# JuanJoZP/cfd-hemodynamic

Hardware: AMD Instinct MI355X
Metric: time-steps/sec, dfg_1 ~1M DOF (stabilized_schur) (higher is better)
Workload: dtype f64 (fp32 only in the AMG matrix values of the flexible preconditioner and in a read-only copy of the Krylov basis that Gram-Schmidt reads in solves of >= 20 iterations)

## Files before the change

### cfd_hemodynamic_amd/_lib.py

```python
from __future__ import annotations

import ctypes as C
import os
import subprocess

import numpy as np

_HERE = os.path.dirname(os.path.abspath(__file__))
_SO = os.path.join(_HERE, "libcfdh.so")
_LIB = None

dp = C.POINTER(C.c_double)
ip = C.POINTER(C.c_int32)
lp = C.POINTER(C.c_int64)


class Options(C.Structure):
    _fields_ = [
        ("snes_rtol", C.c_double), ("snes_atol", C.c_double), ("snes_stol", C.c_double), ("snes_max_it", C.c_int32),
        ("ksp_rtol", C.c_double), ("ksp_atol", C.c_double), ("ksp_max_it", C.c_int32), ("ksp_restart", C.c_int32),
        ("cheb_degree", C.c_int32), ("cheb_ratio", C.c_double), ("schur_full", C.c_int32),
        ("amg_smooth_degree", C.c_int32), ("amg_smooth_ratio", C.c_double), ("amg_theta", C.c_double),
        ("amg_max_coarse", C.c_int32), ("pc_refresh", C.c_int32), ("remove_p_mean", C.c_int32), ("verbose", C.c_int32),
        ("pc_type", C.c_int32), ("cc_smooth_degree", C.c_int32), ("ksp_guess", C.c_int32),
    ]


class Stats(C.Structure):
    _fields_ = [
        ("newton_its", C.c_int32), ("krylov_its", C.c_int32), ("reason", C.c_int32), ("pc_refreshes", C.c_int32),
        ("fnorm0", C.c_double), ("fnorm", C.c_double), ("ms_assemble", C.c_double), ("ms_solve", C.c_double),
        ("ms_pc_setup", C.c_double), ("ms_total", C.c_double),
    ]


class IpcsStats(C.Structure):
    _fields_ = [
        ("its", C.c_int32 * 3), ("reason", C.c_int32 * 3), ("rel_res", C.c_double * 3), ("ms_assemble", C.c_double),
        ("ms_solve", C.c_double * 3), ("ms_total", C.c_double), ("launches", C.c_int32), ("host_syncs", C.c_int32),
    ]


ALLREDUCE_FN = C.CFUNCTYPE(C.c_int, C.c_void_p, dp, C.c_int, C.c_int)
EXCHANGE_FN = C.CFUNCTYPE(C.c_int, C.c_void_p, dp, dp)

SYMBOLS = [
    "cfdh_create", "cfdh_create_elem", "cfdh_create_elem_part", "cfdh_set_facet_markers", "cfdh_destroy", "cfdh_last_error", "cfdh_abi_version", "cfdh_set_params", "cfdh_default_options",
    "cfdh_set_options", "cfdh_clear_dirichlet", "cfdh_add_dirichlet", "cfdh_update_dirichlet", "cfdh_set_state", "cfdh_get_solution",
    "cfdh_get_previous", "cfdh_get_residual", "cfdh_advance", "cfdh_advance_field", "cfdh_set_time_scheme", "cfdh_set_previous2", "cfdh_get_previous2",
    "cfdh_shift_history", "cfdh_set_boundary_terms", "cfdh_set_formulation", "cfdh_set_pressure_boundaries", "cfdh_assemble", "cfdh_get_csr", "cfdh_spmv", "cfdh_solve_step",
    "cfdh_functional", "cfdh_wall_shear_stress", "cfdh_set_global_pressure_space", "cfdh_set_halo", "cfdh_comm_unique_id", "cfdh_comm_init", "cfdh_comm_set_callbacks",
    "cfdh_profile_enable", "cfdh_profile_get", "cfdh_profile_reset", "cfdh_info",
    "cfdh_set_schur_pcd", "cfdh_set_ksp_forcing", "cfdh_get_newton_history", "cfdh_get_pcd_operator", "cfdh_apply_preconditioner", "cfdh_apply_operator",
    "cfdh_get_amg_operator", "cfdh_get_amg_vectors",
    "cfdh_create_ipcs", "cfdh_ipcs_set_form", "cfdh_ipcs_set_tolerances", "cfdh_ipcs_step", "cfdh_ipcs_get_operator", "cfdh_ipcs_get_intermediate",
    "cfdh_ipcs_apply_pressure_pc",
]


def build(force=False):
    src = os.path.join(_HERE, "csrc")
    newest = max(os.path.getmtime(os.path.join(src, f)) for f in os.listdir(src)
                 if f.endswith((".hip", ".cpp", ".hpp", ".h")))
    hdr = os.path.join(os.path.dirname(_HERE), "include", "cfdh.h")
    if os.path.exists(hdr):
        newest = max(newest, os.path.getmtime(hdr))
    if force or not os.path.exists(_SO) or os.path.getmtime(_SO) < newest:
        if not os.path.exists("/opt/rocm/bin/hipcc") and os.path.exists(_SO):
            return _SO
        subprocess.check_call(["make", "-C", src, "-s", "-j4"])
    return _SO


def lib():
    global _LIB
    if _LIB is not None:
        return _LIB
    if not os.path.exists(_SO):
        raise RuntimeError(
            "libcfdh.so is missing (%s): build it with `python -c 'import __graft_entry__ as g; g.build()'`; "
            "this package has no CPU fallback" % _SO)
    L = C.CDLL(_SO)
    vp = C.c_void_p
    L.cfdh_create.argtypes = [C.POINTER(vp), C.c_int, C.c_int, C.c_int64, C.c_int64, C.c_int64, ip, dp, C.c_int64, ip, ip, ip]
    L.cfdh_create_elem.argtypes = [C.POINTER(vp), C.c_int, C.c_int, C.c_int, C.c_int64, C.c_int64, ip, dp, C.c_int64, ip, ip, ip]
    L.cfdh_create_elem_part.argtypes = [C.POINTER(vp), C.c_int, C.c_int, C.c_int, C.c_int64, C.c_int64, C.c_int64, ip, dp, C.c_int64, ip, ip, ip]
    L.cfdh_set_facet_markers.argtypes = [vp, C.c_int64, ip]
    L.cfdh_destroy.argtypes = [vp]
    L.cfdh_destroy.restype = None
    L.cfdh_last_error.argtypes = [vp]
    L.cfdh_last_error.restype = C.c_char_p
    L.cfdh_set_params.argtypes = [vp, C.c_double, C.c_double, C.c_double, C.c_double, dp]
    L.cfdh_default_options.argtypes = [C.POINTER(Options)]
    L.cfdh_set_options.argtypes = [vp, C.POINTER(Options)]
    L.cfdh_clear_dirichlet.argtypes = [vp]
    L.cfdh_add_dirichlet.argtypes = [vp, C.c_int, C.c_int64, ip, dp]
    L.cfdh_update_dirichlet.argtypes = [vp, C.c_int, C.c_int64, ip, dp]
    L.cfdh_set_state.argtypes = [vp, dp, dp, dp, dp]
    L.cfdh_get_solution.argtypes = [vp, dp, dp]
    L.cfdh_set_time_scheme.argtypes = [vp, C.c_double, C.c_double, C.c_double, C.c_double]
    L.cfdh_set_previous2.argtypes = [vp, dp]
    L.cfdh_get_previous2.argtypes = [vp, dp]
    L.cfdh_shift_history.argtypes = [vp]
    L.cfdh_wall_shear_stress.argtypes = [vp, dp]
    L.cfdh_set_boundary_terms.argtypes = [vp, C.c_int, C.c_int, C.c_double]
    L.cfdh_set_formulation.argtypes = [vp, C.c_int]
    L.cfdh_set_pressure_boundaries.argtypes = [vp, C.c_int, ip, dp, C.c_double]
    L.cfdh_get_residual.argtypes = [vp, dp, dp]
    L.cfdh_get_previous.argtypes = [vp, dp, dp]
    L.cfdh_advance.argtypes = [vp]
    L.cfdh_advance_field.argtypes = [vp, C.c_int]
    L.cfdh_assemble.argtypes = [vp, C.c_int]
    L.cfdh_get_csr.argtypes = [vp, lp, ip, ip, dp]
    L.cfdh_spmv.argtypes = [vp, dp, dp]
    L.cfdh_solve_step.argtypes = [vp, C.POINTER(Stats)]
    L.cfdh_functional.argtypes = [vp, C.c_int, C.c_int, dp]
    L.cfdh_set_halo.argtypes = [vp, C.c_int, ip, lp, ip, lp, ip]
    L.cfdh_set_global_pressure_space.argtypes = [vp, C.c_int64, C.c_int64, ip, dp, ip, C.c_int64, ip]
    L.cfdh_comm_unique_id.argtypes = [C.c_void_p]
    L.cfdh_comm_init.argtypes = [vp, C.c_void_p, C.c_int, C.c_int]
    L.cfdh_comm_set_callbacks.argtypes = [vp, ALLREDUCE_FN, EXCHANGE_FN, C.c_void_p, C.c_int, C.c_int]
    L.cfdh_profile_enable.argtypes = [vp, C.c_int]
    L.cfdh_profile_get.argtypes = [vp, C.c_int, dp, lp]
    L.cfdh_profile_reset.argtypes = [vp]
    L.cfdh_info.argtypes = [vp, C.c_int]
    L.cfdh_info.restype = C.c_int64
    L.cfdh_set_schur_pcd.argtypes = [vp, C.c_int, C.c_int, C.c_int]
    L.cfdh_set_ksp_forcing.argtypes = [vp, C.c_int, C.c_double, C.c_double, C.c_double, C.c_double, C.c_double]
    L.cfdh_get_newton_history.argtypes = [vp, ip, dp, dp, ip, dp]
    L.cfdh_get_pcd_operator.argtypes = [vp, lp, ip, ip, dp, dp]
    L.cfdh_apply_preconditioner.argtypes = [vp, dp, dp]
    L.cfdh_apply_operator.argtypes = [vp, dp, dp, dp]
    L.cfdh_get_amg_operator.argtypes = [vp, C.c_int, C.c_int, C.c_int, lp, lp, lp, ip, ip, dp]
    L.cfdh_get_amg_vectors.argtypes = [vp, C.c_int, C.c_int, C.c_int, lp, dp]
    L.cfdh_create_ipcs.argtypes = [C.POINTER(vp), C.c_int, C.c_int, C.c_int64, C.c_int64, C.c_int64, ip, dp, C.c_int64, ip, ip, ip]
    L.cfdh_ipcs_set_form.argtypes = [vp, C.c_double, C.c_double]
    L.cfdh_ipcs_set_tolerances.argtypes = [vp, dp, C.c_double, ip]
    L.cfdh_ipcs_step.argtypes = [vp, C.POINTER(IpcsStats)]
    L.cfdh_ipcs_get_operator.argtypes = [vp, C.c_int, lp, ip, ip, dp]
    L.cfdh_ipcs_get_intermediate.argtypes = [vp, C.c_int, dp]
    L.cfdh_ipcs_apply_pressure_pc.argtypes = [vp, dp, dp]
    _LIB = L
    return L


def _dp(a):
    return None if a is None else a.ctypes.data_as(dp)


def _ip(a):
    return None if a is None else a.ctypes.data_as(ip)


def _lp(a):
    return None if a is None else a.ctypes.data_as(lp)


class CfdhError(RuntimeError):
    pass


def _raise(code, msg):
    if code == -1:
        raise ValueError(msg)
    raise CfdhError(msg)


FORM_CONVECTIVE, FORM_ROTATIONAL = 0, 1
PC_SELFP, PC_CAHOUET_CHABARD, PC_PCD = 0, 1, 2
AMG_HIER_A, AMG_HIER_P, AMG_HIER_H = 0, 1, 2
AMG_OP_A, AMG_OP_P, AMG_OP_G, AMG_OP_SB, AMG_OP_SC = 0, 1, 2, 3, 4
(AMG_VEC_DINV, AMG_VEC_WDINV, AMG_VEC_AGG, AMG_VEC_COARSE_INV, AMG_VEC_D, AMG_VEC_LAMBDA, AMG_VEC_CC_SCALARS, AMG_VEC_CC_ML,
 AMG_VEC_CC_PBC, AMG_VEC_SPGEMM_ROWS, AMG_VEC_SHAPE, AMG_VEC_ORDER, AMG_VEC_A00_LMAX, AMG_VEC_A00_DINV) = range(14)
EW_DEFAULTS = (0.3, 0.9, 1.0, (1.0 + 5.0 ** 0.5) / 2.0, 0.1)


class Context:

    def __init__(self, x, cells, facet_cells, facet_local, facet_marker, nv_owned=None, device=0, etype=0):
        L = lib()
        self.L = L
        x = np.asarray(x, dtype=np.float64)
        cells = np.asarray(cells)
        self.etype = int(etype)
        self.dim = (3 if x.shape[1] >= 3 and cells.shape[1] in (8, 10) or (self.etype == 3 and cells.shape[1] == 4) else 2) if self.etype \
            else cells.shape[1] - 1
        if self.dim not in (2, 3) or x.shape[1] < self.dim:
            raise ValueError("cells must be triangles [nc,3] or tetrahedra [nc,4] with matching coordinates")
        nodes = {(1, 2): 6, (2, 2): 4, (3, 2): 3, (1, 3): 10, (2, 3): 8, (3, 3): 4}
        if self.etype and cells.shape[1] != nodes[(self.etype, self.dim)]:
            raise ValueError("element type %d needs %d nodes per cell for gdim %d" % (self.etype, nodes[(self.etype, self.dim)], self.dim))
        self.x = np.ascontiguousarray(x[:, : self.dim]).copy()
        self.cells = np.ascontiguousarray(cells, dtype=np.int32)
        self.nv = len(self.x)
        self.nvo = self.nv if nv_owned is None else int(nv_owned)
        fc = np.ascontiguousarray(facet_cells, dtype=np.int32)
        fl = np.ascontiguousarray(facet_local, dtype=np.int32)
        fm = np.ascontiguousarray(facet_marker, dtype=np.int32)
        h = C.c_void_p()
        if self.etype:
            if self.nvo != self.nv:
                rc = L.cfdh_create_elem_part(C.byref(h), int(device), self.dim, self.etype, self.nv, self.nvo, len(self.cells), _ip(self.cells),
                                             _dp(self.x), len(fc), _ip(fc), _ip(fl), _ip(fm))
            else:
                rc = L.cfdh_create_elem(C.byref(h), int(device), self.dim, self.etype, self.nv, len(self.cells), _ip(self.cells), _dp(self.x),
                                        len(fc), _ip(fc), _ip(fl), _ip(fm))
        else:
            rc = L.cfdh_create(C.byref(h), int(device), self.dim, self.nv, self.nvo, len(self.cells), _ip(self.cells), _dp(self.x),
                               len(fc), _ip(fc), _ip(fl), _ip(fm))
        if rc != 0:
            _raise(rc, "cfdh_create failed: " + L.cfdh_last_error(None).decode())
        self.h = h
        self._cb = None

    def close(self):
# ... 144 lines not shown
        self._chk(self.L.cfdh_functional(self.h, int(kind), int(marker), C.byref(out)))
        return out.value

    def set_halo(self, nbr_rank, send_ptr, send_idx, recv_ptr, recv_idx):
        a = np.ascontiguousarray(nbr_rank, dtype=np.int32)
        sp_ = np.ascontiguousarray(send_ptr, dtype=np.int64)
        si = np.ascontiguousarray(send_idx, dtype=np.int32)
        rp = np.ascontiguousarray(recv_ptr, dtype=np.int64)
        ri = np.ascontiguousarray(recv_idx, dtype=np.int32)
        self._chk(self.L.cfdh_set_halo(self.h, len(a), _ip(a), _lp(sp_), _ip(si), _lp(rp), _ip(ri)))

    def set_global_pressure_space(self, x_global, cells_global, owned_global, pbc_nodes_global):
        xg = np.ascontiguousarray(x_global, dtype=np.float64)[:, : self.dim].copy()
        cg = np.ascontiguousarray(cells_global, dtype=np.int32)
        og = np.ascontiguousarray(owned_global, dtype=np.int32)
        pb = np.ascontiguousarray(pbc_nodes_global, dtype=np.int32)
        self._chk(self.L.cfdh_set_global_pressure_space(self.h, len(xg), len(cg), _ip(cg), _dp(xg), _ip(og), len(pb), _ip(pb)))

    def comm_init_rccl(self, uid_bytes, rank, nranks):
        buf = C.create_string_buffer(bytes(uid_bytes), 128)
        self._chk(self.L.cfdh_comm_init(self.h, buf, int(rank), int(nranks)))

    def comm_set_callbacks(self, allreduce, exchange, rank, nranks):
        self._cb = (ALLREDUCE_FN(allreduce), EXCHANGE_FN(exchange))
        self._chk(self.L.cfdh_comm_set_callbacks(self.h, self._cb[0], self._cb[1], None, int(rank), int(nranks)))

    def profile_enable(self, on=True):
        self._chk(self.L.cfdh_profile_enable(self.h, int(on)))

    def profile_reset(self):
        self._chk(self.L.cfdh_profile_reset(self.h))

    def profile_get(self, kind):
        ms, n = C.c_double(), C.c_int64()
        self._chk(self.L.cfdh_profile_get(self.h, int(kind), C.byref(ms), C.byref(n)))
        return ms.value, n.value

    def info(self, what):
        return int(self.L.cfdh_info(self.h, int(what)))

    def set_schur_pcd(self, inlet_marker, outlet_marker, time_term=1):
        self._chk(self.L.cfdh_set_schur_pcd(self.h, int(inlet_marker), int(outlet_marker), int(time_term)))

    def set_ksp_forcing(self, version=2, rtol_0=None, rtol_max=None, gamma=None, alpha=None, threshold=None):
        a = [d if v is None else float(v) for v, d in zip((rtol_0, rtol_max, gamma, alpha, threshold), EW_DEFAULTS)]
        self._chk(self.L.cfdh_set_ksp_forcing(self.h, int(version), *a))

    def newton_history(self):
        n = C.c_int32()
        self._chk(self.L.cfdh_get_newton_history(self.h, C.byref(n), None, None, None, None))
        fn, rt, rr = np.zeros(n.value), np.zeros(n.value), np.zeros(n.value)
        its = np.zeros(n.value, dtype=np.int32)
        self._chk(self.L.cfdh_get_newton_history(self.h, C.byref(n), _dp(fn), _dp(rt), _ip(its), _dp(rr)))
        return {"fnorm": fn, "ksp_rtol": rt, "ksp_its": its, "ksp_rel_res": rr}

    def get_pcd_operator(self):
        import scipy.sparse as sp
        nnz = C.c_int64()
        self._chk(self.L.cfdh_get_pcd_operator(self.h, C.byref(nnz), None, None, None, None))
        rowptr = np.empty(self.nvo + 1, dtype=np.int32)
        col = np.empty(nnz.value, dtype=np.int32)
        val = np.empty(nnz.value)
        md = np.empty(self.nvo)
        self._chk(self.L.cfdh_get_pcd_operator(self.h, C.byref(nnz), _ip(rowptr), _ip(col), _dp(val), _dp(md)))
        return sp.csr_matrix((val, col, rowptr), shape=(self.nvo, self.nv)), md

    def apply_preconditioner(self, r):
        r = np.ascontiguousarray(r, dtype=np.float64)
        if r.size != (self.dim + 1) * self.nv:
            raise ValueError("monolithic vector of (gdim + 1) nv entries expected")
        z = np.zeros_like(r)
        self._chk(self.L.cfdh_apply_preconditioner(self.h, _dp(r), _dp(z)))
        return z

    def apply_operator(self, r):
        r = np.ascontiguousarray(r, dtype=np.float64)
        if r.size != (self.dim + 1) * self.nv:
            raise ValueError("monolithic vector of (gdim + 1) nv entries expected")
        z = np.zeros_like(r)
        w = np.zeros((self.dim + 1) * self.nvo)
        self._chk(self.L.cfdh_apply_operator(self.h, _dp(r), _dp(z), _dp(w)))
        return z, w

    def get_amg_operator(self, hier, level, which, raw=False):
        import scipy.sparse as sp
        nr, nc, nnz = C.c_int64(), C.c_int64(), C.c_int64()
        self._chk(self.L.cfdh_get_amg_operator(self.h, int(hier), int(level), int(which), C.byref(nr), C.byref(nc), C.byref(nnz), None, None, None))
        rowptr = np.empty(nr.value + 1, dtype=np.int32)
        col = np.empty(nnz.value, dtype=np.int32)
        val = np.empty(nnz.value)
        self._chk(self.L.cfdh_get_amg_operator(self.h, int(hier), int(level), int(which), C.byref(nr), C.byref(nc), C.byref(nnz), _ip(rowptr),
                                               _ip(col), _dp(val)))
        if raw:
            return rowptr, col, val, (nr.value, nc.value), nnz.value
        return sp.csr_matrix((val, col, rowptr), shape=(nr.value, nc.value))

    def get_amg_vectors(self, hier, level, which):
        n = C.c_int64()
        self._chk(self.L.cfdh_get_amg_vectors(self.h, int(hier), int(level), int(which), C.byref(n), None))
        out = np.empty(n.value)
        self._chk(self.L.cfdh_get_amg_vectors(self.h, int(hier), int(level), int(which), C.byref(n), _dp(out)))
        return out


class IpcsContext(Context):

    def __init__(self, x, cells, nvert, facet_cells, facet_local, facet_marker, device=0):
        L = lib()
        self.L = L
        cells = np.ascontiguousarray(cells, dtype=np.int32)
        if cells.ndim != 2 or cells.shape[1] not in (6, 10):
            raise ValueError("cells must list the 6 nodes of P2 triangles or the 10 nodes of P2 tetrahedra")
        self.dim = 2 if cells.shape[1] == 6 else 3
        self.etype = 1
        self.x = np.ascontiguousarray(np.asarray(x, dtype=np.float64)[:, : self.dim]).copy()
        self.cells = cells
        self.nv = self.nvo = len(self.x)
        self.nvert = int(nvert)
        fc = np.ascontiguousarray(facet_cells, dtype=np.int32)
        fl = np.ascontiguousarray(facet_local, dtype=np.int32)
        fm = np.ascontiguousarray(facet_marker, dtype=np.int32)
        h = C.c_void_p()
        rc = L.cfdh_create_ipcs(C.byref(h), int(device), self.dim, self.nv, self.nvert, len(cells), _ip(cells), _dp(self.x), len(fc), _ip(fc), _ip(fl),
                                _ip(fm))
        if rc != 0:
            _raise(rc, "cfdh_create_ipcs failed: " + L.cfdh_last_error(None).decode())
        self.h = h
        self._cb = None

    def set_state(self, u_prev=None, p_prev=None, u=None, p=None):
        a = [None if v is None else np.ascontiguousarray(v, dtype=np.float64).reshape(-1) for v in (u_prev, p_prev, u, p)]
        for v, n in zip(a, (self.dim * self.nv, self.nvert, self.dim * self.nv, self.nvert)):
            if v is not None and v.size != n:
                raise ValueError("state array has wrong size")
        self._chk(self.L.cfdh_set_state(self.h, _dp(a[0]), _dp(a[1]), _dp(a[2]), _dp(a[3])))

    def get_solution(self, u=None, p=None):
        u = np.empty(self.dim * self.nv) if u is None else u
        p = np.empty(self.nvert) if p is None else p
        self._chk(self.L.cfdh_get_solution(self.h, _dp(u), _dp(p)))
        return u, p

    def get_previous(self, u=None, p=None):
        u = np.empty(self.dim * self.nv) if u is None else u
        p = np.empty(self.nvert) if p is None else p
        self._chk(self.L.cfdh_get_previous(self.h, _dp(u), _dp(p)))
        return u, p

    def set_form(self, conv_coeff, force_coeff):
        self._chk(self.L.cfdh_ipcs_set_form(self.h, float(conv_coeff), float(force_coeff)))

    def set_tolerances(self, rtol=(1e-5, 1e-5, 1e-5), atol=1e-50, max_it=(10000, 10000, 10000)):
        r = np.ascontiguousarray(np.broadcast_to(np.asarray(rtol, dtype=np.float64), (3,)))
        m = np.ascontiguousarray(np.broadcast_to(np.asarray(max_it, dtype=np.int32), (3,)))
        self._chk(self.L.cfdh_ipcs_set_tolerances(self.h, _dp(r), float(atol), _ip(m)))

    def step(self):
        st = IpcsStats()
        rc = self.L.cfdh_ipcs_step(self.h, C.byref(st))
        if rc != 0:
            msg = self.L.cfdh_last_error(self.h).decode()
            if rc == -4:
                bad = [r for r in st.reason if r <= 0]
                raise RuntimeError("Did not converge, reason: %d. (%s)" % (bad[0] if bad else 0, msg))
            _raise(rc, msg)
        return st
# ... 35 lines not shown
```

### cfd_hemodynamic_amd/csrc/cfdh_amg_dev.hip

```cpp
#include <hip/hip_runtime.h>

#include <algorithm>
#include <chrono>
#include <cmath>

#include "cfdh_internal.hpp"

#define TPB 256

namespace {

double now_ms() {
  using namespace std::chrono;
  return duration<double, std::milli>(steady_clock::now().time_since_epoch()).count();
}

__device__ __forceinline__ int wave_incl_scan(int v, int lane) {
#pragma unroll
  for (int d = 1; d < 64; d <<= 1) {
    const int t = __shfl_up(v, d);
    if (lane >= d) v += t;
  }
  return v;
}
__global__ __launch_bounds__(TPB) void scan_block_kernel(int n, int *__restrict__ a, int *__restrict__ sums) {
  __shared__ int wsum[4];
  const int t = threadIdx.x, lane = t & 63, wv = t >> 6;
  const int base = blockIdx.x * 1024 + t * 4;
  int v[4], s = 0;
#pragma unroll
  for (int q = 0; q < 4; q++) { v[q] = base + q < n ? a[base + q] : 0; s += v[q]; v[q] = s; }
  int inc = wave_incl_scan(s, lane);
  if (lane == 63) wsum[wv] = inc;
  __syncthreads();
  int off = inc - s;
  for (int w = 0; w < wv; w++) off += wsum[w];
#pragma unroll
  for (int q = 0; q < 4; q++) if (base + q < n) a[base + q] = v[q] + off;
  if (t == TPB - 1) sums[blockIdx.x] = off + s;
}
__global__ __launch_bounds__(TPB) void scan_sums_kernel(int nb, int *__restrict__ sums) {
  __shared__ int wsum[4];
  __shared__ int carry_s;
  const int t = threadIdx.x, lane = t & 63, wv = t >> 6;
  if (t == 0) carry_s = 0;
  __syncthreads();
  for (int b0 = 0; b0 < nb; b0 += TPB) {
    const int v = b0 + t < nb ? sums[b0 + t] : 0;
    int inc = wave_incl_scan(v, lane);
    if (lane == 63) wsum[wv] = inc;
    __syncthreads();
    int off = carry_s;
    for (int w = 0; w < wv; w++) off += wsum[w];
    if (b0 + t < nb) sums[b0 + t] = inc + off;
    __syncthreads();
    if (t == TPB - 1) carry_s = inc + off;
    __syncthreads();
  }
}
__global__ __launch_bounds__(TPB) void scan_add_kernel(int n, int *__restrict__ a, const int *__restrict__ sums) {
  const int b = blockIdx.x + 1;
  const int off = sums[b - 1];
  const int base = b * 1024 + threadIdx.x * 4;
#pragma unroll
  for (int q = 0; q < 4; q++) if (base + q < n) a[base + q] += off;
}

struct Dev {
  cfdh_ctx *c;
  hipStream_t s;
  dbuf<int> scan_sums;
  int rc = 0;
  long long *path_rows = nullptr;
  explicit Dev(cfdh_ctx *c_) : c(c_), s(c_->stream) {}
  int scan(int *a, int n) {
    if (n <= 0) return 0;
    const int nb = (n + 1023) / 1024;
    if ((size_t)nb > scan_sums.n) HIPCHK(c, scan_sums.alloc((size_t)nb + 1024));
    hipLaunchKernelGGL(scan_block_kernel, dim3(nb), dim3(TPB), 0, s, n, a, scan_sums.p);
    if (nb > 1) {
      hipLaunchKernelGGL(scan_sums_kernel, dim3(1), dim3(TPB), 0, s, nb, scan_sums.p);
      hipLaunchKernelGGL(scan_add_kernel, dim3(nb - 1), dim3(TPB), 0, s, n, a, scan_sums.p);
    }
    HIPCHK(c, hipGetLastError());
    return 0;
  }
  int read_int(const int *p, int *out) {
    HIPCHK(c, hipMemcpyAsync(out, p, sizeof(int), hipMemcpyDeviceToHost, s));
    HIPCHK(c, hipStreamSynchronize(s));
// ... 806 lines not shown
    *na_out = na;
    return 0;
  }
};

struct ProxyF {
  const double *A00;
  int dim, nvo;
  __device__ double value(int i, int k, int w) const {
    double v = 0.0;
    for (int q = 0; q < dim; q++) v += A00[(size_t)dim * dim * k + (size_t)q * (dim + 1)];
    return v / dim;
  }
  __device__ bool whole_row_identity(int) const { return false; }
  __device__ bool keep(int i, int k, int w) const { return w < nvo && (w == i || value(i, k, w) != 0.0); }
};
struct HF {
  const double *A11, *Lval, *Ml;
  const unsigned char *pbc;
  const int *vdiag;
  double alpha, beta;
  int nvo;
  __device__ bool whole_row_identity(int i) const { return (pbc[i] & 1) != 0; }
  __device__ bool keep(int, int, int w) const { return w < nvo && !(pbc[w] & 1); }
  __device__ double value(int i, int k, int w) const {
    double v = beta * A11[k];
    if (w == i) {
      const int kd = vdiag[i];
      const double T = Lval[kd] > 0 ? A11[kd] / Lval[kd] : 0.0;
      v += (1.0 + alpha * T) * Ml[i];
    }
    return v;
  }
};
template <class F>
__global__ __launch_bounds__(TPB) void vg_count_kernel(int n, const int *__restrict__ vptr, const int *__restrict__ vcol, F f, int *__restrict__ rp1) {
  const int i = blockIdx.x * TPB + threadIdx.x;
  if (i >= n) return;
  int cnt = 0;
  if (f.whole_row_identity(i)) cnt = 1;
  else for (int k = vptr[i], e = vptr[i + 1]; k < e; k++) cnt += f.keep(i, k, vcol[k]) ? 1 : 0;
  rp1[i + 1] = cnt;
}
template <class F>
__global__ __launch_bounds__(TPB) void vg_fill_kernel(int n, const int *__restrict__ vptr, const int *__restrict__ vcol, F f, const int *__restrict__ rp,
                                                      int *__restrict__ col, double *__restrict__ val) {
  const int i = blockIdx.x * TPB + threadIdx.x;
  if (i >= n) return;
  int p = rp[i];
  if (f.whole_row_identity(i)) { col[p] = i; val[p] = 1.0; return; }
  for (int k = vptr[i], e = vptr[i + 1]; k < e; k++) {
    const int w = vcol[k];
    if (f.keep(i, k, w)) { col[p] = w; val[p] = f.value(i, k, w); p++; }
  }
}
template <class F>
int vg_build(cfdh_ctx *c, F f, CsrDev &out) {
  Dev dv(c);
  hipStream_t s = c->stream;
  const int n = c->nvo;
  out.n = out.m = n;
  HIPCHK(c, out.rowptr.alloc((size_t)n + 1));
  HIPCHK(c, hipMemsetAsync(out.rowptr.p, 0, sizeof(int), s));
  hipLaunchKernelGGL((vg_count_kernel<F>), dim3((n + TPB - 1) / TPB), dim3(TPB), 0, s, n, c->vptr.p, c->vcol.p, f, out.rowptr.p);
  CHK(dv.scan(out.rowptr.p + 1, n));
  int nnz = 0;
  CHK(dv.read_int(out.rowptr.p + n, &nnz));
  out.nnz = nnz;
  HIPCHK(c, out.col.alloc((size_t)std::max(nnz, 1)));
  HIPCHK(c, out.val.alloc((size_t)std::max(nnz, 1)));
  hipLaunchKernelGGL((vg_fill_kernel<F>), dim3((n + TPB - 1) / TPB), dim3(TPB), 0, s, n, c->vptr.p, c->vcol.p, f, out.rowptr.p, out.col.p, out.val.p);
  HIPCHK(c, hipGetLastError());
  return 0;
}

static void move_csr(CsrDev &dst, CsrDev &src) {
  dst.n = src.n; dst.m = src.m; dst.nnz = src.nnz;
  dst.rowptr.adopt(src.rowptr); dst.col.adopt(src.col); dst.val.adopt(src.val);
}

}

int cfdh_aggregate_host_csr(const CsrHost &A, double theta, std::vector<int> &agg);

int cfdh_amg_setup_dev(cfdh_ctx *c, AmgHier &H, CsrDev &A0, bool singular, int ncol) {
  const double t_begin = now_ms();
  Builder B(c);
  hipStream_t s = c->stream;
  const cfdh_options &o = c->opt;
  H.clear();
  H.ncol = ncol;
  H.fused = false; H.nnz_G0 = H.nnz_S0 = 0;
  H.fine_nnz = A0.nnz;
  const char *ml_env = getenv(&H == &c->hA ? "CFDH_A_MAXLEV" : "CFDH_L_MAXLEV");
  const int maxlev = ml_env && atoi(ml_env) >= 1 ? std::min(atoi(ml_env), 16) : 16;
  static const double theta_env = getenv("CFDH_AMG_THETA") ? atof(getenv("CFDH_AMG_THETA")) : -1.0;
  const double theta = o.amg_theta >= 0 ? o.amg_theta : (theta_env >= 0 ? theta_env : (c->dim == 3 ? 0.02 : 0.07));
  const bool host_agg = getenv("CFDH_AMG_AGG") && !strcmp(getenv("CFDH_AMG_AGG"), "host");
  const bool keep = getenv("CFDH_AMG_KEEP") && getenv("CFDH_AMG_KEEP")[0] == '1';
  for (long long &q : H.spgemm_rows) q = 0;
  B.dv.path_rows = H.spgemm_rows;
  const bool velocity = &H == &c->hA;
  const char *gap_env = getenv(velocity ? "CFDH_AGG_GAP_A" : "CFDH_AGG_GAP_L");
  if (!gap_env) gap_env = getenv("CFDH_AGG_GAP");
  const int gap = gap_env ? atoi(gap_env) : (velocity ? 4 : 0);
  CsrDev A;
  move_csr(A, A0);
  AmgLevel *lastL = nullptr;
  double tm[10] = {0, 0, 0, 0, 0, 0, 0, 0, 0, 0}, tq = now_ms();
  const bool timing = c->opt.verbose > 0;
#define TICK(i) do { if (timing) { (void)hipStreamSynchronize(s); const double n_ = now_ms(); tm[i] += n_ - tq; tq = n_; } } while (0)
  for (;;) {
    AmgLevel *L = new AmgLevel();
    H.lev.push_back(L);
    double lm = 1.0;
    TICK(9);
    CHK(B.level_quantities(*L, A, o.amg_smooth_ratio, &lm));
    CHK(B.work_vectors(*L, ncol));
    TICK(0);
    L->fine = A.nnz <= (c->dim == 3 ? 20ll : 12ll) * A.n && A.n >= 16384;
    L->sell = L->fine && (A.nnz <= 12ll * A.n || ncol == 1);
    const bool last = A.n <= o.amg_max_coarse || (int)H.lev.size() >= maxlev;
    int na = 0;
    dbuf<int> agg;
    static const bool no_pmg = getenv("CFDH_NO_PMG") && getenv("CFDH_NO_PMG")[0] == '1';
    const bool pmg = !last && !no_pmg && H.lev.size() == 1 && c->etype == 1 && c->gen_P1.n == A.n && c->gen_P1.m > 0;
    if (!last && !pmg) {
      if (host_agg) {
        CsrHost Ah;
        Ah.n = Ah.m = A.n;
        Ah.rowptr.resize((size_t)A.n + 1); Ah.col.resize(A.nnz); Ah.val.resize(A.nnz);
        HIPCHK(c, hipMemcpyAsync(Ah.rowptr.data(), A.rowptr.p, sizeof(int) * ((size_t)A.n + 1), hipMemcpyDeviceToHost, s));
        HIPCHK(c, hipMemcpyAsync(Ah.col.data(), A.col.p, sizeof(int) * (size_t)A.nnz, hipMemcpyDeviceToHost, s));
        HIPCHK(c, hipMemcpyAsync(Ah.val.data(), A.val.p, sizeof(double) * (size_t)A.nnz, hipMemcpyDeviceToHost, s));
        HIPCHK(c, hipStreamSynchronize(s));
        std::vector<int> ha;
        na = cfdh_aggregate_host_csr(Ah, theta, ha);
        HIPCHK(c, agg.upload(ha, s));
        HIPCHK(c, hipStreamSynchronize(s));
      } else {
        CHK(B.aggregate(A, theta, gap, agg, &na));
      }
    }
    TICK(1);
    if (pmg) na = c->gen_P1.m;
    if (last || na >= A.n || na < 1) {
      move_csr(L->A, A);
      break;
    }
    const MatV Am{A.rowptr.p, A.col.p, A.val.p};
    CsrDev P, R, AP, Ac;
    if (pmg) {
      P.n = c->gen_P1.n; P.m = c->gen_P1.m; P.nnz = c->gen_P1.nnz();
      HIPCHK(c, P.rowptr.upload(c->gen_P1.rowptr, s)); HIPCHK(c, P.col.upload(c->gen_P1.col, s)); HIPCHK(c, P.val.upload(c->gen_P1.val, s));
      HIPCHK(c, hipStreamSynchronize(s));
    } else
    CHK((Spgemm<AOpImwDA, BOpAgg>::run(B.dv, A.n, na, AOpImwDA{Am, L->dinv.p, 4.0 / 3.0 / lm, agg.p}, BOpAgg{agg.p}, P, B.lists, B.tmp, B.cnts)));
    TICK(2);
    if (H.keep_host0 && H.lev.size() == 1) {
      auto down = [&](const CsrDev &D, CsrHost &Hc) -> int {
        Hc.n = D.n; Hc.m = D.m;
        Hc.rowptr.resize((size_t)D.n + 1); Hc.col.resize((size_t)D.nnz); Hc.val.resize((size_t)D.nnz);
        HIPCHK(c, hipMemcpyAsync(Hc.rowptr.data(), D.rowptr.p, sizeof(int) * ((size_t)D.n + 1), hipMemcpyDeviceToHost, s));
        HIPCHK(c, hipMemcpyAsync(Hc.col.data(), D.col.p, sizeof(int) * (size_t)D.nnz, hipMemcpyDeviceToHost, s));
        HIPCHK(c, hipMemcpyAsync(Hc.val.data(), D.val.p, sizeof(double) * (size_t)D.nnz, hipMemcpyDeviceToHost, s));
        return 0;
// ... 1 lines not shown
      CHK(down(A, H.h_A0)); CHK(down(P, H.h_P0));
      H.h_wdinv0.resize((size_t)A.n);
      HIPCHK(c, hipMemcpyAsync(H.h_wdinv0.data(), L->wdinv.p, sizeof(double) * (size_t)A.n, hipMemcpyDeviceToHost, s));
      HIPCHK(c, hipStreamSynchronize(s));
    }
    CHK(B.transpose(P, R));
    TICK(3);
    const MatV Pm{P.rowptr.p, P.col.p, P.val.p}, Rm{R.rowptr.p, R.col.p, R.val.p};
    CHK((Spgemm<AOpPlain, BOpPlain>::run(B.dv, A.n, na, AOpPlain{Am}, BOpPlain{Pm}, AP, B.lists, B.tmp, B.cnts)));
    TICK(4);
    CHK((Spgemm<AOpPlain, BOpImAW>::run(B.dv, na, A.n, AOpPlain{Rm}, BOpImAW{Am, L->wdinv.p}, L->G, B.lists, B.tmp, B.cnts)));
    TICK(5);
    L->Sb.n = A.n; L->Sb.m = A.n; L->Sb.nnz = A.nnz;
    HIPCHK(c, L->Sb.rowptr.alloc((size_t)A.n + 1)); HIPCHK(c, L->Sb.col.alloc(A.nnz)); HIPCHK(c, L->Sb.val.alloc(A.nnz));
    HIPCHK(c, hipMemcpyAsync(L->Sb.rowptr.p, A.rowptr.p, sizeof(int) * ((size_t)A.n + 1), hipMemcpyDeviceToDevice, s));
    HIPCHK(c, hipMemcpyAsync(L->Sb.col.p, A.col.p, sizeof(int) * (size_t)A.nnz, hipMemcpyDeviceToDevice, s));
    hipLaunchKernelGGL(sb_kernel, dim3((unsigned)((8ll * A.n + TPB - 1) / TPB)), dim3(TPB), 0, s, A.n, A.rowptr.p, A.col.p, A.val.p, L->wdinv.p, L->Sb.val.p);
    L->Sc.n = A.n; L->Sc.m = na; L->Sc.nnz = AP.nnz;
    HIPCHK(c, L->Sc.rowptr.alloc((size_t)A.n + 1)); HIPCHK(c, L->Sc.col.alloc(std::max(AP.nnz, 1))); HIPCHK(c, L->Sc.val.alloc(std::max(AP.nnz, 1)));
    HIPCHK(c, hipMemcpyAsync(L->Sc.rowptr.p, AP.rowptr.p, sizeof(int) * ((size_t)A.n + 1), hipMemcpyDeviceToDevice, s));
    HIPCHK(c, hipMemcpyAsync(L->Sc.col.p, AP.col.p, sizeof(int) * (size_t)AP.nnz, hipMemcpyDeviceToDevice, s));
    hipLaunchKernelGGL(sc_kernel, dim3((A.n + TPB - 1) / TPB), dim3(TPB), 0, s, A.n, AP.rowptr.p, AP.col.p, AP.val.p, P.rowptr.p, P.col.p, P.val.p,
                       L->wdinv.p, L->Sc.val.p);
    HIPCHK(c, hipGetLastError());
    TICK(6);
    const MatV APm{AP.rowptr.p, AP.col.p, AP.val.p};
    CHK((Spgemm<AOpPlain, BOpPlain>::run(B.dv, na, na, AOpPlain{Rm}, BOpPlain{APm}, Ac, B.lists, B.tmp, B.cnts)));
    TICK(7);
    if (L->fine) CHK(B.formats(L->G, CFDH_UP_CSRF));
    if (L->sell) { CHK(B.formats(L->Sb, CFDH_UP_SELL)); CHK(B.formats(L->Sc, CFDH_UP_SELL)); }
    if (H.lev.size() == 1) { H.nnz_G0 = L->G.nnz; H.nnz_S0 = (long long)L->Sb.nnz + L->Sc.nnz; }
    if (c->nranks > 1) { move_csr(L->P, P); move_csr(L->R, R); }
    else if (keep) { move_csr(L->P, P); L->agg.adopt(agg); }
    move_csr(L->A, A);
    lastL = L;
    move_csr(A, Ac);
    HIPCHK(c, hipStreamSynchronize(s));
    TICK(8);
  }
  tq = now_ms();
  AmgLevel *Lc = H.lev.back();
  const int n = Lc->n;
  H.coarse_n = 0;
  if (n > 2500) {
    CsrDev &A = Lc->A;
    Lc->Sb.n = n; Lc->Sb.m = n; Lc->Sb.nnz = A.nnz;
    HIPCHK(c, Lc->Sb.rowptr.alloc((size_t)n + 1)); HIPCHK(c, Lc->Sb.col.alloc(A.nnz)); HIPCHK(c, Lc->Sb.val.alloc(A.nnz));
    HIPCHK(c, hipMemcpyAsync(Lc->Sb.rowptr.p, A.rowptr.p, sizeof(int) * ((size_t)n + 1), hipMemcpyDeviceToDevice, s));
    HIPCHK(c, hipMemcpyAsync(Lc->Sb.col.p, A.col.p, sizeof(int) * (size_t)A.nnz, hipMemcpyDeviceToDevice, s));
    hipLaunchKernelGGL(sb_kernel, dim3((unsigned)((8ll * n + TPB - 1) / TPB)), dim3(TPB), 0, s, n, A.rowptr.p, A.col.p, A.val.p, Lc->wdinv.p, Lc->Sb.val.p);
    if (Lc->sell) CHK(B.formats(Lc->Sb, CFDH_UP_SELL));
    H.fused = true;
  } else {
    dbuf<double> D0, D1, ad;
    dbuf<int> failf;
    HIPCHK(c, D0.alloc((size_t)n * n)); HIPCHK(c, D1.alloc((size_t)n * n)); HIPCHK(c, ad.alloc(n)); HIPCHK(c, failf.alloc(4));
    HIPCHK(c, D0.zero(s)); HIPCHK(c, failf.zero(s));
    hipLaunchKernelGGL(densify_kernel, dim3((n + TPB - 1) / TPB), dim3(TPB), 0, s, n, Lc->A.rowptr.p, Lc->A.col.p, Lc->A.val.p, D0.p, ad.p);
    if (singular) hipLaunchKernelGGL(trace_shift_kernel, dim3(64), dim3(TPB), 0, s, n, ad.p, D0.p);
    const unsigned gb = (unsigned)(((size_t)n * n + TPB - 1) / TPB);
    double *in = D0.p, *out = D1.p;
    for (int p = 0; p < n; p++) { hipLaunchKernelGGL(gj_step_kernel, dim3(gb), dim3(TPB), 0, s, n, p, in, out, failf.p); std::swap(in, out); }
    HIPCHK(c, hipGetLastError());
    int hf = 0;
    CHK(B.dv.read_int(failf.p, &hf));
    if (hf) return cfdh_fail(c, CFDH_E_STATE, "singular coarsest AMG operator (n=%d, device Gauss-Jordan)", n);
    HIPCHK(c, H.coarse_inv.alloc((size_t)n * n));
    HIPCHK(c, hipMemcpyAsync(H.coarse_inv.p, in, sizeof(double) * (size_t)n * n, hipMemcpyDeviceToDevice, s));
    H.coarse_n = n;
    if (lastL) {
      H.fused = true;
      lastL->Dn = 0;
      const long long ent = (long long)lastL->n * n;
      if (lastL->Sc.m == n && ent <= 8000000ll && !lastL->sell) {
        HIPCHK(c, lastL->D.alloc((size_t)ent));
        hipLaunchKernelGGL(fold_dense_kernel, dim3(lastL->n), dim3(TPB), 0, s, lastL->n, n, lastL->Sc.rowptr.p, lastL->Sc.col.p, lastL->Sc.val.p,
                           H.coarse_inv.p, lastL->D.p);
        HIPCHK(c, hipGetLastError());
        lastL->Dn = n;
      }
    }
    HIPCHK(c, hipStreamSynchronize(s));
  }
  H.valid = true;
  HIPCHK(c, hipStreamSynchronize(s));
  if (c->opt.verbose) {
    fprintf(stderr, "[cfdh] AMG hierarchy built on the device in %.1f ms (ncol %d%s):", now_ms() - t_begin, ncol, H.fused ? ", fused" : "");
    for (AmgLevel *l : H.lev) fprintf(stderr, " (%d, nnz %d; G %d Sb %d Sc %d D %d)", l->n, l->A.nnz, l->G.nnz, l->Sb.nnz, l->Sc.nnz, l->Dn);
    fprintf(stderr, "\n[cfdh]   ms: level quantities %.1f, aggregation %.1f, P %.1f, R = P^T %.1f, A P %.1f, G %.1f, Sb + Sc %.1f, A_c %.1f, formats %.1f, releases %.1f, "
            "coarsest level %.1f\n", tm[0], tm[1], tm[2], tm[3], tm[4], tm[5], tm[6], tm[7], tm[8], tm[9], now_ms() - tq);
  }
#undef TICK
  return 0;
}

int cfdh_level_setup_dev(cfdh_ctx *c, AmgLevel &L, CsrDev &A, double ratio, int ncol) {
  Builder B(c);
  double lm;
  CHK(B.level_quantities(L, A, ratio, &lm));
  CHK(B.work_vectors(L, ncol));
  move_csr(L.A, A);
  CHK(B.formats(L.A, CFDH_UP_SELL, L.wdinv.p));
  HIPCHK(c, hipStreamSynchronize(c->stream));
  return 0;
}

bool cfdh_amg_dev_enabled(const cfdh_ctx *c) {
  const bool host_only = getenv("CFDH_AMG_HOST") && getenv("CFDH_AMG_HOST")[0] == '1';
  const char *nf = getenv("CFDH_NO_FUSED_AMG");
  return !host_only && c->opt.amg_smooth_degree == 1 && !(nf && nf[0] == '1');
}

int cfdh_proxy_dev(cfdh_ctx *c, CsrDev &out) { return vg_build(c, ProxyF{c->A00.p, c->dim, c->nvo}, out); }

namespace {
__global__ __launch_bounds__(TPB) void ras_pack_kernel(int nvo, int dim, int k0, const int *__restrict__ vptr, const int *__restrict__ vcol,
                                                       const double *__restrict__ A00, const int *__restrict__ gid, double *__restrict__ rec) {
  const int i = blockIdx.x * TPB + threadIdx.x;
  if (i >= nvo) return;
  for (int t = 0; t <= dim; t++) {
    const int k = vptr[i] + k0 + t;
    double v = gid ? -1.0 : 0.0;
    if (k < vptr[i + 1]) {
      if (gid) v = (double)gid[vcol[k]];
      else {
        v = 0.0;
        for (int q = 0; q < dim; q++) v += A00[(size_t)dim * dim * k + (size_t)q * (dim + 1)];
        v /= dim;
      }
    }
    rec[t < dim ? (size_t)dim * i + t : (size_t)dim * nvo + i] = v;
  }
}
__global__ __launch_bounds__(TPB) void ras_unpack_kernel(int ng, int nvo, int dim, int k0, int maxlen, const double *__restrict__ rec,
                                                         double *__restrict__ gval) {
  const int g = blockIdx.x * TPB + threadIdx.x;
  if (g >= ng) return;
  const size_t W = (size_t)dim + 1;
  for (int t = 0; t <= dim; t++)
    if (k0 + t < maxlen) gval[(size_t)g * maxlen + k0 + t] = rec[W * (size_t)nvo + W * (size_t)g + t];
}
__device__ __forceinline__ double ras_proxy_value(const double *A00, int dim, int k) {
  double v = 0.0;
  for (int q = 0; q < dim; q++) v += A00[(size_t)dim * dim * k + (size_t)q * (dim + 1)];
  return v / dim;
}
template <bool FILL>
__global__ __launch_bounds__(TPB) void ras_rows_kernel(int nv, int nvo, int dim, int maxlen, const int *__restrict__ vptr, const int *__restrict__ vcol,
                                                       const double *__restrict__ A00, const int *__restrict__ gptr, const int *__restrict__ gcol,
                                                       const int *__restrict__ gsrc, const double *__restrict__ gval, int *__restrict__ rp,
                                                       int *__restrict__ col, double *__restrict__ val) {
  const int i = blockIdx.x * TPB + threadIdx.x;
  if (i >= nv) return;
  int p = FILL ? rp[i] : 0;
  if (i < nvo) {
    for (int k = vptr[i], e = vptr[i + 1]; k < e; k++) {
      const int w = vcol[k];
      if (w >= nv) continue;
      const double v = ras_proxy_value(A00, dim, k);
      if (v == 0.0 && w != i) continue;
      if (FILL) { col[p] = w; val[p] = v; }
      p++;
    }
  } else {
    const int g = i - nvo;
    for (int j = gptr[g], e = gptr[g + 1]; j < e; j++) {
// ... 97 lines not shown
```

### cfd_hemodynamic_amd/csrc/cfdh_api.cpp

```cpp
#include <algorithm>
#include <cmath>
#include <numeric>

#include <dlfcn.h>

#include "cfdh_internal.hpp"
#include "cfdh_ipcs.hpp"

std::string g_cfdh_last_error;

int cfdh_prepare_assembly(cfdh_ctx *c);

#define ENTER(c)                         \
  do {                                   \
    if (!(c)) return CFDH_E_ARG;         \
    (void)hipSetDevice((c)->device);     \
  } while (0)

#define NOT_IPCS(c, name)                                                                                                    \
  do {                                                                                                                       \
    if ((c) && (c)->ipcs) return cfdh_fail((c), CFDH_E_STATE, name ": not available on an incremental pressure-correction context (cfdh_create_ipcs)"); \
  } while (0)
#define NEED_IPCS(c, name)                                                                                         \
  do {                                                                                                             \
    if (!(c)) return CFDH_E_ARG;                                                                                   \
    if (!(c)->ipcs) return cfdh_fail((c), CFDH_E_STATE, name ": the context was not created by cfdh_create_ipcs"); \
    (void)hipSetDevice((c)->device);                                                                               \
  } while (0)

static int ipcs_put(cfdh_ctx *c, dbuf<double> &dst, const double *src) {
  if (!src) return 0;
  c->ipcs->n_field_copies++;
  HIPCHK(c, hipMemcpyAsync(dst.p, src, sizeof(double) * dst.n, hipMemcpyHostToDevice, c->stream));
  HIPCHK(c, hipStreamSynchronize(c->stream));
  return 0;
}
static int ipcs_get(cfdh_ctx *c, const dbuf<double> &src, double *dst) {
  if (!dst) return 0;
  c->ipcs->n_field_copies++;
  HIPCHK(c, hipMemcpyAsync(dst, src.p, sizeof(double) * src.n, hipMemcpyDeviceToHost, c->stream));
  HIPCHK(c, hipStreamSynchronize(c->stream));
  return 0;
}
static int ipcs_copy(cfdh_ctx *c, const dbuf<double> &src, dbuf<double> &dst) {
  HIPCHK(c, hipMemcpyAsync(dst.p, src.p, sizeof(double) * src.n, hipMemcpyDeviceToDevice, c->stream));
  return 0;
}

extern "C" {

int cfdh_abi_version(void) { return CFDH_ABI_VERSION; }

const char *cfdh_last_error(const cfdh_ctx *c) { return c ? c->err.c_str() : g_cfdh_last_error.c_str(); }

int cfdh_default_options(cfdh_options *o) {
  if (!o) return CFDH_E_ARG;
  o->snes_rtol = 1e-8; o->snes_atol = 1e-50; o->snes_stol = 1e-8; o->snes_max_it = 100;
  o->ksp_rtol = 1e-5; o->ksp_atol = 1e-50; o->ksp_max_it = 1000; o->ksp_restart = 200;
  o->cheb_degree = 3; o->cheb_ratio = 10.0; o->schur_full = 2;
  o->amg_smooth_degree = 1; o->amg_smooth_ratio = 8.0; o->amg_theta = -1.0; o->amg_max_coarse = 1000;
  o->pc_refresh = 0; o->remove_p_mean = 1; o->verbose = 0; o->pc_type = 1; o->cc_smooth_degree = 2;
  o->ksp_guess = getenv("CFDH_KSP_GUESS") ? atoi(getenv("CFDH_KSP_GUESS")) : 4;
  return 0;
}

static int create_ctx(cfdh_ctx **out, int device, int gdim, int etype, int64_t nv, int64_t nv_owned, int64_t nc, const int32_t *cells,
                      const double *coords, int64_t nfacets, const int32_t *facet_cells, const int32_t *facet_local,
                      const int32_t *facet_marker) {
  if (!out) return cfdh_fail(nullptr, CFDH_E_ARG, "null output pointer");
  *out = nullptr;
  if (gdim != 2 && gdim != 3) return cfdh_fail(nullptr, CFDH_E_ARG, "gdim must be 2 (P1 triangles) or 3 (P1 tetrahedra)");
  if (etype < 0 || etype > 3) return cfdh_fail(nullptr, CFDH_E_ARG, "unknown element type %d", etype);
  if (!cells || !coords || (nfacets > 0 && (!facet_cells || !facet_local)))
    return cfdh_fail(nullptr, CFDH_E_ARG, "null mesh array");
  int ndev = 0;
  if (hipGetDeviceCount(&ndev) != hipSuccess || ndev <= 0)
    return cfdh_fail(nullptr, CFDH_E_HIP, "no HIP device available: libcfdh has no CPU fallback");
  if (device < 0 || device >= ndev) return cfdh_fail(nullptr, CFDH_E_ARG, "device %d out of range (%d devices)", device, ndev);
  cfdh_ctx *c = new (std::nothrow) cfdh_ctx();
  if (!c) return cfdh_fail(nullptr, CFDH_E_NOMEM, "out of host memory");
  c->device = device;
  cfdh_default_options(&c->opt);
  { const char *e = getenv("CFDH_NO_GRAPH"); c->use_graph = !(e && e[0] == '1'); }
  { const char *e = getenv("CFDH_SOLVE_LEAN"); c->lean = !(e && e[0] == '0'); }
  {
    cfdh_ctx::SolveEnv &v = c->env;
    const char *e;
    if ((e = getenv("CFDH_KRYLOV_FP32"))) v.krylov_fp32 = atoi(e);
    v.guess_check = getenv("CFDH_GUESS_CHECK") != nullptr;
    e = getenv("CFDH_NO_ATTAINABLE_STOP"); v.no_attainable_stop = e && e[0] == '1';
    if ((e = getenv("CFDH_GS_REFINE_FROM"))) v.gs_refine_from = atoi(e);
    if ((e = getenv("CFDH_KSP_LAG"))) v.ksp_lag = atoi(e);
    if ((e = getenv("CFDH_GS_ETA2"))) v.gs_eta2 = atof(e);
    if ((e = getenv("CFDH_L_CYCLES"))) v.l_cycles = atoi(e);
    if ((e = getenv("CFDH_A_CYCLES"))) v.a_cycles = atoi(e);
  }
  if (c->use_graph && (getenv("ROCP_TOOL_LIBRARIES") || dlsym(RTLD_DEFAULT, "rocprofiler_configure"))) {
    int rt = 0;
    const char *ov = getenv("CFDH_GRAPH_UNDER_PROFILER");
    if (!(ov && ov[0] == '1') && hipRuntimeGetVersion(&rt) == hipSuccess && rt >= 70200000) c->use_graph = false;
  }
  memset(&c->last_stats, 0, sizeof c->last_stats);
  int rc = 0;
  do {
    if (hipSetDevice(device) != hipSuccess) { rc = cfdh_fail(nullptr, CFDH_E_HIP, "hipSetDevice(%d) failed", device); break; }
    if (hipStreamCreateWithFlags(&c->stream, hipStreamNonBlocking) != hipSuccess) { rc = cfdh_fail(nullptr, CFDH_E_HIP, "hipStreamCreate failed"); break; }
    rc = gdim == 3 ? k3_upload_quadrature(c) : k_upload_quadrature(c);
    if (rc) break;
    if (etype != 0) {
      rc = gdim == 3 ? kg3_upload_tables(c) : kg_upload_tables(c);
      if (rc) break;
      rc = gdim == 3 ? cfdh_build_mesh_gen3(c, etype, nv, nv_owned, nc, cells, coords, nfacets, facet_cells, facet_local, facet_marker)
                     : cfdh_build_mesh_gen(c, etype, nv, nv_owned, nc, cells, coords, nfacets, facet_cells, facet_local, facet_marker);
      break;
    }
    rc = gdim == 3 ? cfdh_build_mesh3(c, nv, nv_owned, nc, cells, coords, nfacets, facet_cells, facet_local, facet_marker)
                   : cfdh_build_mesh(c, nv, nv_owned, nc, cells, coords, nfacets, facet_cells, facet_local, facet_marker);
  } while (0);
  if (rc) {
    g_cfdh_last_error = c->err.empty() ? g_cfdh_last_error : c->err;
    cfdh_destroy(c);
    return rc;
  }
  *out = c;
  return 0;
}

int cfdh_create(cfdh_ctx **out, int device, int gdim, int64_t nv, int64_t nv_owned, int64_t nc, const int32_t *cells,
                const double *coords, int64_t nfacets, const int32_t *facet_cells, const int32_t *facet_local,
                const int32_t *facet_marker) {
  return create_ctx(out, device, gdim, CFDH_ELEM_P1, nv, nv_owned, nc, cells, coords, nfacets, facet_cells, facet_local, facet_marker);
}

int cfdh_create_elem(cfdh_ctx **out, int device, int gdim, int elem, int64_t nn, int64_t nc, const int32_t *cells, const double *node_coords,
                     int64_t nfacets, const int32_t *facet_cells, const int32_t *facet_local, const int32_t *facet_marker) {
  return create_ctx(out, device, gdim, elem, nn, nn, nc, cells, node_coords, nfacets, facet_cells, facet_local, facet_marker);
}

int cfdh_create_elem_part(cfdh_ctx **out, int device, int gdim, int elem, int64_t nn, int64_t nn_owned, int64_t nc, const int32_t *cells,
                          const double *node_coords, int64_t nfacets, const int32_t *facet_cells, const int32_t *facet_local, const int32_t *facet_marker) {
  return create_ctx(out, device, gdim, elem, nn, nn_owned, nc, cells, node_coords, nfacets, facet_cells, facet_local, facet_marker);
}

void cfdh_destroy(cfdh_ctx *c) {
  if (!c) return;
  (void)hipSetDevice(c->device);
  if (c->stream) (void)hipStreamSynchronize(c->stream);
  cfdh_ipcs_free(c);
  comm_finalize(c);
  c->hS.clear(); c->hL.clear(); c->hA.clear(); c->hLg.clear();
  for (hipEvent_t e : c->ev_pool) (void)hipEventDestroy(e);
  for (auto &e : c->pc_graphs) for (auto &x : e.exec) if (x) (void)hipGraphExecDestroy(x);
  if (c->h_pinned) (void)hipHostFree(c->h_pinned);
  if (c->h_stage) (void)hipHostFree(c->h_stage);
  if (c->ev_h) (void)hipEventDestroy(c->ev_h);
  if (c->h_big) (void)hipHostFree(c->h_big);
  if (c->h_ring) (void)hipHostFree(c->h_ring);
  for (hipEvent_t e : c->ev_ring) if (e) (void)hipEventDestroy(e);
  hipStream_t s = c->stream;
  delete c;
  if (s) (void)hipStreamDestroy(s);
}

int cfdh_set_params(cfdh_ctx *c, double dt, double rho, double mu, double mu_facet, const double f[3]) {
  ENTER(c);
  if (!(dt > 0) || !(rho > 0) || !(mu > 0)) return cfdh_fail(c, CFDH_E_ARG, "dt, rho, mu must be positive");
  const bool changed = !c->params_set || dt != c->dt || rho != c->rho || mu != c->mu;
// ... 372 lines not shown
  const bool markers_changed = !c->pcd_set || inlet_marker != c->pcd_in || outlet_marker != c->pcd_out;
  c->pcd_in = inlet_marker; c->pcd_out = outlet_marker; c->pcd_time = time_term;
  c->pcd_set = true;
  if (markers_changed) { c->pcd_ready = false; c->pc_valid = false; }
  return 0;
}

int cfdh_set_ksp_forcing(cfdh_ctx *c, int version, double rtol_0, double rtol_max, double gamma, double alpha, double threshold) {
  NOT_IPCS(c, "cfdh_set_ksp_forcing");
  ENTER(c);
  if (version != 0 && version != 2) return cfdh_fail(c, CFDH_E_ARG, "cfdh_set_ksp_forcing: version 0 (off) or 2");
  if (version == 2 && !(rtol_0 > 0 && rtol_0 < 1 && rtol_max > 0 && rtol_max < 1 && gamma > 0 && gamma <= 1 && alpha > 1 && alpha <= 2 &&
                        threshold > 0 && threshold < 1))
    return cfdh_fail(c, CFDH_E_ARG, "cfdh_set_ksp_forcing: need 0 < rtol_0, rtol_max, threshold < 1, 0 < gamma <= 1, 1 < alpha <= 2");
  c->ew_version = version;
  if (version == 2) { c->ew_rtol0 = rtol_0; c->ew_rtol_max = rtol_max; c->ew_gamma = gamma; c->ew_alpha = alpha; c->ew_threshold = threshold; }
  return 0;
}

int cfdh_get_newton_history(cfdh_ctx *c, int32_t *n, double *fnorm, double *ksp_rtol, int32_t *ksp_its, double *ksp_rel_res) {
  NOT_IPCS(c, "cfdh_get_newton_history");
  if (!c || !n) return CFDH_E_ARG;
  const size_t m = c->hist_fnorm.size();
  *n = (int32_t)m;
  for (size_t k = 0; k < m; k++) {
    if (fnorm) fnorm[k] = c->hist_fnorm[k];
    if (ksp_rtol) ksp_rtol[k] = c->hist_rtol[k];
    if (ksp_its) ksp_its[k] = c->hist_its[k];
    if (ksp_rel_res) ksp_rel_res[k] = c->hist_relres[k];
  }
  return 0;
}

int cfdh_get_pcd_operator(cfdh_ctx *c, int64_t *nnz, int32_t *rowptr, int32_t *col, double *vals, double *mass_diag) {
  NOT_IPCS(c, "cfdh_get_pcd_operator");
  if (!c || !nnz) return CFDH_E_ARG;
  ENTER(c);
  *nnz = c->nnzv;
  if (!rowptr && !col && !vals && !mass_diag) return 0;
  if (!rowptr || !col || !vals) return cfdh_fail(c, CFDH_E_ARG, "pass all of rowptr/col/vals or none");
  CHK(cfdh_pcd_supported(c, "cfdh_get_pcd_operator"));
  if (!c->pcd_set) return cfdh_fail(c, CFDH_E_STATE, "cfdh_get_pcd_operator: cfdh_set_schur_pcd was not called");
  if (!c->params_set || !c->state_set) return cfdh_fail(c, CFDH_E_STATE, "cfdh_get_pcd_operator: parameters and state are needed");
  CHK(k_pcd_assemble(c, c->x.p));
  std::vector<double> K(c->pcd_K.n);
  std::vector<int> sptr(c->pcd_sptr.n);
  HIPCHK(c, hipMemcpyAsync(K.data(), c->pcd_K.p, sizeof(double) * K.size(), hipMemcpyDeviceToHost, c->stream));
  HIPCHK(c, hipMemcpyAsync(sptr.data(), c->pcd_sptr.p, sizeof(int) * sptr.size(), hipMemcpyDeviceToHost, c->stream));
  HIPCHK(c, hipStreamSynchronize(c->stream));
  const int nvo = c->nvo;
  int64_t pos = 0;
  std::vector<std::pair<int, int>> ord;
  for (int vu = 0; vu < nvo; vu++) {
    const int r = c->perm[vu];
    ord.clear();
    for (int k = c->h_vptr[r]; k < c->h_vptr[r + 1]; k++) ord.push_back({c->iperm[c->h_vcol[k]], k - c->h_vptr[r]});
    std::sort(ord.begin(), ord.end());
    rowptr[vu] = (int32_t)pos;
    const size_t base = (size_t)sptr[r >> 6] + (r & 63);
    for (auto &e : ord) { col[pos] = e.first; vals[pos] = K[base + 64 * (size_t)e.second]; pos++; }
  }
  rowptr[nvo] = (int32_t)pos;
  if (mass_diag) for (int vu = 0; vu < nvo; vu++) mass_diag[vu] = c->h_pcd_md[c->perm[vu]];
  return 0;
}

int cfdh_apply_preconditioner(cfdh_ctx *c, const double *r, double *z) {
  NOT_IPCS(c, "cfdh_apply_preconditioner");
  if (!c || !r || !z) return CFDH_E_ARG;
  ENTER(c);
  if (!c->jac_valid) return cfdh_fail(c, CFDH_E_STATE, "no Jacobian assembled yet");
  CHK(cfdh_pc_update(c, false));
  std::vector<double> h;
  pack_vec(c, r, r + (size_t)c->dim * c->nv, h, nullptr);
  CHK(upload_vec(c, h, c->xt.p));
  CHK(cfdh_pc_apply(c, c->xt.p, c->dvec.p));
  std::vector<double> o;
  CHK(download_vec(c, c->dvec.p, o));
  for (int k = 0; k < c->nvo; k++) {
    const int v = c->iperm[k], d = c->dim;
    for (int i = 0; i < d; i++) z[(size_t)d * v + i] = o[(size_t)d * k + i];
    z[(size_t)d * c->nv + v] = o[(size_t)d * c->nvo + k];
  }
  return 0;
}

int cfdh_apply_operator(cfdh_ctx *c, const double *r, double *z, double *w) {
  NOT_IPCS(c, "cfdh_apply_operator");
  if (!c || !r || !z || !w) return CFDH_E_ARG;
  ENTER(c);
  if (c->nranks > 1 || c->nvo != c->nv) return cfdh_fail(c, CFDH_E_STATE, "cfdh_apply_operator: one GPU only");
  if (!c->jac_valid) return cfdh_fail(c, CFDH_E_STATE, "no Jacobian assembled yet");
  CHK(cfdh_pc_update(c, false));
  std::vector<double> h;
  pack_vec(c, r, r + (size_t)c->dim * c->nv, h, nullptr);
  CHK(upload_vec(c, h, c->xt.p));
  CHK(cfdh_apply_operator_dev(c, c->xt.p, c->dvec.p));
  std::vector<double> oz, ow;
  CHK(download_vec(c, c->dvec.p, oz));
  CHK(download_vec(c, c->kw.p, ow));
  for (int k = 0; k < c->nvo; k++) {
    const int v = c->iperm[k], d = c->dim;
    for (int i = 0; i < d; i++) { z[(size_t)d * v + i] = oz[(size_t)d * k + i]; w[(size_t)d * v + i] = ow[(size_t)d * k + i]; }
    z[(size_t)d * c->nv + v] = oz[(size_t)d * c->nvo + k];
    w[(size_t)d * c->nvo + v] = ow[(size_t)d * c->nvo + k];
  }
  return 0;
}

static int amg_pick(cfdh_ctx *c, const char *name, int hier, int level, AmgHier **H, AmgLevel **L) {
  if (c->nranks > 1 || c->nvo != c->nv) return cfdh_fail(c, CFDH_E_STATE, "%s: one GPU only", name);
  if (!c->pc_valid) return cfdh_fail(c, CFDH_E_STATE, "%s: no preconditioner built yet (cfdh_apply_preconditioner or cfdh_solve_step first)", name);
  *H = nullptr;
  if (hier == CFDH_AMG_HIER_H) {
    if (c->opt.pc_type != 1 || c->Hlev.n <= 0) return cfdh_fail(c, CFDH_E_STATE, "%s: H exists for pc_type 1 only", name);
    *L = &c->Hlev;
    return 0;
  }
  if (hier != CFDH_AMG_HIER_A && hier != CFDH_AMG_HIER_P) return cfdh_fail(c, CFDH_E_ARG, "%s: unknown hierarchy %d", name, hier);
  if (hier == CFDH_AMG_HIER_A && c->opt.pc_type == 0) return cfdh_fail(c, CFDH_E_STATE, "%s: pc_type 0 has no velocity hierarchy", name);
  AmgHier *h = hier == CFDH_AMG_HIER_A ? &c->hA : (c->opt.pc_type == 0 ? &c->hS : &c->hL);
  if (!h->valid) return cfdh_fail(c, CFDH_E_STATE, "%s: hierarchy %d is not built", name, hier);
  if (level < 0 || level >= (int)h->lev.size()) return cfdh_fail(c, CFDH_E_ARG, "%s: level %d of %d", name, level, (int)h->lev.size());
  *H = h;
  *L = h->lev[level];
  return 0;
}

int cfdh_get_amg_operator(cfdh_ctx *c, int hier, int level, int which, int64_t *nrow, int64_t *ncol, int64_t *nnz, int32_t *rowptr,
                          int32_t *col, double *vals) {
  NOT_IPCS(c, "cfdh_get_amg_operator");
  if (!c || !nrow || !ncol || !nnz) return CFDH_E_ARG;
  ENTER(c);
  AmgHier *H = nullptr;
  AmgLevel *L = nullptr;
  CHK(amg_pick(c, "cfdh_get_amg_operator", hier, level, &H, &L));
  if (which < CFDH_AMG_OP_A || which > CFDH_AMG_OP_SC) return cfdh_fail(c, CFDH_E_ARG, "cfdh_get_amg_operator: unknown operator %d", which);
  if (!H) level = 0;
  const CsrDev &M = which == CFDH_AMG_OP_A ? L->A : which == CFDH_AMG_OP_P ? L->P : which == CFDH_AMG_OP_G ? L->G : which == CFDH_AMG_OP_SB ? L->Sb : L->Sc;
  if (M.n <= 0 || !M.rowptr.p || !M.col.p || !M.val.p)
    return cfdh_fail(c, CFDH_E_STATE, "cfdh_get_amg_operator: operator %d of level %d is not kept in fp64 CSR (P: CFDH_AMG_KEEP=1 before the build)", which, level);
  *nrow = M.n; *ncol = M.m; *nnz = M.nnz;
  if (!rowptr && !col && !vals) return 0;
  if (!rowptr || !col || !vals) return cfdh_fail(c, CFDH_E_ARG, "pass all of rowptr/col/vals or none");
  std::vector<int> rp((size_t)M.n + 1), cl((size_t)M.nnz);
  std::vector<double> vl((size_t)M.nnz);
  HIPCHK(c, hipMemcpyAsync(rp.data(), M.rowptr.p, sizeof(int) * rp.size(), hipMemcpyDeviceToHost, c->stream));
  if (M.nnz > 0) {
    HIPCHK(c, hipMemcpyAsync(cl.data(), M.col.p, sizeof(int) * cl.size(), hipMemcpyDeviceToHost, c->stream));
    HIPCHK(c, hipMemcpyAsync(vl.data(), M.val.p, sizeof(double) * vl.size(), hipMemcpyDeviceToHost, c->stream));
  }
  HIPCHK(c, hipStreamSynchronize(c->stream));
  if (rp[M.n] != M.nnz) return cfdh_fail(c, CFDH_E_STATE, "cfdh_get_amg_operator: rowptr ends at %d, the operator holds %d entries", rp[M.n], M.nnz);
  const bool rows0 = level == 0 && which != CFDH_AMG_OP_G && (int)c->perm.size() == M.n;
  const bool cols0 = level == 0 && (which == CFDH_AMG_OP_A || which == CFDH_AMG_OP_SB || which == CFDH_AMG_OP_G) && (int)c->iperm.size() == M.m;
  int64_t pos = 0;
  std::vector<std::pair<int, double>> row;
  for (int ru = 0; ru < M.n; ru++) {
    const int r = rows0 ? c->perm[ru] : ru;
    rowptr[ru] = (int32_t)pos;
    row.clear();
    for (int k = rp[r]; k < rp[r + 1]; k++) row.push_back({cols0 ? c->iperm[cl[k]] : cl[k], vl[k]});
    if (cols0) std::stable_sort(row.begin(), row.end(), [](const std::pair<int, double> &a, const std::pair<int, double> &b) { return a.first < b.first; });
    for (auto &e : row) { col[pos] = e.first; vals[pos] = e.second; pos++; }
  }
  rowptr[M.n] = (int32_t)pos;
// ... 435 lines not shown
  return 0;
}
int cfdh_profile_get(cfdh_ctx *c, int kind, double *total_ms, int64_t *launches) {
  NOT_IPCS(c, "cfdh_profile_get");
  if (!c || kind < 0 || kind >= 12) return CFDH_E_ARG;
  prof_flush(c);
  if (total_ms) *total_ms = c->prof[kind].total_ms;
  if (launches) *launches = c->prof[kind].launches;
  return 0;
}
int cfdh_profile_reset(cfdh_ctx *c) {
  NOT_IPCS(c, "cfdh_profile_reset");
  ENTER(c);
  prof_flush(c);
  for (auto &p : c->prof) { p.total_ms = 0; p.launches = 0; }
  c->n_allreduce = c->n_halo = c->n_host_sync = c->n_krylov = c->n_allgather = 0;
  c->n_cycles = c->n_guess_projections = c->n_iter_sync = 0;
  c->n_krylov_discarded = 0;
  return 0;
}

int64_t cfdh_info(const cfdh_ctx *c, int what) {
  if (!c) return -1;
  if (c->ipcs) {
    const IpcsData *I = c->ipcs;
    switch (what) {
      case 0: case 1: return I->nn;
      case 2: return I->nc;
      case 3: return (int64_t)I->hM.col.size();
      case 6: return (int64_t)I->hLam.lev.size();
      case 15: return I->last.host_syncs;
      case 18: return 1;
      case 26: return I->D;
      case 29: return I->NL;
      case 80: return I->last.launches;
      case 81: return I->nvert;
      case 82: return I->n_field_copies;
      case 83: return 1;
      default: return -1;
    }
  }
  switch (what) {
    case 0: return c->nvo;
    case 1: return c->nv;
    case 2: return c->nc;
    case 3: return c->nnzv;
    case 4: return c->opt.pc_type >= 1 ? c->hL.fine_nnz : c->hS.fine_nnz;
    case 5: return c->ninc;
    case 6: return (int64_t)(c->opt.pc_type >= 1 ? c->hL.lev.size() : c->hS.lev.size());
    case 7: return c->nblk;
    case 8: return c->hA.fine_nnz;
    case 9: return c->gp_allgather ? c->gp_maxcnt : 0;
    case 10: return c->nccl_comm ? 1 : 0;
    case 11: return c->dl0.on ? c->dl0.n1 : 0;
    case 12: return c->ras ? 1 : 0;
    case 13: return c->n_allreduce;
    case 14: return c->n_halo;
    case 15: return c->n_host_sync;
    case 16: return c->n_krylov;
    case 17: return c->n_allgather;
    case 18: return c->nranks;
    case 26: return c->dim;
    case 30: case 31: case 32: case 33: case 34: case 35: case 36: case 37: case 38: case 39:
    case 40: case 41: case 42: case 43: case 44: case 45: case 46: case 47: case 48: case 49:
    case 50: case 51: case 52: case 53: case 54: case 55: case 56: case 57: case 58: case 59:
    case 60: case 61: case 62: case 63: case 64: case 65: case 66: case 67: case 68: case 69: {
      const AmgHier &h = what < 50 ? c->hA : (c->opt.pc_type >= 1 ? c->hL : c->hS);
      const size_t l = (size_t)(what % 10);
      if (l >= h.lev.size()) return 0;
      return ((what / 10) & 1) ? (int64_t)h.lev[l]->n : (int64_t)h.lev[l]->A.nnz;
    }
    case 28: return c->etype;
    case 70: return c->n_guess_solves;
    case 71: return c->n_guess_solves ? (int64_t)(1e6 * c->guess_reduction_sum / (double)c->n_guess_solves) : 0;
    case 29: return c->nloc;
    case 73: return c->n_krylov_discarded;
    case 74: return c->n_pc_builds;
    case 84: return c->n_cycles;
    case 86: return c->n_guess_projections;
    case 87: return c->n_iter_sync;
    case 88: return c->guess_last_rank;
    case 89: return c->guess_last_k;
    case 85: return c->lean ? 1 : 0;
    case 75: return c->pc_valid ? 1 : 0;
    case 76: return c->singular;
    case 77: return c->form;
    case 78: return c->opt.pc_type;
    case 79: return c->ew_version;
    case 72: return c->n_attainable_stops;
    case 27: return (int64_t)(1000.0 * c->ms_pc_build_dev);
    case 19: return c->opt.pc_type >= 1 ? c->hL.nnz_S0 : c->hS.nnz_S0;
    case 20: return c->hA.nnz_S0;
    case 21: return c->opt.pc_type >= 1 ? c->hL.nnz_G0 : c->hS.nnz_G0;
    case 22: return c->hA.nnz_G0;
    case 23: { const AmgHier &h = c->opt.pc_type >= 1 ? c->hL : c->hS; return h.lev.size() > 1 ? h.lev[1]->n : 0; }
    case 24: return c->hA.lev.size() > 1 ? c->hA.lev[1]->n : 0;
    case 25: { const AmgHier &h = c->opt.pc_type >= 1 ? c->hL : c->hS; return h.fused ? 1 : 0; }
    default: return -1;
  }
}


int cfdh_create_ipcs(cfdh_ctx **out, int device, int gdim, int64_t nn, int64_t nvert, int64_t nc, const int32_t *cells, const double *node_coords,
                     int64_t nfacets, const int32_t *facet_cells, const int32_t *facet_local, const int32_t *facet_marker) {
  if (!out) return cfdh_fail(nullptr, CFDH_E_ARG, "null output pointer");
  *out = nullptr;
  if (gdim != 2 && gdim != 3) return cfdh_fail(nullptr, CFDH_E_ARG, "gdim must be 2 (P2/P1 triangles) or 3 (P2/P1 tetrahedra)");
  if (!cells || !node_coords || nfacets < 0 || (nfacets > 0 && (!facet_cells || !facet_local))) return cfdh_fail(nullptr, CFDH_E_ARG, "null mesh array");
  int ndev = 0;
  if (hipGetDeviceCount(&ndev) != hipSuccess || ndev <= 0)
    return cfdh_fail(nullptr, CFDH_E_HIP, "no HIP device available: libcfdh has no CPU fallback");
  if (device < 0 || device >= ndev) return cfdh_fail(nullptr, CFDH_E_ARG, "device %d out of range (%d devices)", device, ndev);
  cfdh_ctx *c = new (std::nothrow) cfdh_ctx();
  if (!c) return cfdh_fail(nullptr, CFDH_E_NOMEM, "out of host memory");
  c->device = device;
  cfdh_default_options(&c->opt);
  c->use_graph = false;
  memset(&c->last_stats, 0, sizeof c->last_stats);
  int rc = 0;
  if (hipSetDevice(device) != hipSuccess) rc = cfdh_fail(nullptr, CFDH_E_HIP, "hipSetDevice(%d) failed", device);
  else if (hipStreamCreateWithFlags(&c->stream, hipStreamNonBlocking) != hipSuccess) rc = cfdh_fail(nullptr, CFDH_E_HIP, "hipStreamCreate failed");
  else rc = cfdh_ipcs_create(c, gdim, nn, nvert, nc, cells, node_coords, nfacets, facet_cells, facet_local, facet_marker);
  if (rc) {
    g_cfdh_last_error = c->err.empty() ? g_cfdh_last_error : c->err;
    cfdh_destroy(c);
    return rc;
  }
  *out = c;
  return 0;
}

int cfdh_ipcs_set_form(cfdh_ctx *c, double conv_coeff, double force_coeff) {
  NEED_IPCS(c, "cfdh_ipcs_set_form");
  if (!(conv_coeff >= 0) || !std::isfinite(conv_coeff) || !std::isfinite(force_coeff)) return cfdh_fail(c, CFDH_E_ARG, "cfdh_ipcs_set_form: conv_coeff >= 0 and finite coefficients");
  c->ipcs->conv_coeff = conv_coeff; c->ipcs->force_coeff = force_coeff; c->ipcs->force_default = false;
  c->ipcs->assembled = false;
  return 0;
}

int cfdh_ipcs_set_tolerances(cfdh_ctx *c, const double rtol[3], double atol, const int32_t max_it[3]) {
  NEED_IPCS(c, "cfdh_ipcs_set_tolerances");
  if (!rtol || !max_it || !(atol >= 0)) return cfdh_fail(c, CFDH_E_ARG, "cfdh_ipcs_set_tolerances: bad arguments");
  for (int k = 0; k < 3; k++)
    if (!(rtol[k] >= 0) || !(rtol[k] < 1) || max_it[k] < 1) return cfdh_fail(c, CFDH_E_ARG, "cfdh_ipcs_set_tolerances: 0 <= rtol < 1, max_it >= 1");
  for (int k = 0; k < 3; k++) { c->ipcs->rtol[k] = rtol[k]; c->ipcs->max_it[k] = max_it[k]; }
  c->ipcs->atol = atol;
  return 0;
}

int cfdh_ipcs_step(cfdh_ctx *c, cfdh_ipcs_stats *stats) {
  NEED_IPCS(c, "cfdh_ipcs_step");
  c->err.clear();
  cfdh_ipcs_stats st;
  const int rc = cfdh_ipcs_step_impl(c, &st);
  if (stats) *stats = st;
  return rc;
}

int cfdh_ipcs_get_operator(cfdh_ctx *c, int which, int64_t *nnz, int32_t *rowptr, int32_t *col, double *vals) {
  NEED_IPCS(c, "cfdh_ipcs_get_operator");
  IpcsData *I = c->ipcs;
  const int D = I->D;
  if (!nnz || which < 0 || which >= 3 + 2 * D) return cfdh_fail(c, CFDH_E_ARG, "cfdh_ipcs_get_operator: which in [0, %d)", 3 + 2 * D);
  const std::vector<int> &ptr = which == 1 ? I->hL.rowptr : which < 3 ? I->hM.rowptr : which < 3 + D ? I->bptr : I->gptr;
  const std::vector<int> &cl = which == 1 ? I->hL.col : which < 3 ? I->hM.col : which < 3 + D ? I->bcol : I->gcol;
  *nnz = (int64_t)cl.size();
// ... 42 lines not shown
```

### cfd_hemodynamic_amd/csrc/cfdh_internal.hpp

```cpp
#pragma once
#include <hip/hip_runtime.h>

#include <cstdint>
#include <cstdio>
#include <cstring>
#include <string>
#include <vector>

#include "cfdh.h"

#ifndef CFDH_MAX_INC
#define CFDH_MAX_INC 256
#endif
#ifndef CFDH_MAX_BV
#define CFDH_MAX_BV 192
#endif
#ifndef CFDH_MAX_BC
#define CFDH_MAX_BC 192
#endif
#ifndef CFDH_MAX_ROWS
#define CFDH_MAX_ROWS 128
#endif

#if defined(__HIPCC__)
__device__ __forceinline__ double cfdh_rsqrt(double x) {
  double y = __builtin_amdgcn_rsq(x);
  const double h = 0.5 * x;
  y = __builtin_fma(y, __builtin_fma(-h * y, y, 0.5), y);
  y = __builtin_fma(y, __builtin_fma(-h * y, y, 0.5), y);
  return y;
}
#endif

template <class T>
struct dbuf {
  T *p = nullptr;
  size_t n = 0;
  dbuf() = default;
  dbuf(const dbuf &) = delete;
  dbuf &operator=(const dbuf &) = delete;
  ~dbuf() { release(); }
  void release() {
    if (p) (void)hipFree(p);
    p = nullptr;
    n = 0;
  }
  hipError_t alloc(size_t count) {
    if (count == n && p) return hipSuccess;
    release();
    if (count == 0) return hipSuccess;
    hipError_t e = hipMalloc((void **)&p, count * sizeof(T));
    if (e == hipSuccess) n = count;
    return e;
  }
  hipError_t upload(const std::vector<T> &h, hipStream_t s) {
    hipError_t e = alloc(h.size());
    if (e != hipSuccess || h.empty()) return e;
    return hipMemcpyAsync(p, h.data(), h.size() * sizeof(T), hipMemcpyHostToDevice, s);
  }
  hipError_t zero(hipStream_t s) { return n ? hipMemsetAsync(p, 0, n * sizeof(T), s) : hipSuccess; }
  void adopt(dbuf &o) {
    if (&o == this) return;
    release();
    p = o.p; n = o.n;
    o.p = nullptr; o.n = 0;
  }
};

struct CsrHost {
  int n = 0, m = 0;
  std::vector<int> rowptr, col;
  std::vector<double> val;
  int nnz() const { return (int)col.size(); }
};

struct CsrDev {
  int n = 0, m = 0, nnz = 0;
  dbuf<int> rowptr, col;
  dbuf<double> val;
  int nslice = 0, sell_maxw = 0;
  dbuf<int> sptr, scol;
  dbuf<float> sval, svalw;
  dbuf<float> valf;
};
enum { CFDH_UP_CSR = 1, CFDH_UP_SELL = 2, CFDH_UP_CSRF = 4};

struct AmgLevel {
  int n = 0;
  CsrDev A, P, R;
  dbuf<double> dinv, wdinv, x, b, r, d0, d1;
  double lmax = 0, lmin = 0;
  CsrDev G, Sb, Sc;
  dbuf<float> D;
  int Dn = 0;
  bool fine = false;
  bool sell = false;
  dbuf<int> agg;
};

struct AmgHier {
  std::vector<AmgLevel *> lev;
  dbuf<double> coarse_inv;
  int coarse_n = 0, ncol = 1;
  long long fine_nnz = 0;
  bool valid = false;
  bool fused = false;
  long long nnz_G0 = 0, nnz_S0 = 0;
  long long spgemm_rows[3] = {0, 0, 0};
  bool keep_host0 = false;
  CsrHost h_A0, h_P0;
  std::vector<double> h_wdinv0;
  void clear() {
    for (AmgLevel *l : lev) delete l;
    lev.clear();
    valid = false;
  }
  ~AmgHier() { clear(); }
};

struct ProfSlot {
  double total_ms = 0;
  long long launches = 0;
};

struct IpcsData;

struct cfdh_ctx {
  int device = 0;
  IpcsData *ipcs = nullptr;
  hipStream_t stream = nullptr;
  std::string err;

  int dim = 2;
  int etype = 0, nloc = 3;
  bool gen = false;
  dbuf<int> gslot;
  dbuf<int> g_eptr, g_fptr, g_fdst;
  dbuf<double> gE, gEF;
  dbuf<unsigned short> gflag;
  dbuf<unsigned char> gpbidx;
  dbuf<int> g3_fcells;
  int g3_nfcells = 0;
  dbuf<unsigned char> g3_pbslot;
  dbuf<int> g3_pcells;
  int g3_npcells = 0;
  CsrHost gen_P1;
  int nv = 0, nvo = 0, ng = 0, nc = 0, nfac = 0;
  int NL = 0;
  int NO = 0;

  std::vector<int> perm;
  std::vector<int> iperm;
  std::vector<int> h_cells;
  std::vector<int> cell_user;
  std::vector<double> h_coords;
  std::vector<int> fac_cell, fac_local, fac_marker;
  std::vector<int> fac_user;
  int nfac_user = 0;

  bool params_set = false;
  double dt = 0, rho = 0, mu = 0, muf = 0, f[3] = {0, 0, 0};
  cfdh_options opt;

  dbuf<double> coords;
  dbuf<int> cells;
  dbuf<unsigned char> cflag;
// ... 105 lines not shown
  long long bc_version = 0;
  int gp_n = 0;
  CsrHost gp_L;
  bool gp_singular = false, gp_dirty = false;
  AmgHier hLg;
  dbuf<int> gp_l2g;
  dbuf<double> gp_rhs, gp_sol;
  bool ras = false;
  std::vector<int> h_gid;
  std::vector<int> h_g2l;
  dbuf<double> ras_b, ras_x;
  struct RasPlan {
    bool ready = false;
    int maxlen = 0;
    int nent = 0;
    dbuf<int> gptr, gcol, gsrc;
    dbuf<double> gval;
  } rasp;
  struct DistL0 {
    bool on = false;
    bool ghost_rhs = true;
    int n1 = 0;
    CsrDev A;
    CsrDev P;
    CsrDev PT;
    dbuf<double> wdinv, b, xa, r, x1;
  } dl0;
  bool gp_allgather = false;
  int gp_maxcnt = 0;
  dbuf<int> gp_send_idx;
  dbuf<int> gp_src_idx;
  dbuf<double> gp_sendbuf, gp_recvbuf;
  dbuf<double> pcw;
  double *h_big = nullptr;
  size_t h_big_n = 0;
  std::vector<unsigned char> hL_pbc;
  int hL_singular = -1;
  bool pc_valid = false;
  int pc_its_ref = 0;
  int steps_since_refresh = 0;
  int singular = 0;

  int nnbr = 0;
  std::vector<int> nbr_rank;
  std::vector<long long> send_ptr, recv_ptr;
  dbuf<int> send_idx;
  dbuf<double> send_buf;
  std::vector<double> h_send, h_recv;
  int rank = 0, nranks = 1;
  double nvo_global = 0;
  void *nccl_comm = nullptr;
  cfdh_allreduce_fn cb_ar = nullptr;
  cfdh_exchange_fn cb_ex = nullptr;
  void *cb_user = nullptr;

  bool prof_on = false;
  ProfSlot prof[12];
  std::vector<hipEvent_t> ev_pool;
  struct EvRec { int kind; hipEvent_t a, b; };
  std::vector<EvRec> ev_pending;
  size_t ev_next = 0;

  cfdh_stats last_stats;
  long long n_allreduce = 0, n_halo = 0, n_host_sync = 0, n_krylov = 0, n_allgather = 0;
  long long n_attainable_stops = 0;
  long long n_pc_builds = 0;

  bool pcd_set = false, pcd_ready = false;
  int pcd_in = -1, pcd_out = -1, pcd_time = 0;
  double pcd_ct = 0;
  dbuf<int> pcd_iptr, pcd_inc, pcd_fptr, pcd_fac;
  dbuf<unsigned> pcd_islot, pcd_fslot;
  dbuf<int> pcd_sptr, pcd_scol, pcd_rlen;
  dbuf<double> pcd_K, pcd_mdinv, pcd_t, pcd_q;
  dbuf<float> pcd_Kf;
  dbuf<unsigned char> pcd_flag;
  std::vector<double> h_pcd_md;
  int ew_version = 0;
  double ew_rtol0 = 0.3, ew_rtol_max = 0.9, ew_gamma = 1.0, ew_alpha = 1.6180339887498949, ew_threshold = 0.1;
  std::vector<double> hist_fnorm, hist_rtol, hist_relres;
  std::vector<int> hist_its;
  double ksp_last_relres = 0;
  bool lean = true;
  struct SolveEnv {
    int krylov_fp32 = 1;
    bool guess_check = false;
    bool no_attainable_stop = false;
    int gs_refine_from = -1;
    int ksp_lag = KRING - 3;
    double gs_eta2 = 1e-6;
    int l_cycles = 1, a_cycles = 1;
  } env;
  dbuf<double> qu;
  long long n_guess_projections = 0;
  int guess_last_rank = -1, guess_last_k = 0;
  long long n_iter_sync = 0;
  long long n_cycles = 0;
};

#define CFDH_MAX_PBND 8

int cfdh_fail(cfdh_ctx *c, int code, const char *fmt, ...);
#define HIPCHK(c, call)                                                                           \
  do {                                                                                            \
    hipError_t e_ = (call);                                                                       \
    if (e_ != hipSuccess) return cfdh_fail((c), CFDH_E_HIP, "%s: %s (%s:%d)", #call, hipGetErrorString(e_), \
                                           __FILE__, __LINE__);                                   \
  } while (0)
#define CHK(call)            \
  do {                       \
    int r_ = (call);         \
    if (r_ != 0) return r_;  \
  } while (0)

int cfdh_build_mesh(cfdh_ctx *c, int64_t nv, int64_t nvo, int64_t nc, const int32_t *cells, const double *coords,
                    int64_t nfac, const int32_t *fcell, const int32_t *flocal, const int32_t *fmarker);
int cfdh_amg_setup(cfdh_ctx *c, AmgHier &H, const CsrHost &A, bool singular, int ncol);
int cfdh_level_setup(cfdh_ctx *c, AmgLevel &L, const CsrHost &A, double ratio, int ncol, std::vector<double> *w_out = nullptr);
int cfdh_upload_csr(cfdh_ctx *c, const CsrHost &H, CsrDev &D, const std::vector<double> *colw = nullptr, int parts = CFDH_UP_CSR | CFDH_UP_SELL);
int cfdh_aggregate_host_csr(const CsrHost &A, double theta, std::vector<int> &agg);

bool cfdh_amg_dev_enabled(const cfdh_ctx *c);
int cfdh_amg_setup_dev(cfdh_ctx *c, AmgHier &H, CsrDev &A0, bool singular, int ncol);
int cfdh_level_setup_dev(cfdh_ctx *c, AmgLevel &L, CsrDev &A, double ratio, int ncol);
int cfdh_proxy_dev(cfdh_ctx *c, CsrDev &out);
int cfdh_proxy_ras_dev(cfdh_ctx *c, CsrDev &out);
int cfdh_cc_h_dev(cfdh_ctx *c, double alpha, double beta, CsrDev &out);

#define CFDH3_MAX_SLOTS 320
int cfdh_build_mesh3(cfdh_ctx *c, int64_t nv, int64_t nvo, int64_t nc, const int32_t *cells, const double *coords,
                     int64_t nfac, const int32_t *fcell, const int32_t *flocal, const int32_t *fmarker);
int k3_upload_quadrature(cfdh_ctx *c);
int k3_moments(cfdh_ctx *c);
int k3_assemble(cfdh_ctx *c, const double *xstate, int mode);
int k3_spmv_full(cfdh_ctx *c, const double *x, double *y);
int k3_spmv_full_multi(cfdh_ctx *c, const double *X, double *Y, int ld, int nvec);
int k3_spmv_block(cfdh_ctx *c, int blk, const double *x, double *y, const double *b);
int k3_spmv_block_ghost(cfdh_ctx *c, int blk, const double *xv, double *y, const double *b);
int k3_nullspace_test(cfdh_ctx *c, double *nrm, double *absnrm);
int k3_functional(cfdh_ctx *c, int kind, int marker, double *out);
int k3_wss(cfdh_ctx *c, double *out);

int kg_upload_tables(cfdh_ctx *c);
int cfdh_build_mesh_gen(cfdh_ctx *c, int etype, int64_t nv, int64_t nv_owned, int64_t nc, const int32_t *cells, const double *coords, int64_t nfac,
                        const int32_t *fcell, const int32_t *flocal, const int32_t *fmarker);
int cfdh_gen_element_stiffness(const cfdh_ctx *c, const int32_t *v, const double *X, double *K);
int cfdh_facet_nodes(const cfdh_ctx *c, int f, int out[3]);
int kg_assemble(cfdh_ctx *c, const double *xstate, int mode);
int kg_functional_partials(cfdh_ctx *c, int kind, int marker, int nb);
int kg_wss(cfdh_ctx *c, double *out);

int kg3_upload_tables(cfdh_ctx *c);
int cfdh_build_mesh_gen3(cfdh_ctx *c, int etype, int64_t nv, int64_t nv_owned, int64_t nc, const int32_t *cells, const double *coords, int64_t nfac,
                         const int32_t *fcell, const int32_t *flocal, const int32_t *fmarker);
int cfdh_gen3_element_stiffness(const cfdh_ctx *c, const int32_t *v, const double *X, double *K);
int cfdh_facet_nodes3(const cfdh_ctx *c, int f, int out[8]);
int kg3_assemble(cfdh_ctx *c, const double *xstate, int mode);
int kg3_functional_partials(cfdh_ctx *c, int kind, int marker, int nb);
int kg3_wss(cfdh_ctx *c, double *out);

int cfdh_pcd_supported(cfdh_ctx *c, const char *who);
int cfdh_pcd_setup(cfdh_ctx *c);
int k_pcd_assemble(cfdh_ctx *c, const double *xstate);
int k_pcd_apply(cfdh_ctx *c, const double *r, double *s);

void prof_begin(cfdh_ctx *c, int kind);
void prof_end(cfdh_ctx *c, int kind);
void prof_flush(cfdh_ctx *c);

int k_upload_quadrature(cfdh_ctx *c);
int k_halo_pack(cfdh_ctx *c, const double *vec);
int v_pointwise_mult(cfdh_ctx *c, int n, const double *a, const double *b, double *out);
int k_moments(cfdh_ctx *c);
int k_assemble(cfdh_ctx *c, const double *xstate, int mode);
int k_spmv_full(cfdh_ctx *c, const double *x, double *y);
int k_spmv_full_multi(cfdh_ctx *c, const double *X, double *Y, int ld, int nvec);
int k_spmv_block(cfdh_ctx *c, int blk, const double *x, double *y, const double *b, double alpha);
int k_spmv_block_ghost(cfdh_ctx *c, int blk, const double *xv, double *y, const double *b);
int k_extract_diag(cfdh_ctx *c);
int k_cheb_a00(cfdh_ctx *c, const double *b, double *x);
int k_cheb_a00_coeffs(cfdh_ctx *c);
int k_csr_spmv(cfdh_ctx *c, const CsrDev &A, const double *x, double *y, int mode, const double *b);
int k_csr_spmv_ncol(cfdh_ctx *c, const CsrDev &A, const double *x, double *y, int mode, const double *b, int ncol);
int k_amg_vcycle(cfdh_ctx *c, AmgHier &H, const double *b, double *x);
int k_level_smooth(cfdh_ctx *c, AmgLevel *L, const double *b, double *x, int degree);
bool k_cc_cheb2_scale(cfdh_ctx *c, AmgLevel *L, const double *b, double *x, const double *ml, double *y);
int k_cc_scale(cfdh_ctx *c, int n, const double *ml, const double *z, double *y);
int k_dl0_down(cfdh_ctx *c, const double *halo_vec);
int k_dl0_up(cfdh_ctx *c, double *out);
int k_ext_pack(cfdh_ctx *c, const double *vec, double *out);
int k_scatter_global(cfdh_ctx *c, int n, const int *l2g, const double *loc, double *glob);
int k_gather_global(cfdh_ctx *c, int n, const int *l2g, const double *glob, double *loc);
int k_cc_combine(cfdh_ctx *c, int n, double alpha, double beta, const double *t, const double *z, const double *r, const unsigned char *pbc, double *out, double *out2 = nullptr);
int k_nullspace_test(cfdh_ctx *c, double *nrm, double *absnrm);
int k_spmv_a01_keep(cfdh_ctx *c, const double *x, double *y, const double *b, double *q);
int k_spmv_full_kept(cfdh_ctx *c, const double *x, double *y, const double *q);
int k_resid_norm(cfdh_ctx *c, const double *x, const double *b, double *r, double *nrm, bool *done);
int k_fnorm_nulltest(cfdh_ctx *c, int n, const double *F, double *fn, double *nrm, double *absnrm);
int v_guess_combine(cfdh_ctx *c, int n, const double *U, const double *W, int ld, int k, const double *hd, const double *b, double *x, double *r);
int v_guess_read(cfdh_ctx *c, int k, double *beta, bool *used, int *rank, double *y);
int v_scale_inv_lean(cfdh_ctx *c, int n, double *x);
int v_lincomb_keep(cfdh_ctx *c, int n, const double *Z, int ld, int nvec, const double *y_dev, double *x, double *x2);
int v_norm2_triple(cfdh_ctx *c, int n, const double *a, const double *b, const double *cc, double *out);
int k_bc_scatter(cfdh_ctx *c, int n, int ncomp, const int *idx, const unsigned char *flag, const double *val, const double *mult);

int v_copy(cfdh_ctx *c, int n, const double *x, double *y);
int v_zero(cfdh_ctx *c, int n, double *y);
int v_axpy(cfdh_ctx *c, int n, double a, const double *x, double *y);
int v_waxpy(cfdh_ctx *c, int n, double a, const double *x, const double *y, double *w);
int v_scale(cfdh_ctx *c, int n, double a, double *x);
int v_dot(cfdh_ctx *c, int n, const double *x, const double *y, double *out_host);
int v_norm2(cfdh_ctx *c, int n, const double *x, double *out_host);
int v_norminf_diff(cfdh_ctx *c, int n, const double *x, const double *y, double *out_host);
int v_sub_mean(cfdh_ctx *c, int n, double *p);
int v_multidot(cfdh_ctx *c, int n, const double *V, int ld, int nvec, const double *w, double *h_dev, bool with_ww, double *mirror = nullptr,
               bool reduce_ranks = true);
int v_scale_to(cfdh_ctx *c, int n, double a, const double *x, double *y);
int v_multidot32(cfdh_ctx *c, int n, const float *V, int ld, int nvec, const double *w, double *h_dev, double *mirror);
int v_gs_update32(cfdh_ctx *c, int n, const float *V, int ld, int nvec, const double *h_dev, const double *w, double *vn, float *v32n,
                  double *s_dev, double *mirror);
int v_store32(cfdh_ctx *c, int n, const double *v, float *v32);
int v_gram(cfdh_ctx *c, int n, const double *W, int ld, int k, const double *b, double *out_dev);
int v_multiaxpy(cfdh_ctx *c, int n, const double *V, int ld, int nvec, const double *h_dev, double *w);
int v_gs_update_normalize(cfdh_ctx *c, int n, const double *V, int ld, int nvec, const double *h_dev, const double *w, double *vn, double *s_dev);
int v_norm_to_dev(cfdh_ctx *c, int n, const double *w, double *out_dev);
int v_norm_to_dev_local(cfdh_ctx *c, int n, const double *w, double *out_dev);
int v_scale_inv_dev(cfdh_ctx *c, int n, const double *w, const double *nrm_dev, double *v);
int v_lincomb(cfdh_ctx *c, int n, const double *Z, int ld, int nvec, const double *y_dev, double *x);
int v_pack_state(cfdh_ctx *c, const double *u_user, const double *p_user, double *dst);
int k_functional(cfdh_ctx *c, int kind, int marker, double *out);
int k_wss(cfdh_ctx *c, double *out);

int comm_allreduce_dev(cfdh_ctx *c, double *dev, int n, int op);
int comm_allgather_dev(cfdh_ctx *c, const double *send, double *recv, int count);
int comm_halo(cfdh_ctx *c, double *vec);
int comm_finalize(cfdh_ctx *c);

int cfdh_pc_update(cfdh_ctx *c, bool force_refresh);
int cfdh_pc_apply(cfdh_ctx *c, const double *r, double *z);
int cfdh_apply_operator_dev(cfdh_ctx *c, const double *r, double *z);
int cfdh_host_threads();
int cfdh_fgmres(cfdh_ctx *c, const double *b, double *x, int *its, int *reason, double bnorm = -1.0);
int v_norm2_pair(cfdh_ctx *c, int n, const double *x, const double *y, double *nx, double *ny);
int cfdh_newton_step(cfdh_ctx *c, cfdh_stats *st);
int cfdh_download_blocks(cfdh_ctx *c, std::vector<double> &a00, std::vector<double> &a01, std::vector<double> &a10,
                         std::vector<double> &a11);
```

### cfd_hemodynamic_amd/csrc/cfdh_kernels.hip

```cpp
#include <hip/hip_runtime.h>

#include <cmath>

#include "cfdh_internal.hpp"
#include "cfdh_krylov_host.hpp"
#include "cfdh_quad_tri.h"

#define TPB 256
#define NTLOAD(p) __builtin_nontemporal_load(p)

__constant__ double d_qw[CFDH_NQ];
__constant__ double d_ql[CFDH_NQ][3];

int k_upload_quadrature(cfdh_ctx *c) {
  HIPCHK(c, hipMemcpyToSymbol(HIP_SYMBOL(d_qw), CFDH_QW, sizeof(CFDH_QW)));
  HIPCHK(c, hipMemcpyToSymbol(HIP_SYMBOL(d_ql), CFDH_QL, sizeof(CFDH_QL)));
  return 0;
}

void prof_begin(cfdh_ctx *c, int kind) {
  if (!c->prof_on || c->capturing) return;
  if (c->ev_next + 2 > c->ev_pool.size()) {
    for (int i = 0; i < 64; i++) { hipEvent_t e; if (hipEventCreate(&e) != hipSuccess) return; c->ev_pool.push_back(e); }
  }
  cfdh_ctx::EvRec r;
  r.kind = kind; r.a = c->ev_pool[c->ev_next++]; r.b = c->ev_pool[c->ev_next++];
  (void)hipEventRecord(r.a, c->stream);
  c->ev_pending.push_back(r);
}
void prof_end(cfdh_ctx *c, int kind) {
  if (!c->prof_on || c->capturing || c->ev_pending.empty()) return;
  (void)kind;
  (void)hipEventRecord(c->ev_pending.back().b, c->stream);
  if (c->ev_pending.size() >= 4096) prof_flush(c);
}
void prof_flush(cfdh_ctx *c) {
  if (c->ev_pending.empty()) return;
  (void)hipStreamSynchronize(c->stream);
  for (auto &r : c->ev_pending) {
    float ms = 0;
    if (hipEventElapsedTime(&ms, r.a, r.b) == hipSuccess) { c->prof[r.kind].total_ms += ms; c->prof[r.kind].launches++; }
  }
  c->ev_pending.clear();
  c->ev_next = 0;
}

#include "cfdh_wave.hpp"

__device__ __forceinline__ int uoff(int w, int nvo) { return w < nvo ? 2 * w : 3 * w; }
__device__ __forceinline__ int poff(int w, int nvo) { return w < nvo ? 2 * nvo + w : 3 * w + 2; }

__global__ __launch_bounds__(TPB) void moments_kernel(int nc, int nvo, const int *__restrict__ cells,
                                                      const double *__restrict__ coords,
                                                      const double *__restrict__ un, double *__restrict__ mom,
                                                      double dt, double nu) {
  int e = blockIdx.x * TPB + threadIdx.x;
  if (e >= nc) return;
  int v0 = cells[3 * e], v1 = cells[3 * e + 1], v2 = cells[3 * e + 2];
  double2 X0 = *(const double2 *)(coords + 2 * v0), X1 = *(const double2 *)(coords + 2 * v1), X2 = *(const double2 *)(coords + 2 * v2);
  double u0x = un[uoff(v0, nvo)], u0y = un[uoff(v0, nvo) + 1];
  double u1x = un[uoff(v1, nvo)], u1y = un[uoff(v1, nvo) + 1];
  double u2x = un[uoff(v2, nvo)], u2y = un[uoff(v2, nvo) + 1];
  double det = (X1.x - X0.x) * (X2.y - X0.y) - (X1.y - X0.y) * (X2.x - X0.x);
  double area = 0.5 * fabs(det);
  double d01 = hypot(X0.x - X1.x, X0.y - X1.y), d12 = hypot(X1.x - X2.x, X1.y - X2.y), d20 = hypot(X2.x - X0.x, X2.y - X0.y);
  double h = fmax(d01, fmax(d12, d20));
  double ih2 = 1.0 / (h * h);
  double t2 = 4.0 / (dt * dt), t3 = 16.0 * nu * nu * ih2 * ih2;
  double hr = h / (2.0 * nu);
  double m00 = 0, m01 = 0, m02 = 0, m11 = 0, m12 = 0, m22 = 0, L = 0;
#pragma unroll 7
  for (int q = 0; q < CFDH_NQ; q++) {
    double l0 = d_ql[q][0], l1 = d_ql[q][1], l2 = d_ql[q][2], wq = d_qw[q];
    double ux = l0 * u0x + l1 * u1x + l2 * u2x;
    double uy = l0 * u0y + l1 * u1y + l2 * u2y;
    double s = ux * ux + uy * uy;
    double t1 = fmax(4.0 * s, 1e-30) * ih2;
    double tau = cfdh_rsqrt(t1 + t2 + t3);
    double vn = s > 1e-280 ? s * cfdh_rsqrt(s) : 0.0;
    double Re = vn * hr;
    double z = (Re <= 3.0) ? Re * (1.0 / 3.0) : 1.0;
    double tl = vn * h * z * 0.5;
    double w = wq * tau;
    m00 += w * l0 * l0; m01 += w * l0 * l1; m02 += w * l0 * l2;
    m11 += w * l1 * l1; m12 += w * l1 * l2; m22 += w * l2 * l2;
    L += wq * tl;
  }
  double4 *o = (double4 *)(mom + 8 * (size_t)e);
// ... 1190 lines not shown
  const int p0 = sptr[sl], w = (sptr[sl + 1] - p0) >> 6;
  T a = vzero((const T *)nullptr);
#pragma unroll 4
  for (int k = 0; k < w; k++) {
    const int p = p0 + k * 64 + lane;
    a = vfma((double)sval[p], xin[scol[p]], a);
  }
  xout[row] = vadd(xin[row], vscale(wdinv[row], vsub(b[row], a)));
}

template <typename T>
static int amg_cycle_jacobi(cfdh_ctx *c, AmgHier &H, size_t lev, const T *b, T *x, int prof) {
  AmgLevel *L = H.lev[lev];
  if (lev + 1 == H.lev.size()) {
    if (H.coarse_n > 0) {
      hipLaunchKernelGGL((dense_mv_kernel<T>), dim3(H.coarse_n), dim3(64), 0, c->stream, H.coarse_n, H.coarse_inv.p, b, x);
    } else {
      const int n = L->n;
      dim3 block(TPB), gridC((unsigned)((8ll * n + TPB - 1) / TPB));
      T *xa = (T *)L->d0.p, *r = (T *)L->r.p;
      hipLaunchKernelGGL((jacobi_pre_kernel<T>), gridC, block, 0, c->stream, n, L->A.rowptr.p, L->A.col.p, L->A.val.p,
                         L->wdinv.p, b, xa, r);
      hipLaunchKernelGGL((jacobi_post_kernel<T>), gridC, block, 0, c->stream, n, L->A.rowptr.p, L->A.col.p, L->A.val.p,
                         L->wdinv.p, b, (const T *)xa, x);
    }
    HIPCHK(c, hipGetLastError());
    return 0;
  }
  AmgLevel *N = H.lev[lev + 1];
  const int n = L->n;
  const bool sell = L->A.nnz <= 12ll * n && n >= 16384;
  dim3 block(TPB), gridS((unsigned)((n + TPB - 1) / TPB)), gridC((unsigned)((8ll * n + TPB - 1) / TPB));
  T *xa = (T *)L->d0.p, *x1 = (T *)L->d1.p, *r = (T *)L->r.p;
  if (prof && lev == 0) prof_begin(c, prof);
  if (sell)
    hipLaunchKernelGGL((sell_jacobi_pre_kernel<T>), gridS, block, 0, c->stream, n, L->A.sptr.p, L->A.scol.p, L->A.svalw.p,
                       L->wdinv.p, b, xa, r);
  else
    hipLaunchKernelGGL((jacobi_pre_kernel<T>), gridC, block, 0, c->stream, n, L->A.rowptr.p, L->A.col.p, L->A.val.p,
                       L->wdinv.p, b, xa, r);
  if (prof && lev == 0) prof_end(c, prof);
  CHK(csr_spmv_t<T>(c, L->R, r, (T *)N->b.p, 0, (const T *)nullptr));
  CHK(amg_cycle_jacobi<T>(c, H, lev + 1, (const T *)N->b.p, (T *)N->x.p, prof));
  if (sell)
    hipLaunchKernelGGL((sell_spmv_kernel<3, T>), gridS, block, 0, c->stream, n, L->P.sptr.p, L->P.scol.p, L->P.sval.p,
                       (const T *)N->x.p, x1, (const T *)xa);
  else
    CHK(csr_spmv_t<T>(c, L->P, (const T *)N->x.p, x1, 3, xa));
  if (prof && lev == 0) prof_begin(c, prof);
  if (sell)
    hipLaunchKernelGGL((sell_jacobi_post_kernel<T>), gridS, block, 0, c->stream, n, L->A.sptr.p, L->A.scol.p, L->A.sval.p,
                       L->wdinv.p, b, x1, x);
  else
    hipLaunchKernelGGL((jacobi_post_kernel<T>), gridC, block, 0, c->stream, n, L->A.rowptr.p, L->A.col.p, L->A.val.p,
                       L->wdinv.p, b, x1, x);
  if (prof && lev == 0) prof_end(c, prof);
  HIPCHK(c, hipGetLastError());
  return 0;
}

template <int LPR>
__device__ __forceinline__ double lpr_sum(double v) {
  v = group8_sum(v);
  if (LPR >= 16) v += dpp_shuffle<0x140>(v);
  if (LPR >= 32) v += __shfl_xor(v, 16);
  if (LPR >= 64) v += __shfl_xor(v, 32);
  return v;
}
template <int LPR> __device__ __forceinline__ double lsum(double v) { return lpr_sum<LPR>(v); }
template <int LPR> __device__ __forceinline__ double2 lsum(double2 v) { return make_double2(lpr_sum<LPR>(v.x), lpr_sum<LPR>(v.y)); }
template <int LPR> __device__ __forceinline__ d3 lsum(d3 v) { return d3{lpr_sum<LPR>(v.x), lpr_sum<LPR>(v.y), lpr_sum<LPR>(v.z)}; }

__device__ __forceinline__ double epi_apply(double acc, int row, double alpha, double beta, const double *zH, const double *r, const unsigned char *pbc) {
  return (pbc[row] & 1) ? r[row] : alpha * acc + beta * zH[row];
}
__device__ __forceinline__ double2 epi_apply(double2 acc, int, double, double, const double *, const double *, const unsigned char *) { return acc; }
__device__ __forceinline__ double epi_value(double acc, unsigned flag, double alpha, double beta, double zh, double r) { return (flag & 1u) ? r : alpha * acc + beta * zh; }
__device__ __forceinline__ double2 epi_value(double2 acc, unsigned, double, double, double, double) { return acc; }
__device__ __forceinline__ d3 epi_apply(d3 acc, int, double, double, const double *, const double *, const unsigned char *) { return acc; }
__device__ __forceinline__ d3 epi_value(d3 acc, unsigned, double, double, double, double) { return acc; }

template <int LPR, typename VT, typename T>
__global__ __launch_bounds__(TPB) void fused_down_kernel(int n, const int *__restrict__ rowptr, const int *__restrict__ col,
                                                         const VT *__restrict__ val, const T *__restrict__ x, T *__restrict__ y) {
  const int gid = blockIdx.x * TPB + threadIdx.x;
  const int row = gid / LPR, l = gid % LPR;
  T a = vzero((const T *)nullptr);
  if (row < n) {
    const int ks = rowptr[row], ke = rowptr[row + 1];
    int cidx[4];
    VT cval[4];
#pragma unroll
    for (int q = 0; q < 4; q++) { const int k = ks + l + q * LPR; if (k < ke) { cidx[q] = col[k]; cval[q] = val[k]; } }
    T g[4];
#pragma unroll
    for (int q = 0; q < 4; q++) { const int k = ks + l + q * LPR; if (k < ke) g[q] = x[cidx[q]]; }
#pragma unroll
    for (int q = 0; q < 4; q++) { const int k = ks + l + q * LPR; if (k < ke) a = vfma((double)cval[q], g[q], a); }
    for (int k = ks + l + 4 * LPR; k < ke; k += LPR) a = vfma((double)val[k], x[col[k]], a);
  }
  a = lsum<LPR>(a);
  if (row < n && l == 0) y[row] = a;
}
template <typename T>
__global__ __launch_bounds__(TPB) void fused_up_csr_kernel(int n, const int *__restrict__ rpB, const int *__restrict__ clB,
                                                           const double *__restrict__ vlB, const T *__restrict__ b,
                                                           const int *__restrict__ rpC, const int *__restrict__ clC,
                                                           const double *__restrict__ vlC, const T *__restrict__ xc,
                                                           T *__restrict__ x, double ea, double eb, const double *__restrict__ ezH,
                                                           const double *__restrict__ er, const unsigned char *__restrict__ epbc) {
  const int gid = blockIdx.x * TPB + threadIdx.x;
  const int row = gid >> 3, l = gid & 7;
  T a = vzero((const T *)nullptr);
  if (row < n) {
    const int kb = rpB[row] + l, keB = rpB[row + 1];
    int kc = 0, keC = 0;
    if (rpC) { kc = rpC[row] + l; keC = rpC[row + 1]; }
    int cb[2], cc[2];
    double vb[2], vc[2];
#pragma unroll
    for (int q = 0; q < 2; q++) {
      if (kb + 8 * q < keB) { cb[q] = clB[kb + 8 * q]; vb[q] = vlB[kb + 8 * q]; }
      if (kc + 8 * q < keC) { cc[q] = clC[kc + 8 * q]; vc[q] = vlC[kc + 8 * q]; }
    }
    T gb[2], gc[2];
#pragma unroll
    for (int q = 0; q < 2; q++) {
      if (kb + 8 * q < keB) gb[q] = b[cb[q]];
      if (kc + 8 * q < keC) gc[q] = xc[cc[q]];
    }
#pragma unroll
    for (int q = 0; q < 2; q++) {
      if (kb + 8 * q < keB) a = vfma(vb[q], gb[q], a);
      if (kc + 8 * q < keC) a = vfma(vc[q], gc[q], a);
    }
    for (int k = kb + 16; k < keB; k += 8) a = vfma(vlB[k], b[clB[k]], a);
    for (int k = kc + 16; k < keC; k += 8) a = vfma(vlC[k], xc[clC[k]], a);
  }
  a = g8(a);
  if (row < n && l == 0) x[row] = epbc ? epi_apply(a, row, ea, eb, ezH, er, epbc) : a;
}
template <typename T, bool WIDE>
__global__ __launch_bounds__(TPB) void fused_up_sell_kernel(int n, const int *__restrict__ spB, const int *__restrict__ scB,
                                                            const float *__restrict__ svB, const T *__restrict__ b,
                                                            const int *__restrict__ spC, const int *__restrict__ scC,
                                                            const float *__restrict__ svC, const T *__restrict__ xc,
                                                            T *__restrict__ x, double ea, double eb, const double *__restrict__ ezH,
                                                            const double *__restrict__ er, const unsigned char *__restrict__ epbc) {
  const int row = blockIdx.x * TPB + threadIdx.x;
  if (row >= n) return;
  const int sl = __builtin_amdgcn_readfirstlane(row >> 6), lane = row & 63;
  T a = vzero((const T *)nullptr);
  double e_zh = 0.0, e_r = 0.0;
  unsigned e_f = 0;
  if (epbc) { e_f = epbc[row]; e_zh = ezH[row]; e_r = er[row]; }
  constexpr int MW = sizeof(T) > 8 ? 8 : 10;
  const int pB = spB[sl], wB = (spB[sl + 1] - pB) >> 6;
  int pC = 0, wC = 0;
  if (spC) { pC = spC[sl]; wC = (spC[sl + 1] - pC) >> 6; }
  const int wmax = wB > wC ? wB : wC;
  for (int k0 = 0; k0 < (WIDE ? wmax : 1); k0 += MW) {
    int cB[MW], cC[MW];
    float vB[MW], vC[MW];
#pragma unroll
    for (int k = 0; k < MW; k++) if (k0 + k < wB) { const int p = pB + (k0 + k) * 64 + lane; cB[k] = NTLOAD(scB + p); vB[k] = NTLOAD(svB + p); }
#pragma unroll
    for (int k = 0; k < MW; k++) if (k0 + k < wC) { const int p = pC + (k0 + k) * 64 + lane; cC[k] = NTLOAD(scC + p); vC[k] = NTLOAD(svC + p); }
    T gB[MW], gC[MW];
#pragma unroll
    for (int k = 0; k < MW; k++) if (k0 + k < wB) gB[k] = b[cB[k]];
#pragma unroll
    for (int k = 0; k < MW; k++) if (k0 + k < wC) gC[k] = xc[cC[k]];
#pragma unroll
    for (int k = 0; k < MW; k++) if (k0 + k < wB) a = vfma((double)vB[k], gB[k], a);
#pragma unroll
    for (int k = 0; k < MW; k++) if (k0 + k < wC) a = vfma((double)vC[k], gC[k], a);
  }
  if (!WIDE) {
    for (int k = MW; k < wB; k++) { const int p = pB + k * 64 + lane; a = vfma((double)svB[p], b[scB[p]], a); }
    for (int k = MW; k < wC; k++) { const int p = pC + k * 64 + lane; a = vfma((double)svC[p], xc[scC[p]], a); }
  }
  x[row] = epbc ? epi_value(a, e_f, ea, eb, e_zh, e_r) : a;
}
template <typename T>
__global__ __launch_bounds__(TPB) void fused_up_dense_kernel(int n, const int *__restrict__ rpB, const int *__restrict__ clB,
                                                             const double *__restrict__ vlB, const T *__restrict__ b,
                                                             const float *__restrict__ D, int nc, const T *__restrict__ bc,
                                                             T *__restrict__ x) {
  const int gid = blockIdx.x * TPB + threadIdx.x;
  const int row = gid >> 6, l = gid & 63;
  T a = vzero((const T *)nullptr);
  if (row < n) {
    for (int k = rpB[row] + l, ke = rpB[row + 1]; k < ke; k += 64) a = vfma(vlB[k], b[clB[k]], a);
    const float *Dr = D + (size_t)row * nc;
    float dv[12];
    T bv[12];
#pragma unroll
    for (int q = 0; q < 12; q++) { const int j = l + 64 * q; if (j < nc) { dv[q] = Dr[j]; bv[q] = bc[j]; } }
#pragma unroll
    for (int q = 0; q < 12; q++) { const int j = l + 64 * q; if (j < nc) a = vfma((double)dv[q], bv[q], a); }
    for (int j = l + 768; j < nc; j += 64) a = vfma((double)Dr[j], bc[j], a);
  }
  a = wsum(a);
  if (row < n && l == 0) x[row] = a;
}

template <typename VT, typename T>
static void launch_down(cfdh_ctx *c, const CsrDev &G, const VT *val, const T *x, T *y) {
  const long long avg = G.n > 0 ? (G.nnz + G.n - 1) / G.n : 1;
  const int lpr = avg > 96 ? 64 : (avg > 48 ? 32 : (avg > 20 ? 16 : 8));
  dim3 block(TPB), grid((unsigned)(((long long)G.n * lpr + TPB - 1) / TPB));
  if (lpr == 64) hipLaunchKernelGGL((fused_down_kernel<64, VT, T>), grid, block, 0, c->stream, G.n, G.rowptr.p, G.col.p, val, x, y);
  else if (lpr == 32) hipLaunchKernelGGL((fused_down_kernel<32, VT, T>), grid, block, 0, c->stream, G.n, G.rowptr.p, G.col.p, val, x, y);
  else if (lpr == 16) hipLaunchKernelGGL((fused_down_kernel<16, VT, T>), grid, block, 0, c->stream, G.n, G.rowptr.p, G.col.p, val, x, y);
  else hipLaunchKernelGGL((fused_down_kernel<8, VT, T>), grid, block, 0, c->stream, G.n, G.rowptr.p, G.col.p, val, x, y);
}

template <typename T>
static int amg_cycle_fused(cfdh_ctx *c, AmgHier &H, const T *b, T *x, int prof, int l0 = 0) {
  const int nl = (int)H.lev.size();
  for (int l = l0; l + 1 < nl; l++) {
    AmgLevel *L = H.lev[l], *N = H.lev[l + 1];
    const T *src = l == l0 ? b : (const T *)L->b.p;
    if (prof && l == 0) prof_begin(c, prof + 4);
    if (L->fine) launch_down<float, T>(c, L->G, L->G.valf.p, src, (T *)N->b.p);
    else launch_down<double, T>(c, L->G, L->G.val.p, src, (T *)N->b.p);
    if (prof && l == 0) prof_end(c, prof + 4);
  }
  int l = nl - 1;
  {
    AmgLevel *L = H.lev[l];
    const T *bl = l == l0 ? b : (const T *)L->b.p;
    T *xl = l == l0 ? x : (T *)L->x.p;
    if (nl - 2 >= l0 && H.lev[nl - 2]->Dn > 0) {
      AmgLevel *U = H.lev[nl - 2];
      const T *bu = nl - 2 == l0 ? b : (const T *)U->b.p;
      T *xu = nl - 2 == l0 ? x : (T *)U->x.p;
      const int un = (nl - 2 == 0 && c->up0_rows > 0 && c->up0_rows < U->n) ? c->up0_rows : U->n;
      hipLaunchKernelGGL((fused_up_dense_kernel<T>), dim3((unsigned)((64ll * un + TPB - 1) / TPB)), dim3(TPB), 0, c->stream, un,
                         U->Sb.rowptr.p, U->Sb.col.p, U->Sb.val.p, bu, U->D.p, U->Dn, bl, xu);
      l = nl - 3;
    } else {
      if (H.coarse_n > 0)
        hipLaunchKernelGGL((dense_mv_kernel<T>), dim3(H.coarse_n), dim3(64), 0, c->stream, H.coarse_n, H.coarse_inv.p, bl, xl);
      else if (L->sell)
        hipLaunchKernelGGL((fused_up_sell_kernel<T, true>), dim3((unsigned)((L->n + TPB - 1) / TPB)), dim3(TPB), 0, c->stream, L->n,
                           L->Sb.sptr.p, L->Sb.scol.p, L->Sb.sval.p, bl, (const int *)nullptr, (const int *)nullptr,
                           (const float *)nullptr, (const T *)nullptr, xl, 0.0, 0.0, (const double *)nullptr, (const double *)nullptr,
                           (const unsigned char *)nullptr);
      else
        hipLaunchKernelGGL((fused_up_csr_kernel<T>), dim3((unsigned)((8ll * L->n + TPB - 1) / TPB)), dim3(TPB), 0, c->stream, L->n,
                           L->Sb.rowptr.p, L->Sb.col.p, L->Sb.val.p, bl, (const int *)nullptr, (const int *)nullptr,
                           (const double *)nullptr, (const T *)nullptr, xl, 0.0, 0.0, (const double *)nullptr, (const double *)nullptr,
                           (const unsigned char *)nullptr);
      l = nl - 2;
    }
  }
  for (; l >= l0; l--) {
    AmgLevel *L = H.lev[l], *N = H.lev[l + 1];
    const T *bl = l == l0 ? b : (const T *)L->b.p;
    T *xl = l == l0 ? x : (T *)L->x.p;
    const bool epi = l == 0 && c->epi.on && sizeof(T) == sizeof(double);
    const double ea = epi ? c->epi.alpha : 0.0, eb = epi ? c->epi.beta : 0.0;
    const double *ezH = epi ? c->epi.zH : nullptr, *er = epi ? c->epi.r : nullptr;
    const unsigned char *epbc = epi ? c->epi.pbc : nullptr;
    if (epi) { xl = (T *)c->epi.out; c->epi.done = true; }
    const int nrow = (l == 0 && c->up0_rows > 0 && c->up0_rows < L->n) ? c->up0_rows : L->n;
    if (prof && l == 0) prof_begin(c, prof);
    if (L->sell && L->Sb.sell_maxw <= 14 && L->Sc.sell_maxw <= 14)
      hipLaunchKernelGGL((fused_up_sell_kernel<T, false>), dim3((unsigned)((nrow + TPB - 1) / TPB)), dim3(TPB), 0, c->stream, nrow,
                         L->Sb.sptr.p, L->Sb.scol.p, L->Sb.sval.p, bl, L->Sc.sptr.p, L->Sc.scol.p, L->Sc.sval.p, (const T *)N->x.p, xl,
                         ea, eb, ezH, er, epbc);
    else if (L->sell)
      hipLaunchKernelGGL((fused_up_sell_kernel<T, true>), dim3((unsigned)((nrow + TPB - 1) / TPB)), dim3(TPB), 0, c->stream, nrow,
                         L->Sb.sptr.p, L->Sb.scol.p, L->Sb.sval.p, bl, L->Sc.sptr.p, L->Sc.scol.p, L->Sc.sval.p, (const T *)N->x.p, xl,
                         ea, eb, ezH, er, epbc);
    else
      hipLaunchKernelGGL((fused_up_csr_kernel<T>), dim3((unsigned)((8ll * nrow + TPB - 1) / TPB)), dim3(TPB), 0, c->stream, nrow,
                         L->Sb.rowptr.p, L->Sb.col.p, L->Sb.val.p, bl, L->Sc.rowptr.p, L->Sc.col.p, L->Sc.val.p, (const T *)N->x.p, xl,
                         ea, eb, ezH, er, epbc);
    if (prof && l == 0) prof_end(c, prof);
  }
  HIPCHK(c, hipGetLastError());
  return 0;
}

static int amg_cycle_cheb(cfdh_ctx *c, AmgHier &H, size_t lev, const double *b, double *x, bool prof) {
  AmgLevel *L = H.lev[lev];
  if (lev + 1 == H.lev.size()) {
    if (H.coarse_n > 0) {
      hipLaunchKernelGGL((dense_mv_kernel<double>), dim3(H.coarse_n), dim3(64), 0, c->stream, H.coarse_n, H.coarse_inv.p, b, x);
      HIPCHK(c, hipGetLastError());
      return 0;
    }
    return level_cheb(c, L, b, x, true, c->opt.amg_smooth_degree > 2 ? c->opt.amg_smooth_degree : 2, false);
  }
  AmgLevel *N = H.lev[lev + 1];
  const int deg = c->opt.amg_smooth_degree;
  CHK(level_cheb(c, L, b, x, true, deg, prof && lev == 0));
  CHK(k_csr_spmv(c, L->A, x, L->r.p, 1, b));
  CHK(k_csr_spmv(c, L->R, L->r.p, N->b.p, 0, nullptr));
  CHK(amg_cycle_cheb(c, H, lev + 1, N->b.p, N->x.p, prof));
  CHK(k_csr_spmv(c, L->P, N->x.p, x, 2, nullptr));
  CHK(level_cheb(c, L, b, x, false, deg, prof && lev == 0));
  return 0;
}

__global__ __launch_bounds__(TPB) void dl0_pack_kernel(int nvo, int nv, int dim, const double *__restrict__ vec, const double *__restrict__ wdinv,
                                                       double *__restrict__ b, double *__restrict__ xa, int ghosts) {
  const int i = blockIdx.x * TPB + threadIdx.x;
  if (i >= nv) return;
  const double v = i < nvo ? vec[(size_t)dim * nvo + i] : (ghosts ? vec[((size_t)dim + 1) * nvo + ((size_t)dim + 1) * (size_t)(i - nvo) + dim] : 0.0);
  b[i] = v;
  xa[i] = wdinv[i] * v;
}
int k_dl0_down(cfdh_ctx *c, const double *halo_vec) {
  cfdh_ctx::DistL0 &d = c->dl0;
  AmgLevel *N = c->hLg.lev[1];
  const int nvo = c->nvo, nv = c->nv;
  if (d.ghost_rhs) hipLaunchKernelGGL(dl0_pack_kernel, dim3((nv + TPB - 1) / TPB), dim3(TPB), 0, c->stream, nvo, nv, c->dim, halo_vec, d.wdinv.p, d.b.p, d.xa.p, 1);
  dim3 block(TPB), grid((unsigned)((8ll * nvo + TPB - 1) / TPB)), gridS((unsigned)((nvo + TPB - 1) / TPB));
  if (d.A.nnz <= 12ll * nvo && nvo >= 16384)
    hipLaunchKernelGGL((sell_jacobi_pre_kernel<double>), gridS, block, 0, c->stream, nvo, d.A.sptr.p, d.A.scol.p, d.A.svalw.p,
                       d.wdinv.p, (const double *)d.b.p, d.xa.p, d.r.p);
  else
    hipLaunchKernelGGL((jacobi_pre_kernel<double>), grid, block, 0, c->stream, nvo, d.A.rowptr.p, d.A.col.p, d.A.val.p, d.wdinv.p,
                       (const double *)d.b.p, d.xa.p, d.r.p);
  HIPCHK(c, hipGetLastError());
  return csr_spmv_t<double>(c, d.PT, d.r.p, N->b.p, 0, (const double *)nullptr);
}
int k_dl0_up(cfdh_ctx *c, double *out) {
  cfdh_ctx::DistL0 &d = c->dl0;
  AmgLevel *N = c->hLg.lev[1];
  const int nvo = c->nvo;
  static const bool sweeps = getenv("CFDH_DL0_COARSE_SWEEPS") && getenv("CFDH_DL0_COARSE_SWEEPS")[0] == '1';
  if (c->hLg.fused && c->opt.amg_smooth_degree == 1 && !sweeps) CHK(amg_cycle_fused<double>(c, c->hLg, (const double *)N->b.p, N->x.p, 0, 1));
  else CHK(amg_cycle_jacobi<double>(c, c->hLg, 1, (const double *)N->b.p, N->x.p, 0));
  if (d.P.nnz <= 12ll * c->nv && c->nv >= 16384)
    hipLaunchKernelGGL((sell_spmv_kernel<3, double>), dim3((unsigned)((c->nv + TPB - 1) / TPB)), dim3(TPB), 0, c->stream, c->nv,
                       d.P.sptr.p, d.P.scol.p, d.P.sval.p, (const double *)N->x.p, d.x1.p, (const double *)d.xa.p);
  else
    CHK(csr_spmv_t<double>(c, d.P, (const double *)N->x.p, d.x1.p, 3, (const double *)d.xa.p));
  dim3 block(TPB), grid((unsigned)((8ll * nvo + TPB - 1) / TPB)), gridS((unsigned)((nvo + TPB - 1) / TPB));
  if (d.A.nnz <= 12ll * nvo && nvo >= 16384)
    hipLaunchKernelGGL((sell_jacobi_post_kernel<double>), gridS, block, 0, c->stream, nvo, d.A.sptr.p, d.A.scol.p, d.A.sval.p,
                       d.wdinv.p, (const double *)d.b.p, (const double *)d.x1.p, out);
  else
    hipLaunchKernelGGL((jacobi_post_kernel<double>), grid, block, 0, c->stream, nvo, d.A.rowptr.p, d.A.col.p, d.A.val.p, d.wdinv.p,
                       (const double *)d.b.p, (const double *)d.x1.p, out);
  HIPCHK(c, hipGetLastError());
  return 0;
}

int k_amg_vcycle(cfdh_ctx *c, AmgHier &H, const double *b, double *x) {
  if (!H.valid || H.lev.empty()) return cfdh_fail(c, CFDH_E_STATE, "AMG hierarchy not built");
  const bool prof = (&H == &c->hS) || (&H == &c->hL) || (&H == &c->hLg);
  if (H.ncol == 3) {
    if (H.fused && c->opt.amg_smooth_degree == 1 && H.lev.size() >= 2) return amg_cycle_fused<d3>(c, H, (const d3 *)b, (d3 *)x, 5);
    return amg_cycle_jacobi<d3>(c, H, 0, (const d3 *)b, (d3 *)x, 5);
  }
  if (H.fused && c->opt.amg_smooth_degree == 1 && H.lev.size() >= 2) {
    if (H.ncol == 2) return amg_cycle_fused<double2>(c, H, (const double2 *)b, (double2 *)x, 5);
    return amg_cycle_fused<double>(c, H, b, x, prof ? 4 : 0);
// ... 540 lines not shown
  }
  hipLaunchKernelGGL(scale_store32_kernel, dim3(vgrid(n)), dim3(TPB), 0, c->stream, n, vn, (const double *)s_dev, v32n);
  HIPCHK(c, hipGetLastError());
  return 0;
}
int v_lincomb(cfdh_ctx *c, int n, const double *Z, int ld, int nvec, const double *y_dev, double *x) {
  hipLaunchKernelGGL(multiaxpy_kernel, dim3(vgrid(n)), dim3(TPB), 0, c->stream, n, Z, (size_t)ld, nvec, y_dev, x, 1.0);
  HIPCHK(c, hipGetLastError());
  return 0;
}

__global__ void gram_solve_kernel(int k, const double *__restrict__ hd, double *__restrict__ y, double *__restrict__ info) {
  if (threadIdx.x != 0 || blockIdx.x != 0) return;
  int r = 0;
  const bool used = cfdh_krylov::gram_solve(k, hd, y, &r);
  for (int i = 0; i < k; i++) info[3 + i] = y[i];
  info[1] = used ? 1.0 : 0.0;
  info[2] = (double)r;
}
__global__ __launch_bounds__(TPB) void guess_combine_kernel(int n, const double *__restrict__ U, const double *__restrict__ W, size_t ld,
                                                            int nvec, const double *__restrict__ y, const double *__restrict__ b,
                                                            double *__restrict__ x, double *__restrict__ r, double *__restrict__ partial) {
  __shared__ double sh[4];
  double ss = 0.0;
  for (int i = blockIdx.x * TPB + threadIdx.x; i < n; i += gridDim.x * TPB) {
    double a0 = 0.0, a1 = 0.0, a2 = 0.0, a3 = 0.0, c0 = b[i], c1 = 0.0, c2 = 0.0, c3 = 0.0;
    int v = 0;
    for (; v + 4 <= nvec; v += 4) {
      const double y0 = y[v], y1 = y[v + 1], y2 = y[v + 2], y3 = y[v + 3];
      const double u0 = U[(size_t)v * ld + i], u1 = U[(size_t)(v + 1) * ld + i], u2 = U[(size_t)(v + 2) * ld + i], u3 = U[(size_t)(v + 3) * ld + i];
      const double w0 = W[(size_t)v * ld + i], w1 = W[(size_t)(v + 1) * ld + i], w2 = W[(size_t)(v + 2) * ld + i], w3 = W[(size_t)(v + 3) * ld + i];
      a0 += y0 * u0; a1 += y1 * u1; a2 += y2 * u2; a3 += y3 * u3;
      c0 -= y0 * w0; c1 -= y1 * w1; c2 -= y2 * w2; c3 -= y3 * w3;
    }
    for (; v < nvec; v++) { a0 += y[v] * U[(size_t)v * ld + i]; c0 -= y[v] * W[(size_t)v * ld + i]; }
    const double ri = (c0 + c1) + (c2 + c3);
    x[i] = (a0 + a1) + (a2 + a3);
    r[i] = ri;
    ss += ri * ri;
  }
  ss = block_sum(ss, sh);
  if (threadIdx.x == 0) partial[blockIdx.x] = ss;
}
__global__ __launch_bounds__(TPB) void scale_inv_sqrt_kernel(int n, double *__restrict__ x, const double *__restrict__ s2) {
  const double beta = sqrt(s2[0]);
  const double a = beta > 0.0 ? 1.0 / beta : 0.0;
  for (int i = blockIdx.x * TPB + threadIdx.x; i < n; i += gridDim.x * TPB) x[i] *= a;
}
__global__ __launch_bounds__(TPB) void lincomb_keep_kernel(int n, const double *__restrict__ V, size_t ld, int nvec,
                                                           const double *__restrict__ h, double *__restrict__ w, double *__restrict__ w2) {
  for (int i = blockIdx.x * TPB + threadIdx.x; i < n; i += gridDim.x * TPB) {
    double a0 = w[i], a1 = 0.0, a2 = 0.0, a3 = 0.0;
    int v = 0;
    for (; v + 4 <= nvec; v += 4) {
      const double x0 = V[(size_t)v * ld + i], x1 = V[(size_t)(v + 1) * ld + i], x2 = V[(size_t)(v + 2) * ld + i],
                   x3 = V[(size_t)(v + 3) * ld + i];
      a0 += h[v] * x0; a1 += h[v + 1] * x1; a2 += h[v + 2] * x2; a3 += h[v + 3] * x3;
    }
    for (; v < nvec; v++) a0 += h[v] * V[(size_t)v * ld + i];
    const double o = (a0 + a1) + (a2 + a3);
    w[i] = o;
    w2[i] = o;
  }
}
__global__ __launch_bounds__(TPB) void norm3_partial_kernel(int n, const double *__restrict__ a, const double *__restrict__ b,
                                                            const double *__restrict__ cc, double *__restrict__ partial) {
  __shared__ double sh[4];
  double s0 = 0, s1 = 0, s2 = 0;
  for (int i = blockIdx.x * TPB + threadIdx.x; i < n; i += gridDim.x * TPB) {
    const double ai = a[i], bi = b[i], ci = cc[i];
    s0 += ai * ai; s1 += bi * bi; s2 += ci * ci;
  }
  s0 = block_sum(s0, sh);
  s1 = block_sum(s1, sh);
  s2 = block_sum(s2, sh);
  if (threadIdx.x == 0) { partial[blockIdx.x] = s0; partial[gridDim.x + blockIdx.x] = s1; partial[2 * gridDim.x + blockIdx.x] = s2; }
}
static double *lean_mirror(cfdh_ctx *c) { c->mirror_src = nullptr; return c->h_pinned_dev + CFDH_MIRROR_OFF; }
static int lean_sync(cfdh_ctx *c) {
  c->n_host_sync++;
  HIPCHK(c, hipStreamSynchronize(c->stream));
  return 0;
}
#define CFDH_LEAN_S2 12
int v_guess_combine(cfdh_ctx *c, int n, const double *U, const double *W, int ld, int k, const double *hd, const double *b, double *x, double *r) {
  if (k < 1 || k > 8) return cfdh_fail(c, CFDH_E_STATE, "projected guess: %d kept vectors", k);
  const int nb = vgrid(n) > c->red_blocks ? c->red_blocks : vgrid(n);
  double *mir = lean_mirror(c);
  hipLaunchKernelGGL(gram_solve_kernel, dim3(1), dim3(64), 0, c->stream, k, hd, c->ky.p, mir);
  hipLaunchKernelGGL(guess_combine_kernel, dim3(nb), dim3(TPB), 0, c->stream, n, U, W, (size_t)ld, k, (const double *)c->ky.p, b, x, r, c->red_partial.p);
  hipLaunchKernelGGL(reduce_final_kernel<0>, dim3(1), dim3(TPB), 0, c->stream, nb, nb, c->red_partial.p, c->red_out.p + CFDH_LEAN_S2, mir);
  HIPCHK(c, hipGetLastError());
  return 0;
}
int v_guess_read(cfdh_ctx *c, int k, double *beta, bool *used, int *rank, double *y) {
  CHK(lean_sync(c));
  const double *m = c->h_pinned + CFDH_MIRROR_OFF;
  *beta = sqrt(m[0]);
  *used = m[1] != 0.0;
  *rank = (int)m[2];
  for (int i = 0; i < k; i++) y[i] = m[3 + i];
  return 0;
}
int v_scale_inv_lean(cfdh_ctx *c, int n, double *x) {
  hipLaunchKernelGGL(scale_inv_sqrt_kernel, dim3(vgrid(n)), dim3(TPB), 0, c->stream, n, x, (const double *)(c->red_out.p + CFDH_LEAN_S2));
  HIPCHK(c, hipGetLastError());
  return 0;
}
int k_resid_norm(cfdh_ctx *c, const double *x, const double *b, double *r, double *nrm, bool *done) {
  const long long nthreads = 8ll * c->nvo;
  const long long nb = (nthreads + TPB - 1) / TPB;
  *done = false;
  if (c->dim != 2 || (size_t)nb > c->red_partial.n) return 0;
  double *mir = lean_mirror(c);
  hipLaunchKernelGGL((spmv_full_lean_kernel<false, true>), dim3((unsigned)nb), dim3(TPB), 0, c->stream, c->nvo, c->vptr.p, c->vcol.p, c->A00.p,
                     c->A01.p, c->A10.p, c->A11.p, x, r, (const double *)nullptr, b, c->red_partial.p);
  hipLaunchKernelGGL(reduce_final_kernel<0>, dim3(1), dim3(TPB), 0, c->stream, (int)nb, (int)nb, c->red_partial.p, c->red_out.p + CFDH_LEAN_S2, mir);
  HIPCHK(c, hipGetLastError());
  CHK(lean_sync(c));
  *nrm = sqrt(c->h_pinned[CFDH_MIRROR_OFF]);
  *done = true;
  return 0;
}
int v_lincomb_keep(cfdh_ctx *c, int n, const double *Z, int ld, int nvec, const double *y_dev, double *x, double *x2) {
  hipLaunchKernelGGL(lincomb_keep_kernel, dim3(vgrid(n)), dim3(TPB), 0, c->stream, n, Z, (size_t)ld, nvec, y_dev, x, x2);
  HIPCHK(c, hipGetLastError());
  return 0;
}
int v_norm2_triple(cfdh_ctx *c, int n, const double *a, const double *b, const double *cc, double *out) {
  const int nb = vgrid(n) > c->red_blocks ? c->red_blocks : vgrid(n);
  if ((size_t)3 * nb > c->red_partial.n) return cfdh_fail(c, CFDH_E_STATE, "reduction workspace too small");
  double *mir = lean_mirror(c);
  hipLaunchKernelGGL(norm3_partial_kernel, dim3(nb), dim3(TPB), 0, c->stream, n, a, b, cc, c->red_partial.p);
  hipLaunchKernelGGL(reduce_final_kernel<0>, dim3(3), dim3(TPB), 0, c->stream, nb, nb, c->red_partial.p, c->red_out.p, mir);
  HIPCHK(c, hipGetLastError());
  CHK(lean_sync(c));
  for (int i = 0; i < 3; i++) out[i] = sqrt(c->h_pinned[CFDH_MIRROR_OFF + i]);
  return 0;
}
__global__ void sqrt_kernel(double *s) { s[0] = sqrt(s[0]); }
int v_norm_to_dev(cfdh_ctx *c, int n, const double *w, double *out_dev) {
  CHK(reduce_dev(c, 0, n, w, w, out_dev));
  hipLaunchKernelGGL(sqrt_kernel, dim3(1), dim3(1), 0, c->stream, out_dev);
  HIPCHK(c, hipGetLastError());
  return 0;
}
int v_norm_to_dev_local(cfdh_ctx *c, int n, const double *w, double *out_dev) {
  const int nb = vgrid(n) > c->red_blocks ? c->red_blocks : vgrid(n);
  hipLaunchKernelGGL(reduce_partial_kernel<0>, dim3(nb), dim3(TPB), 0, c->stream, n, w, w, c->red_partial.p);
  hipLaunchKernelGGL(reduce_final_kernel<0>, dim3(1), dim3(TPB), 0, c->stream, nb, nb, c->red_partial.p, out_dev, (double *)nullptr);
  hipLaunchKernelGGL(sqrt_kernel, dim3(1), dim3(1), 0, c->stream, out_dev);
  HIPCHK(c, hipGetLastError());
  return 0;
}
__global__ __launch_bounds__(TPB) void scale_inv_dev_kernel(int n, const double *__restrict__ w, const double *__restrict__ nrm,
                                                            double *__restrict__ v) {
  const double s = nrm[0] != 0.0 ? 1.0 / nrm[0] : 0.0;
  for (int i = blockIdx.x * TPB + threadIdx.x; i < n; i += gridDim.x * TPB) v[i] = w[i] * s;
}
int v_scale_inv_dev(cfdh_ctx *c, int n, const double *w, const double *nrm_dev, double *v) {
  hipLaunchKernelGGL(scale_inv_dev_kernel, dim3(vgrid(n)), dim3(TPB), 0, c->stream, n, w, nrm_dev, v);
  HIPCHK(c, hipGetLastError());
  return 0;
}

__global__ __launch_bounds__(TPB) void nulltest_kernel(int nvo, const int *__restrict__ vptr, const double *__restrict__ A01,
                                                       const double *__restrict__ A11, double *__restrict__ partial) {
  __shared__ double sh[4];
  double a = 0, b = 0;
  for (int row = blockIdx.x * TPB + threadIdx.x; row < nvo; row += gridDim.x * TPB) {
    double s0 = 0, s1 = 0, s2 = 0, t0 = 0, t1 = 0, t2 = 0;
    for (int k = vptr[row]; k < vptr[row + 1]; k++) {
      const double c0 = A01[2 * (size_t)k], c1 = A01[2 * (size_t)k + 1], c2 = A11[k];
      s0 += c0; s1 += c1; s2 += c2;
      t0 += fabs(c0); t1 += fabs(c1); t2 += fabs(c2);
    }
    a += s0 * s0 + s1 * s1 + s2 * s2;
    b += t0 * t0 + t1 * t1 + t2 * t2;
  }
  a = block_sum(a, sh);
  b = block_sum(b, sh);
// ... 263 lines not shown
```

### cfd_hemodynamic_amd/csrc/cfdh_krylov_host.hpp

```cpp
#pragma once
#include <algorithm>
#include <cmath>
#include <vector>

#ifdef __HIPCC__
#define CFDH_HD __host__ __device__
#else
#define CFDH_HD
#endif

namespace cfdh_krylov {

CFDH_HD inline bool gram_solve(int k, const double *hd, double *y, int *rank) {
  double G[64], Lc[64], dg[8], g[8], yy[8], t[8];
  int piv[8];
  bool taken[8];
  for (int i = 0; i < k; i++) {
    for (int q = 0; q < k; q++) { G[q * k + i] = hd[i * 8 + q]; Lc[q * k + i] = 0.0; }
    g[i] = hd[k * 8 + i]; yy[i] = 0.0; taken[i] = false;
  }
  double dmax0 = 0.0;
  bool ok = true;
  for (int i = 0; i < k; i++) {
    dg[i] = G[i * k + i];
    if (!std::isfinite(dg[i])) ok = false;
    if (i == 0 || dg[i] > dmax0) dmax0 = dg[i];
  }
  ok = ok && dmax0 > 0.0 && std::isfinite(dmax0);
  int r = 0;
  if (ok) {
    for (int it = 0; it < k; it++) {
      int p = -1;
      for (int i = 0; i < k; i++) if (!taken[i] && (p < 0 || dg[i] > dg[p])) p = i;
      if (p < 0 || !(dg[p] > 1e-10 * G[p * k + p]) || !(dg[p] > 1e-14 * dmax0)) break;
      taken[p] = true;
      const int rr = r;
      piv[r++] = p;
      const double lpp = std::sqrt(dg[p]);
      Lc[p * k + rr] = lpp;
      for (int i = 0; i < k; i++) {
        if (taken[i]) continue;
        double sacc = G[i * k + p];
        for (int q = 0; q < rr; q++) sacc -= Lc[i * k + q] * Lc[p * k + q];
        Lc[i * k + rr] = sacc / lpp;
        dg[i] -= Lc[i * k + rr] * Lc[i * k + rr];
      }
    }
    for (int a = 0; a < r; a++) {
      double sacc = g[piv[a]];
      for (int q = 0; q < a; q++) sacc -= Lc[piv[a] * k + q] * t[q];
      t[a] = sacc / Lc[piv[a] * k + a];
    }
    for (int a = r - 1; a >= 0; a--) {
      double sacc = t[a];
      for (int q = a + 1; q < r; q++) sacc -= Lc[piv[q] * k + a] * yy[piv[q]];
      yy[piv[a]] = sacc / Lc[piv[a] * k + a];
    }
  }
  bool used = ok && r > 0;
  for (int i = 0; i < k; i++) if (!std::isfinite(yy[i])) used = false;
  for (int i = 0; i < k; i++) y[i] = used ? yy[i] : 0.0;
  *rank = r;
  return used;
}

CFDH_HD inline double gs_scale(double ww, double hh2) {
  const double nrm2 = ww - hh2;
  return (nrm2 > 0.0 && nrm2 <= ww) ? std::sqrt(nrm2) : std::sqrt(ww);
}

struct ArnoldiLsq {
  int m;
  std::vector<double> H, cs, sn, g, y;
  explicit ArnoldiLsq(int m_) : m(m_), H((size_t)(m_ + 1) * m_, 0.0), cs(m_), sn(m_), g(m_ + 1), y(m_) {}
  void start(double beta) {
    std::fill(g.begin(), g.end(), 0.0);
    g[0] = beta;
  }
  bool add_column(int j, const double *h, double hnorm) {
    double *Hj = &H[(size_t)j * (m + 1)];
    for (int i = 0; i <= j; i++) Hj[i] = h[i];
    Hj[j + 1] = hnorm;
    for (int i = 0; i < j; i++) {
      const double t = cs[i] * Hj[i] + sn[i] * Hj[i + 1];
      Hj[i + 1] = -sn[i] * Hj[i] + cs[i] * Hj[i + 1];
      Hj[i] = t;
    }
    const double d = std::hypot(Hj[j], Hj[j + 1]);
    if (!(d > 0) || !std::isfinite(d)) return false;
    cs[j] = Hj[j] / d; sn[j] = Hj[j + 1] / d;
    Hj[j] = d; Hj[j + 1] = 0.0;
    g[j + 1] = -sn[j] * g[j]; g[j] = cs[j] * g[j];
    return true;
  }
  double residual(int j) const { return std::fabs(g[j]); }
  const double *solve(int j) {
    for (int i = j - 1; i >= 0; i--) {
      double s = g[i];
      for (int k = i + 1; k < j; k++) s -= H[(size_t)k * (m + 1) + i] * y[k];
      y[i] = s / H[(size_t)i * (m + 1) + i];
    }
    return y.data();
  }
};

struct LaunchAhead {
  int need = 1;
  double res_hist[4] = {0, 0, 0, 0};
  int nhist = 0;
  int e_its = 0;
  CFDH_HD void start(double beta, int e_its_, int its) {
    e_its = e_its_;
    need = std::max(1, std::min(e_its - its - 2, 3));
    res_hist[0] = beta; res_hist[1] = res_hist[2] = res_hist[3] = 0.0;
    nhist = 1;
  }
  CFDH_HD int in_flight(bool sync_now, int lagmax) const {
    return sync_now ? 1 : std::max(1, std::min(need - (need >= 4 ? 1 : 0), lagmax + 1));
  }
  CFDH_HD int process_upto(int j, int jl, int maxl, bool sync_now) const {
    return (!sync_now && jl - j > 1 && jl < maxl && need > jl - j) ? jl - 1 : jl;
  }
  CFDH_HD void observe(double res, double tol, int its) {
    if (nhist < 4) res_hist[nhist++] = res;
    else { res_hist[0] = res_hist[1]; res_hist[1] = res_hist[2]; res_hist[2] = res_hist[3]; res_hist[3] = res; }
    const double rho = std::pow(res / res_hist[0], 1.0 / (nhist - 1));
    int n_rem = (rho > 0.0 && rho < 0.97) ? (int)std::ceil(std::log(tol / res) / std::log(rho)) : (1 << 20);
    if (nhist == 2) n_rem = std::min(n_rem, 3);
    need = std::max(1, e_its > 0 ? std::min(n_rem, std::max(e_its - its, 1) + 2) : n_rem);
  }
};

}
```

### cfd_hemodynamic_amd/csrc/cfdh_setup.cpp

```cpp
#include <algorithm>
#include <chrono>
#include <cmath>
#include <cstdarg>
#include <cstdlib>
#include <numeric>

#include "cfdh_internal.hpp"

int cfdh_fail(cfdh_ctx *c, int code, const char *fmt, ...) {
  char buf[512];
  va_list ap;
  va_start(ap, fmt);
  vsnprintf(buf, sizeof buf, fmt, ap);
  va_end(ap);
  extern std::string g_cfdh_last_error;
  g_cfdh_last_error = buf;
  if (c) c->err = buf;
  return code;
}

int cfdh_host_threads() {
  const char *e = getenv("CFDH_HOST_THREADS");
  int n = e ? atoi(e) : 8;
  return n < 1 ? 1 : (n > 64 ? 64 : n);
// ... 653 lines not shown
      CsrHost RA, G, Sb, Sc, Dg;
      spgemm_host(R, A, RA);
      csr_axpby_scaled(RA, -1.0, nullptr, curW.data(), R, G);
      Dg.n = Dg.m = A.n; Dg.rowptr.resize(A.n + 1); Dg.col.resize(A.n); Dg.val.resize(A.n);
      for (int i = 0; i < A.n; i++) { Dg.rowptr[i] = i; Dg.col[i] = i; Dg.val[i] = 2.0 * curW[i]; }
      Dg.rowptr[A.n] = A.n;
      csr_axpby_scaled(A, -1.0, curW.data(), curW.data(), Dg, Sb);
      csr_axpby_scaled(AP, -1.0, curW.data(), nullptr, P, Sc);
      spgemm_host(RA, P, Ac);
      TICK(3);
      const int fmt = L->fine ? CFDH_UP_CSRF : CFDH_UP_CSR;
      CHK(upload_csr(c, G, L->G, nullptr, fmt));
      CHK(upload_csr(c, Sb, L->Sb, nullptr, L->sell ? CFDH_UP_SELL : CFDH_UP_CSR));
      CHK(upload_csr(c, Sc, L->Sc, nullptr, L->sell ? CFDH_UP_SELL : CFDH_UP_CSR));
      if (H.lev.size() == 1) { H.nnz_G0 = G.nnz(); H.nnz_S0 = (long long)Sb.nnz() + Sc.nnz(); }
      TICK(4);
      lastSc.n = Sc.n; lastSc.m = Sc.m; lastSc.rowptr.swap(Sc.rowptr); lastSc.col.swap(Sc.col); lastSc.val.swap(Sc.val);
    } else {
      spgemm_host(R, AP, Ac);
      TICK(3);
    }
    A.n = Ac.n; A.m = Ac.m;
    A.rowptr.swap(Ac.rowptr); A.col.swap(Ac.col); A.val.swap(Ac.val);
  }
  H.coarse_n = 0;
  if (A.n > 2500) {
    if (want_fused) {
      AmgLevel *L = H.lev.back();
      CsrHost Sb, Dg;
      Dg.n = Dg.m = A.n; Dg.rowptr.resize(A.n + 1); Dg.col.resize(A.n); Dg.val.resize(A.n);
      for (int i = 0; i < A.n; i++) { Dg.rowptr[i] = i; Dg.col[i] = i; Dg.val[i] = 2.0 * curW[i]; }
      Dg.rowptr[A.n] = A.n;
      csr_axpby_scaled(A, -1.0, curW.data(), curW.data(), Dg, Sb);
      CHK(upload_csr(c, Sb, L->Sb, nullptr, L->sell ? CFDH_UP_SELL : CFDH_UP_CSR));
      H.fused = H.lev.size() >= 1;
    }
    H.valid = true;
    H.fine_nnz = A0.nnz();
    HIPCHK(c, hipStreamSynchronize(c->stream));
    if (c->opt.verbose) {
      fprintf(stderr, "[cfdh] AMG hierarchy (ncol %d, smoothed coarsest level%s):", ncol, H.fused ? ", fused" : "");
      for (AmgLevel *l : H.lev) fprintf(stderr, " (%d, nnz %d; G %d Sb %d Sc %d)", l->n, l->A.nnz, l->G.nnz, l->Sb.nnz, l->Sc.nnz);
      fprintf(stderr, "\n");
    }
    return 0;
  }
  {
    int n = A.n;
    std::vector<double> D((size_t)n * n, 0.0);
    double tr = 0;
    for (int i = 0; i < n; i++)
      for (int k = A.rowptr[i]; k < A.rowptr[i + 1]; k++) { D[(size_t)i * n + A.col[k]] = A.val[k]; if (A.col[k] == i) tr += std::fabs(A.val[k]); }
    if (singular) {
      double alpha = tr / n / n;
      for (size_t k = 0; k < D.size(); k++) D[k] += alpha;
    }
    if (!dense_inverse(D, n)) return cfdh_fail(c, CFDH_E_STATE, "singular coarsest AMG operator (n=%d)", n);
    HIPCHK(c, H.coarse_inv.upload(D, c->stream));
    H.coarse_n = n;
    if (want_fused && H.lev.size() >= 2) {
      H.fused = true;
      AmgLevel *U = H.lev[H.lev.size() - 2];
      const long long ent = (long long)lastSc.n * n;
      U->Dn = 0;
      if (lastSc.m == n && ent <= 8000000ll && !U->sell) {
        std::vector<float> Df((size_t)ent);
#pragma omp parallel for schedule(static) num_threads(cfdh_host_threads())
        for (int i = 0; i < lastSc.n; i++) {
          std::vector<double> acc(n, 0.0);
          for (int k = lastSc.rowptr[i]; k < lastSc.rowptr[i + 1]; k++) {
            const double s = lastSc.val[k];
            const double *row = &D[(size_t)lastSc.col[k] * n];
            for (int j = 0; j < n; j++) acc[j] += s * row[j];
          }
          for (int j = 0; j < n; j++) Df[(size_t)i * n + j] = (float)acc[j];
        }
        HIPCHK(c, U->D.upload(Df, c->stream));
        HIPCHK(c, hipStreamSynchronize(c->stream));
        U->Dn = n;
      }
    }
  }
  H.fine_nnz = A0.nnz();
  H.valid = true;
  HIPCHK(c, hipStreamSynchronize(c->stream));
  if (c->opt.verbose) {
    fprintf(stderr, "[cfdh] AMG hierarchy (ncol %d%s):", ncol, H.fused ? ", fused" : "");
    for (AmgLevel *l : H.lev) fprintf(stderr, " (%d, nnz %d; G %d Sb %d Sc %d D %d)", l->n, l->A.nnz, l->G.nnz, l->Sb.nnz, l->Sc.nnz, l->Dn);
    TICK(5);
    fprintf(stderr, "\n[cfdh]   host set-up ms: levels %.0f, aggregation %.0f, prolongator %.0f, products %.0f, uploads %.0f, dense %.0f\n", tm[0], tm[1],
            tm[2], tm[3], tm[4], tm[5]);
  }
#undef TICK
  return 0;
}
```

### cfd_hemodynamic_amd/csrc/cfdh_solver.cpp

```cpp
#include <algorithm>
#include <chrono>
#include <cmath>

#include "cfdh_internal.hpp"
#include "cfdh_krylov_host.hpp"

int cfdh_host_threads();

static double wall_ms() {
  using namespace std::chrono;
  return duration<double, std::milli>(steady_clock::now().time_since_epoch()).count();
}

int cfdh_download_blocks(cfdh_ctx *c, std::vector<double> &a00, std::vector<double> &a01, std::vector<double> &a10,
                         std::vector<double> &a11) {
  const size_t nz = (size_t)c->nnzv, d = (size_t)c->dim;
  a00.resize(d * d * nz); a01.resize(d * nz); a10.resize(d * nz); a11.resize(nz);
  HIPCHK(c, hipMemcpyAsync(a00.data(), c->A00.p, sizeof(double) * d * d * nz, hipMemcpyDeviceToHost, c->stream));
  HIPCHK(c, hipMemcpyAsync(a01.data(), c->A01.p, sizeof(double) * d * nz, hipMemcpyDeviceToHost, c->stream));
  HIPCHK(c, hipMemcpyAsync(a10.data(), c->A10.p, sizeof(double) * d * nz, hipMemcpyDeviceToHost, c->stream));
  HIPCHK(c, hipMemcpyAsync(a11.data(), c->A11.p, sizeof(double) * nz, hipMemcpyDeviceToHost, c->stream));
  HIPCHK(c, hipStreamSynchronize(c->stream));
  return 0;
}
// ... 642 lines not shown

static int pc_exchange(cfdh_ctx *c, int stage) {
  if (c->nranks <= 1 || c->opt.pc_type != 1) return 0;
  const bool dist = c->gp_n > 0 && c->dl0.on;
  int ls = stage;
  if (dist) ls = stage <= 1 ? stage : (stage == 2 ? 10 : stage - 1);
  switch (ls) {
    case 0: return c->opt.schur_full == 2 ? 0 : comm_halo(c, c->pcw.p);
    case 1:
      if (c->gp_n <= 0) return 0;
      if (dist) return c->dl0.ghost_rhs ? comm_halo(c, c->pcw.p) : 0;
      if (c->gp_allgather) return comm_allgather_dev(c, c->gp_sendbuf.p, c->gp_recvbuf.p, c->gp_maxcnt);
      return comm_allreduce_dev(c, c->gp_rhs.p, c->gp_n, 0);
    case 10: return comm_allreduce_dev(c, c->hLg.lev[1]->b.p, c->dl0.n1, 0);
    case 2: return c->opt.schur_full ? comm_halo(c, c->pcw.p) : 0;
    case 3: return (c->ras && c->opt.schur_full && ras_ghost_rhs()) ? comm_halo(c, c->pcw.p) : 0;
    default: return 0;
  }
}

int cfdh_pc_apply(cfdh_ctx *c, const double *r, double *z) {
  const int nvo = c->nvo;
  const bool graph = c->use_graph && !c->prof_on;
  const bool multi = c->nranks > 1 && c->opt.pc_type == 1;
  if (multi && !c->pcw.p) { HIPCHK(c, c->pcw.alloc(c->NL)); HIPCHK(c, c->pcw.zero(c->stream)); }
  if (lean_scope(c) && c->opt.schur_full != 0 && !c->qu.p) {
    HIPCHK(c, c->qu.alloc(2 * (size_t)c->nvo));
    c->pc_graph_valid = false;
  }
  if (!graph) {
    for (int st = 0; st < 6; st++) { CHK(pc_stage(c, r, z, st)); CHK(pc_exchange(c, st)); }
  } else {
    if (!c->pc_graph_valid) {
      for (auto &e : c->pc_graphs) for (auto &x : e.exec) if (x) (void)hipGraphExecDestroy(x);
      c->pc_graphs.clear();
      c->pc_graph_valid = true;
    }
    cfdh_ctx::PcGraph *pg = nullptr;
    for (auto &e : c->pc_graphs) if (e.r == r && e.z == z) { pg = &e; break; }
    if (!pg) {
      cfdh_ctx::PcGraph ng{r, z, {nullptr, nullptr, nullptr, nullptr, nullptr, nullptr}};
      for (int gidx = 0; gidx < (multi ? 6 : 1); gidx++) {
        hipGraph_t g = nullptr;
        HIPCHK(c, hipStreamBeginCapture(c->stream, hipStreamCaptureModeThreadLocal));
        c->capturing = true;
        int rc = 0;
        if (multi) rc = pc_stage(c, r, z, gidx);
        else for (int st = 0; st < 6 && !rc; st++) rc = pc_stage(c, r, z, st);
        c->capturing = false;
        hipError_t e = hipStreamEndCapture(c->stream, &g);
        if (rc) return rc;
        if (e != hipSuccess || !g) return cfdh_fail(c, CFDH_E_HIP, "hipStreamEndCapture: %s", hipGetErrorString(e));
        e = hipGraphInstantiate(&ng.exec[gidx], g, nullptr, nullptr, 0);
        (void)hipGraphDestroy(g);
        if (e != hipSuccess) return cfdh_fail(c, CFDH_E_HIP, "hipGraphInstantiate: %s", hipGetErrorString(e));
      }
      c->pc_graphs.push_back(ng);
      pg = &c->pc_graphs.back();
    }
    if (!multi) {
      HIPCHK(c, hipGraphLaunch(pg->exec[0], c->stream));
    } else {
      for (int st = 0; st < 6; st++) { HIPCHK(c, hipGraphLaunch(pg->exec[st], c->stream)); CHK(pc_exchange(c, st)); }
    }
  }
  if (c->singular) CHK(v_sub_mean(c, nvo, z + (size_t)c->dim * nvo));
  return 0;
}

static int pc_then_product(cfdh_ctx *c, const double *r, double *z, double *w) {
  CHK(cfdh_pc_apply(c, r, z));
  CHK(comm_halo(c, z));
  if (lean_keep_qu(c) && !c->prof_on) return k_spmv_full_kept(c, z, w, c->qu.p);
  return k_spmv_full(c, z, w);
}

static size_t krylov_ld(const cfdh_ctx *c) { return ((size_t)c->NL + 1) & ~(size_t)1; }

static int ensure_krylov(cfdh_ctx *c);
int cfdh_apply_operator_dev(cfdh_ctx *c, const double *r, double *z) {
  CHK(ensure_krylov(c));
  return pc_then_product(c, r, z, c->kw.p);
}

static int ensure_krylov(cfdh_ctx *c) {
  const int m = c->opt.ksp_restart;
  if (c->kry_m == m && c->kV.p) return 0;
  const size_t NL = krylov_ld(c);
  c->pc_graph_valid = false;
  HIPCHK(c, c->kV.alloc(NL * (m + 1)));
  HIPCHK(c, c->kZ.alloc(NL * m));
  HIPCHK(c, c->kw.alloc(NL));
  HIPCHK(c, c->kh.alloc(std::max(2 * (size_t)(m + 2) + 8, (size_t)8 * (8 + 1))));
  HIPCHK(c, c->ky.alloc(m + 8));
  if (c->h_ring) { (void)hipHostFree(c->h_ring); c->h_ring = nullptr; }
  c->h_ring_stride = ((size_t)m + 5) & ~(size_t)1;
  HIPCHK(c, hipHostMalloc((void **)&c->h_ring, sizeof(double) * c->h_ring_stride * (cfdh_ctx::KRING + 1)));
  HIPCHK(c, hipHostGetDevicePointer((void **)&c->h_ring_dev, c->h_ring, 0));
  for (auto &e : c->ev_ring) if (!e) HIPCHK(c, hipEventCreateWithFlags(&e, hipEventDisableTiming));
  HIPCHK(c, c->kV.zero(c->stream)); HIPCHK(c, c->kZ.zero(c->stream)); HIPCHK(c, c->kw.zero(c->stream));
  if ((size_t)(m + 2) * 1024 > c->red_partial.n) HIPCHK(c, c->red_partial.alloc((size_t)(m + 2) * 1024 + 1024));
  c->kry_m = m;
  return 0;
}

static int guess_ensure(cfdh_ctx *c) {
  const int m = c->opt.ksp_guess;
  const size_t ld = krylov_ld(c);
  if (m == c->guess_m && (m == 0 || c->guessU.p)) return 0;
  c->guess_m = m;
  for (int k = 0; k < cfdh_ctx::GUESS_NEWTON; k++) c->guess_cnt[k] = c->guess_head[k] = 0;
  if (m > 0) {
    HIPCHK(c, c->guessU.alloc(ld * (size_t)m * cfdh_ctx::GUESS_NEWTON)); HIPCHK(c, c->guessU.zero(c->stream));
    HIPCHK(c, c->guessX.alloc(ld * (size_t)cfdh_ctx::GUESS_NEWTON));
  }
  return 0;
}

static bool guess_ring_valid(const cfdh_ctx *c) {
  return c->guess_m > 0 && c->guess_slot >= 0 && c->guess_slot < cfdh_ctx::GUESS_NEWTON;
}
static int guess_usable(const cfdh_ctx *c) {
  return (guess_ring_valid(c) && c->kry_m >= c->guess_m + 1) ? c->guess_cnt[c->guess_slot] : 0;
}
static int guess_expected_its(const cfdh_ctx *c) {
  return (c->guess_slot >= 0 && c->guess_slot < cfdh_ctx::GUESS_NEWTON) ? c->guess_last_its[c->guess_slot] : 0;
}

static int guess_project(cfdh_ctx *c, const double *b, double *x, bool *used) {
  *used = false;
  CHK(guess_ensure(c));
  const int k = guess_usable(c), n = c->NO;
  if (k == 0) return 0;
  const size_t ld = krylov_ld(c);
  double *U = c->guessU.p + ld * (size_t)c->guess_m * c->guess_slot;
  double *V = c->kV.p, *Z = c->kZ.p, *hd = c->kh.p;
  if (c->nranks > 1) {
    for (int i = 0; i < k; i++) {
      double *t = V + (size_t)(i + 1) * ld;
      CHK(v_copy(c, n, U + (size_t)i * ld, t));
      CHK(comm_halo(c, t));
    }
    CHK(k_spmv_full_multi(c, V + ld, Z, (int)ld, k));
  } else {
    CHK(k_spmv_full_multi(c, U, Z, (int)ld, k));
  }
  HIPCHK(c, hipMemsetAsync(hd, 0, sizeof(double) * 8 * (size_t)(k + 1), c->stream));
  CHK(v_gram(c, n, Z, (int)ld, k, b, hd));
  CHK(comm_allreduce_dev(c, hd, 8 * (k + 1), 0));
  HIPCHK(c, hipMemcpyAsync(c->h_pinned, hd, sizeof(double) * 8 * (size_t)(k + 1), hipMemcpyDeviceToHost, c->stream));
  HIPCHK(c, hipStreamSynchronize(c->stream));
  c->n_host_sync++;
  c->n_guess_projections++;
  double gram[8 * 9];
  std::copy(c->h_pinned, c->h_pinned + 8 * (size_t)(k + 1), gram);
  if (c->opt.verbose > 1) {
    double bb = 0.0;
    CHK(v_norm2(c, n, b, &bb));
    fprintf(stderr, "[cfdh]     guess diag (newton %d): cos(W_i, b) =", c->guess_slot);
    for (int i = 0; i < k; i++) fprintf(stderr, " %.6f", gram[8 * k + i] / (std::sqrt(gram[9 * i]) * bb));
    fprintf(stderr, "; |W_i|/|b| =");
    for (int i = 0; i < k; i++) fprintf(stderr, " %.4f", std::sqrt(gram[9 * i]) / bb);
    fprintf(stderr, "\n");
  }
  double y[8];
  int rank = 0;
// ... 530 lines not shown
```

### include/cfdh.h

```cpp
#ifndef CFDH_H
#define CFDH_H

#include <stdint.h>

#ifdef __cplusplus
extern "C" {
#endif

#define CFDH_ABI_VERSION 1

enum {
  CFDH_OK = 0,
  CFDH_E_ARG = -1,
  CFDH_E_HIP = -2,
  CFDH_E_STATE = -3,
  CFDH_E_DIVERGED = -4,
  CFDH_E_COMM = -5,
  CFDH_E_NOMEM = -6
};

enum {
  CFDH_CONVERGED_FNORM_ABS = 2,
  CFDH_CONVERGED_FNORM_RELATIVE = 3,
  CFDH_CONVERGED_SNORM_RELATIVE = 4,
// ... 7 lines not shown
  CFDH_KSP_CONVERGED_ATTAINABLE = 12,
  CFDH_KSP_DIVERGED_ITS = -3,
  CFDH_KSP_DIVERGED_NANORINF = -9
};

typedef struct cfdh_ctx cfdh_ctx;

typedef struct cfdh_options {
  double snes_rtol, snes_atol, snes_stol;
  int32_t snes_max_it;
  double ksp_rtol, ksp_atol;
  int32_t ksp_max_it, ksp_restart;
  int32_t cheb_degree;
  double cheb_ratio;
  int32_t schur_full;
  int32_t amg_smooth_degree;
  double amg_smooth_ratio;
  double amg_theta;
  int32_t amg_max_coarse;
  int32_t pc_refresh;
  int32_t remove_p_mean;
  int32_t verbose;
  int32_t pc_type;
  int32_t cc_smooth_degree;
  int32_t ksp_guess;
} cfdh_options;

typedef struct cfdh_stats {
  int32_t newton_its, krylov_its, reason, pc_refreshes;
  double fnorm0, fnorm;
  double ms_assemble, ms_solve, ms_pc_setup, ms_total;
} cfdh_stats;


int cfdh_create(cfdh_ctx **out, int device, int gdim, int64_t nv, int64_t nv_owned, int64_t nc,
                const int32_t *cells, const double *coords, int64_t nfacets, const int32_t *facet_cells,
                const int32_t *facet_local, const int32_t *facet_marker);
enum { CFDH_ELEM_P1 = 0, CFDH_ELEM_P2_TRIANGLE = 1, CFDH_ELEM_Q1_QUADRILATERAL = 2, CFDH_ELEM_P1_GENERIC = 3 };
int cfdh_create_elem(cfdh_ctx **out, int device, int gdim, int elem, int64_t nn, int64_t nc, const int32_t *cells,
                     const double *node_coords, int64_t nfacets, const int32_t *facet_cells, const int32_t *facet_local,
                     const int32_t *facet_marker);
int cfdh_create_elem_part(cfdh_ctx **out, int device, int gdim, int elem, int64_t nn, int64_t nn_owned, int64_t nc, const int32_t *cells,
                          const double *node_coords, int64_t nfacets, const int32_t *facet_cells, const int32_t *facet_local,
                          const int32_t *facet_marker);
int cfdh_set_facet_markers(cfdh_ctx *ctx, int64_t nfacets, const int32_t *markers);
void cfdh_destroy(cfdh_ctx *ctx);
const char *cfdh_last_error(const cfdh_ctx *ctx);
int cfdh_abi_version(void);

int cfdh_set_params(cfdh_ctx *ctx, double dt, double rho, double mu, double mu_facet, const double f[3]);
int cfdh_default_options(cfdh_options *opt);
int cfdh_set_options(cfdh_ctx *ctx, const cfdh_options *opt);


int cfdh_clear_dirichlet(cfdh_ctx *ctx);
int cfdh_add_dirichlet(cfdh_ctx *ctx, int field, int64_t n, const int32_t *nodes, const double *values);
int cfdh_update_dirichlet(cfdh_ctx *ctx, int field, int64_t n, const int32_t *nodes, const double *values);


int cfdh_set_state(cfdh_ctx *ctx, const double *u_prev, const double *p_prev, const double *u, const double *p);
int cfdh_get_solution(cfdh_ctx *ctx, double *u, double *p);
int cfdh_get_previous(cfdh_ctx *ctx, double *u_prev, double *p_prev);
int cfdh_get_residual(cfdh_ctx *ctx, double *ru, double *rp);
int cfdh_advance(cfdh_ctx *ctx);
int cfdh_advance_field(cfdh_ctx *ctx, int field);


int cfdh_set_time_scheme(cfdh_ctx *ctx, double theta, double a0, double a1, double a2);

int cfdh_set_boundary_terms(cfdh_ctx *ctx, int ds_terms, int backflow_marker, double beta);


enum { CFDH_FORM_CONVECTIVE = 0, CFDH_FORM_ROTATIONAL = 1 };
int cfdh_set_formulation(cfdh_ctx *ctx, int form);
int cfdh_set_pressure_boundaries(cfdh_ctx *ctx, int n, const int32_t *markers, const double *values, double beta_nitsche);


int cfdh_set_schur_pcd(cfdh_ctx *ctx, int inlet_marker, int outlet_marker, int time_term);
int cfdh_set_ksp_forcing(cfdh_ctx *ctx, int version, double rtol_0, double rtol_max, double gamma, double alpha, double threshold);
int cfdh_get_newton_history(cfdh_ctx *ctx, int32_t *n, double *fnorm, double *ksp_rtol, int32_t *ksp_its, double *ksp_rel_res);
int cfdh_get_pcd_operator(cfdh_ctx *ctx, int64_t *nnz, int32_t *rowptr, int32_t *col, double *vals, double *mass_diag);
int cfdh_apply_preconditioner(cfdh_ctx *ctx, const double *r, double *z);
int cfdh_apply_operator(cfdh_ctx *ctx, const double *r, double *z, double *w);

#define CFDH_AMG_HIER_A 0
#define CFDH_AMG_HIER_P 1
#define CFDH_AMG_HIER_H 2
#define CFDH_AMG_OP_A 0
#define CFDH_AMG_OP_P 1
#define CFDH_AMG_OP_G 2
#define CFDH_AMG_OP_SB 3
#define CFDH_AMG_OP_SC 4
int cfdh_get_amg_operator(cfdh_ctx *ctx, int hier, int level, int which, int64_t *nrow, int64_t *ncol, int64_t *nnz, int32_t *rowptr,
                          int32_t *col, double *vals);
#define CFDH_AMG_VEC_DINV 0
#define CFDH_AMG_VEC_WDINV 1
#define CFDH_AMG_VEC_AGG 2
#define CFDH_AMG_VEC_COARSE_INV 3
#define CFDH_AMG_VEC_D 4
#define CFDH_AMG_VEC_LAMBDA 5
#define CFDH_AMG_VEC_CC_SCALARS 6
#define CFDH_AMG_VEC_CC_ML 7
#define CFDH_AMG_VEC_CC_PBC 8
#define CFDH_AMG_VEC_SPGEMM_ROWS 9
#define CFDH_AMG_VEC_SHAPE 10
#define CFDH_AMG_VEC_ORDER 11
#define CFDH_AMG_VEC_A00_LMAX 12
#define CFDH_AMG_VEC_A00_DINV 13
int cfdh_get_amg_vectors(cfdh_ctx *ctx, int hier, int level, int which, int64_t *n, double *out);


int cfdh_create_ipcs(cfdh_ctx **out, int device, int gdim, int64_t nn, int64_t nvert, int64_t nc, const int32_t *cells,
                     const double *node_coords, int64_t nfacets, const int32_t *facet_cells, const int32_t *facet_local,
                     const int32_t *facet_marker);
int cfdh_ipcs_set_form(cfdh_ctx *ctx, double conv_coeff, double force_coeff);
int cfdh_ipcs_set_tolerances(cfdh_ctx *ctx, const double rtol[3], double atol, const int32_t max_it[3]);
typedef struct cfdh_ipcs_stats {
  int32_t its[3], reason[3];
  double rel_res[3];
  double ms_assemble, ms_solve[3], ms_total;
  int32_t launches, host_syncs;
} cfdh_ipcs_stats;
int cfdh_ipcs_step(cfdh_ctx *ctx, cfdh_ipcs_stats *stats);
int cfdh_ipcs_get_operator(cfdh_ctx *ctx, int which, int64_t *nnz, int32_t *rowptr, int32_t *col, double *vals);
int cfdh_ipcs_get_intermediate(cfdh_ctx *ctx, int which, double *out);
int cfdh_ipcs_apply_pressure_pc(cfdh_ctx *ctx, const double *r, double *z);

int cfdh_set_previous2(cfdh_ctx *ctx, const double *u_prev2);
int cfdh_get_previous2(cfdh_ctx *ctx, double *u_prev2);
int cfdh_shift_history(cfdh_ctx *ctx);


int cfdh_assemble(cfdh_ctx *ctx, int want_jacobian);
int cfdh_get_csr(cfdh_ctx *ctx, int64_t *nnz, int32_t *rowptr, int32_t *col, double *vals);
int cfdh_spmv(cfdh_ctx *ctx, const double *x, double *y);


int cfdh_solve_step(cfdh_ctx *ctx, cfdh_stats *stats);

int cfdh_functional(cfdh_ctx *ctx, int kind, int marker, double *out);

int cfdh_wall_shear_stress(cfdh_ctx *ctx, double *shear);


int cfdh_set_halo(cfdh_ctx *ctx, int nnbr, const int32_t *nbr_rank, const int64_t *send_ptr,
                  const int32_t *send_idx, const int64_t *recv_ptr, const int32_t *recv_idx);
int cfdh_set_global_pressure_space(cfdh_ctx *ctx, int64_t nv_global, int64_t nc_global, const int32_t *cells_global,
                                   const double *coords_global, const int32_t *owned_global, int64_t n_pbc,
                                   const int32_t *pbc_nodes_global);
int cfdh_comm_unique_id(void *id128);
int cfdh_comm_init(cfdh_ctx *ctx, const void *id128, int rank, int nranks);
typedef int (*cfdh_allreduce_fn)(void *user, double *buf, int n, int op);
typedef int (*cfdh_exchange_fn)(void *user, const double *sendbuf, double *recvbuf);
int cfdh_comm_set_callbacks(cfdh_ctx *ctx, cfdh_allreduce_fn ar, cfdh_exchange_fn ex, void *user, int rank, int nranks);


int cfdh_profile_enable(cfdh_ctx *ctx, int on);
int cfdh_profile_get(cfdh_ctx *ctx, int kind, double *total_ms, int64_t *launches);
int cfdh_profile_reset(cfdh_ctx *ctx);
int64_t cfdh_info(const cfdh_ctx *ctx, int what);

#ifdef __cplusplus
}
#endif
#endif
```

Measured before the change: 433.9.

## Pad coarse AMG operators into fixed-slot layout and use LDS Gram solve

At AMG setup, the coarse-level G, Sb and Sc operators get a padded per-lane slot layout (K slots of LPR lanes per row, zero-filled). The fused down and up kernels read their first K entries from that layout without bounds checks and fall back to CSR only for the tail. The goal is more uniform, coalesced loads and fewer divergent branches in the cycle kernels. Separately, the projected-guess Gram solve switches to an LDS-based kernel variant, and a debug API exposes that solve. The cost is extra memory for the padded copies, a setup-time kernel launch plus a host sync per operator, and some redundant zero-valued FMAs.

```diff
diff --git a/cfd_hemodynamic_amd/_lib.py b/cfd_hemodynamic_amd/_lib.py
--- a/cfd_hemodynamic_amd/_lib.py
+++ b/cfd_hemodynamic_amd/_lib.py
@@ -52,6 +52,7 @@
     "cfdh_functional", "cfdh_wall_shear_stress", "cfdh_set_global_pressure_space", "cfdh_set_halo", "cfdh_comm_unique_id", "cfdh_comm_init", "cfdh_comm_set_callbacks",
     "cfdh_profile_enable", "cfdh_profile_get", "cfdh_profile_reset", "cfdh_info",
     "cfdh_set_schur_pcd", "cfdh_set_ksp_forcing", "cfdh_get_newton_history", "cfdh_get_pcd_operator", "cfdh_apply_preconditioner", "cfdh_apply_operator",
+    "cfdh_gram_solve",
     "cfdh_get_amg_operator", "cfdh_get_amg_vectors",
     "cfdh_create_ipcs", "cfdh_ipcs_set_form", "cfdh_ipcs_set_tolerances", "cfdh_ipcs_step", "cfdh_ipcs_get_operator", "cfdh_ipcs_get_intermediate",
     "cfdh_ipcs_apply_pressure_pc",
@@ -131,6 +132,7 @@
     L.cfdh_get_pcd_operator.argtypes = [vp, lp, ip, ip, dp, dp]
     L.cfdh_apply_preconditioner.argtypes = [vp, dp, dp]
     L.cfdh_apply_operator.argtypes = [vp, dp, dp, dp]
+    L.cfdh_gram_solve.argtypes = [vp, C.c_int, dp, dp, ip, ip]
     L.cfdh_get_amg_operator.argtypes = [vp, C.c_int, C.c_int, C.c_int, lp, lp, lp, ip, ip, dp]
     L.cfdh_get_amg_vectors.argtypes = [vp, C.c_int, C.c_int, C.c_int, lp, dp]
     L.cfdh_create_ipcs.argtypes = [C.POINTER(vp), C.c_int, C.c_int, C.c_int64, C.c_int64, C.c_int64, ip, dp, C.c_int64, ip, ip, ip]
@@ -441,6 +443,15 @@
         self._chk(self.L.cfdh_apply_operator(self.h, _dp(r), _dp(z), _dp(w)))
         return z, w
 
+    def gram_solve(self, hd, k):
+        hd = np.ascontiguousarray(hd, dtype=np.float64)
+        if hd.size < 8 * (k + 1):
+            raise ValueError("8 (k + 1) words expected")
+        y = np.zeros(8)
+        rank, used = np.zeros(1, dtype=np.int32), np.zeros(1, dtype=np.int32)
+        self._chk(self.L.cfdh_gram_solve(self.h, int(k), _dp(hd), _dp(y), _ip(rank), _ip(used)))
+        return y[:k].copy(), int(rank[0]), bool(used[0])
+
     def get_amg_operator(self, hier, level, which, raw=False):
         import scipy.sparse as sp
         nr, nc, nnz = C.c_int64(), C.c_int64(), C.c_int64()
diff --git a/cfd_hemodynamic_amd/csrc/cfdh_amg_dev.hip b/cfd_hemodynamic_amd/csrc/cfdh_amg_dev.hip
--- a/cfd_hemodynamic_amd/csrc/cfdh_amg_dev.hip
+++ b/cfd_hemodynamic_amd/csrc/cfdh_amg_dev.hip
@@ -5,6 +5,7 @@
 #include <cmath>
 
 #include "cfdh_internal.hpp"
+#include "cfdh_pad_layout.hpp"
 
 #define TPB 256
 
@@ -977,6 +978,55 @@
 }
 
 int cfdh_aggregate_host_csr(const CsrHost &A, double theta, std::vector<int> &agg);
+
+__global__ __launch_bounds__(TPB) void pad_fill_kernel(int n, int K, int lpr, const int *__restrict__ rowptr, const int *__restrict__ col,
+                                                       const double *__restrict__ val, int *__restrict__ pcol, double *__restrict__ pval,
+                                                       int *__restrict__ cnt ) {
+  const size_t idx = (size_t)blockIdx.x * TPB + threadIdx.x;
+  if (idx >= cfdh_pad::slot_count(n, K, lpr)) return;
+  const int l = (int)(idx % lpr), q = (int)((idx / lpr) % K);
+  const long long r = (long long)(idx / ((size_t)lpr * K));
+  cfdh_pad::fill_slot(rowptr, col, val, r, K, q, lpr, l, pcol, pval);
+  if (l == 0 && q == 0 && cfdh_pad::has_tail(rowptr[r], rowptr[r + 1], K, lpr)) atomicAdd(cnt, 1);
+  if (cfdh_pad::slot_entry(rowptr[r], rowptr[r + 1], q, lpr, l) < 0) atomicAdd(cnt + 1, 1);
+}
+static int pad_operator(cfdh_ctx *c, CsrDev &M, int lpr, int kcap, dbuf<int> &cnt) {
+  M.pad_k = 0; M.pad_lpr = 0; M.pad_tail_rows = 0; M.pad_empty_slots = 0;
+  if (M.n <= 0 || M.nnz <= 0 || !M.rowptr.p || !M.col.p || !M.val.p) return 0;
+  const int K = cfdh_pad::choose_k(M.n, M.nnz, lpr, kcap);
+  if (K == 0) return 0;
+  const size_t slots = cfdh_pad::slot_count(M.n, K, lpr);
+  HIPCHK(c, M.pcol.alloc(slots)); HIPCHK(c, M.pval.alloc(slots));
+  HIPCHK(c, cnt.zero(c->stream));
+  hipLaunchKernelGGL(pad_fill_kernel, dim3((unsigned)((slots + TPB - 1) / TPB)), dim3(TPB), 0, c->stream, M.n, K, lpr, M.rowptr.p, M.col.p, M.val.p,
+                     M.pcol.p, M.pval.p, cnt.p);
+  HIPCHK(c, hipGetLastError());
+  int h[2] = {0, 0};
+  HIPCHK(c, hipMemcpyAsync(h, cnt.p, 2 * sizeof(int), hipMemcpyDeviceToHost, c->stream));
+  HIPCHK(c, hipStreamSynchronize(c->stream));
+  M.pad_k = K; M.pad_lpr = lpr; M.pad_tail_rows = h[0]; M.pad_empty_slots = h[1];
+  return 0;
+}
+int cfdh_amg_pad_levels(cfdh_ctx *c, AmgHier &H) {
+  if (!c->trim || !H.fused || c->nranks > 1) return 0;
+  dbuf<int> cnt;
+  HIPCHK(c, cnt.alloc(2));
+  for (size_t l = 1; l < H.lev.size(); l++) {
+    AmgLevel *L = H.lev[l];
+    if (!L->fine) CHK(pad_operator(c, L->G, cfdh_pad::down_lpr(L->G.n, L->G.nnz), 4, cnt));
+    if (L->sell) continue;
+    CHK(pad_operator(c, L->Sb, L->Dn > 0 ? 64 : 8, 2, cnt));
+    if (L->Dn == 0) CHK(pad_operator(c, L->Sc, 8, 2, cnt));
+  }
+  if (c->opt.verbose) {
+    fprintf(stderr, "[cfdh]   padded coarse operators (lanes x slots, rows with a tail):");
+    for (size_t l = 1; l < H.lev.size(); l++)
+      for (const CsrDev *M : {&H.lev[l]->G, &H.lev[l]->Sb, &H.lev[l]->Sc})
+        if (M->pad_k > 0) fprintf(stderr, " L%zu %s %d x %d, %lld of %d", l, M == &H.lev[l]->G ? "G" : (M == &H.lev[l]->Sb ? "Sb" : "Sc"), M->pad_lpr, M->pad_k, M->pad_tail_rows, M->n);
+    fprintf(stderr, "\n");
+  }
+  return 0;
+}
 
 int cfdh_amg_setup_dev(cfdh_ctx *c, AmgHier &H, CsrDev &A0, bool singular, int ncol) {
   const double t_begin = now_ms();
@@ -1144,6 +1194,7 @@
     }
     HIPCHK(c, hipStreamSynchronize(s));
   }
+  CHK(cfdh_amg_pad_levels(c, H));
   H.valid = true;
   HIPCHK(c, hipStreamSynchronize(s));
   if (c->opt.verbose) {
diff --git a/cfd_hemodynamic_amd/csrc/cfdh_api.cpp b/cfd_hemodynamic_amd/csrc/cfdh_api.cpp
--- a/cfd_hemodynamic_amd/csrc/cfdh_api.cpp
+++ b/cfd_hemodynamic_amd/csrc/cfdh_api.cpp
@@ -83,6 +83,7 @@
   cfdh_default_options(&c->opt);
   { const char *e = getenv("CFDH_NO_GRAPH"); c->use_graph = !(e && e[0] == '1'); }
   { const char *e = getenv("CFDH_SOLVE_LEAN"); c->lean = !(e && e[0] == '0'); }
+  { const char *e = getenv("CFDH_ITER_TRIM"); c->trim = !(e && e[0] == '0'); }
   {
     cfdh_ctx::SolveEnv &v = c->env;
     const char *e;
@@ -621,6 +622,17 @@
     for (int i = 0; i < d; i++) z[(size_t)d * v + i] = o[(size_t)d * k + i];
     z[(size_t)d * c->nv + v] = o[(size_t)d * c->nvo + k];
   }
+  return 0;
+}
+
+int cfdh_gram_solve(cfdh_ctx *c, int k, const double *hd, double *y, int32_t *rank, int32_t *used) {
+  NOT_IPCS(c, "cfdh_gram_solve");
+  if (!c || !hd || !y || !rank || !used) return CFDH_E_ARG;
+  ENTER(c);
+  if (c->nranks > 1) return cfdh_fail(c, CFDH_E_STATE, "cfdh_gram_solve: one GPU only");
+  int r = 0, u = 0;
+  CHK(cfdh_gram_solve_dev(c, k, hd, y, &r, &u));
+  *rank = r; *used = u;
   return 0;
 }
 
@@ -1222,6 +1234,16 @@
     case 88: return c->guess_last_rank;
     case 89: return c->guess_last_k;
     case 85: return c->lean ? 1 : 0;
+    case 90: return c->trim ? 1 : 0;
+    case 91: case 92: case 93: case 94: case 95: case 96: {
+      const AmgHier *hs[2] = {&c->hA, c->opt.pc_type >= 1 ? &c->hL : &c->hS};
+      int64_t ops[2] = {0, 0}, slots = 0, nnz = 0, tails = 0, empty = 0;
+      for (int h = 0; h < 2; h++)
+        for (const AmgLevel *l : hs[h]->lev)
+          for (const CsrDev *M : {&l->G, &l->Sb, &l->Sc})
+            if (M->pad_k > 0) { ops[h]++; slots += (int64_t)M->n * M->pad_k * M->pad_lpr; nnz += M->nnz; tails += M->pad_tail_rows; empty += M->pad_empty_slots; }
+      return what == 91 ? ops[0] : what == 92 ? ops[1] : what == 93 ? slots : what == 94 ? nnz : what == 95 ? tails : empty;
+    }
     case 75: return c->pc_valid ? 1 : 0;
     case 76: return c->singular;
     case 77: return c->form;
diff --git a/cfd_hemodynamic_amd/csrc/cfdh_internal.hpp b/cfd_hemodynamic_amd/csrc/cfdh_internal.hpp
--- a/cfd_hemodynamic_amd/csrc/cfdh_internal.hpp
+++ b/cfd_hemodynamic_amd/csrc/cfdh_internal.hpp
@@ -82,6 +82,11 @@
   dbuf<int> sptr, scol;
   dbuf<float> sval, svalw;
   dbuf<float> valf;
+  int pad_k = 0, pad_lpr = 0;
+  long long pad_tail_rows = 0;
+  long long pad_empty_slots = 0;
+  dbuf<int> pcol;
+  dbuf<double> pval;
 };
 enum { CFDH_UP_CSR = 1, CFDH_UP_SELL = 2, CFDH_UP_CSRF = 4};
 
@@ -353,6 +358,7 @@
   std::vector<int> hist_its;
   double ksp_last_relres = 0;
   bool lean = true;
+  bool trim = true;
   struct SolveEnv {
     int krylov_fp32 = 1;
     bool guess_check = false;
@@ -394,6 +400,7 @@
 bool cfdh_amg_dev_enabled(const cfdh_ctx *c);
 int cfdh_amg_setup_dev(cfdh_ctx *c, AmgHier &H, CsrDev &A0, bool singular, int ncol);
 int cfdh_level_setup_dev(cfdh_ctx *c, AmgLevel &L, CsrDev &A, double ratio, int ncol);
+int cfdh_amg_pad_levels(cfdh_ctx *c, AmgHier &H);
 int cfdh_proxy_dev(cfdh_ctx *c, CsrDev &out);
 int cfdh_proxy_ras_dev(cfdh_ctx *c, CsrDev &out);
 int cfdh_cc_h_dev(cfdh_ctx *c, double alpha, double beta, CsrDev &out);
@@ -494,6 +501,7 @@
 int v_gram(cfdh_ctx *c, int n, const double *W, int ld, int k, const double *b, double *out_dev);
 int v_multiaxpy(cfdh_ctx *c, int n, const double *V, int ld, int nvec, const double *h_dev, double *w);
 int v_gs_update_normalize(cfdh_ctx *c, int n, const double *V, int ld, int nvec, const double *h_dev, const double *w, double *vn, double *s_dev);
+int v_gram_solve_debug(cfdh_ctx *c, int k, const double *hd_host, double *y, int *rank, int *used);
 int v_norm_to_dev(cfdh_ctx *c, int n, const double *w, double *out_dev);
 int v_norm_to_dev_local(cfdh_ctx *c, int n, const double *w, double *out_dev);
 int v_scale_inv_dev(cfdh_ctx *c, int n, const double *w, const double *nrm_dev, double *v);
@@ -509,6 +517,7 @@
 
 int cfdh_pc_update(cfdh_ctx *c, bool force_refresh);
 int cfdh_pc_apply(cfdh_ctx *c, const double *r, double *z);
+int cfdh_gram_solve_dev(cfdh_ctx *c, int k, const double *hd, double *y, int *rank, int *used);
 int cfdh_apply_operator_dev(cfdh_ctx *c, const double *r, double *z);
 int cfdh_host_threads();
 int cfdh_fgmres(cfdh_ctx *c, const double *b, double *x, int *its, int *reason, double bnorm = -1.0);
diff --git a/cfd_hemodynamic_amd/csrc/cfdh_kernels.hip b/cfd_hemodynamic_amd/csrc/cfdh_kernels.hip
--- a/cfd_hemodynamic_amd/csrc/cfdh_kernels.hip
+++ b/cfd_hemodynamic_amd/csrc/cfdh_kernels.hip
@@ -4,6 +4,7 @@
 
 #include "cfdh_internal.hpp"
 #include "cfdh_krylov_host.hpp"
+#include "cfdh_pad_layout.hpp"
 #include "cfdh_quad_tri.h"
 
 #define TPB 256
@@ -1360,21 +1361,25 @@
 
 template <int LPR, typename VT, typename T>
 __global__ __launch_bounds__(TPB) void fused_down_kernel(int n, const int *__restrict__ rowptr, const int *__restrict__ col,
-                                                         const VT *__restrict__ val, const T *__restrict__ x, T *__restrict__ y) {
+                                                         const VT *__restrict__ val, const T *__restrict__ x, T *__restrict__ y,
+                                                         int K, const int *__restrict__ pcol, const double *__restrict__ pval) {
   const int gid = blockIdx.x * TPB + threadIdx.x;
   const int row = gid / LPR, l = gid % LPR;
   T a = vzero((const T *)nullptr);
   if (row < n) {
+    const size_t pb = (size_t)row * K * LPR + l;
+    int cidx[4];
+    double cval[4];
+#pragma unroll
+    for (int q = 0; q < 4; q++) if (q < K) { cidx[q] = pcol[pb + (size_t)q * LPR]; cval[q] = pval[pb + (size_t)q * LPR]; }
     const int ks = rowptr[row], ke = rowptr[row + 1];
-    int cidx[4];
-    VT cval[4];
-#pragma unroll
-    for (int q = 0; q < 4; q++) { const int k = ks + l + q * LPR; if (k < ke) { cidx[q] = col[k]; cval[q] = val[k]; } }
+#pragma unroll
+    for (int q = 0; q < 4; q++) { const int k = ks + l + q * LPR; if (q >= K && k < ke) { cidx[q] = col[k]; cval[q] = (double)val[k]; } }
     T g[4];
 #pragma unroll
-    for (int q = 0; q < 4; q++) { const int k = ks + l + q * LPR; if (k < ke) g[q] = x[cidx[q]]; }
-#pragma unroll
-    for (int q = 0; q < 4; q++) { const int k = ks + l + q * LPR; if (k < ke) a = vfma((double)cval[q], g[q], a); }
+    for (int q = 0; q < 4; q++) { const int k = ks + l + q * LPR; if (q < K || k < ke) g[q] = x[cidx[q]]; }
+#pragma unroll
+    for (int q = 0; q < 4; q++) { const int k = ks + l + q * LPR; if (q < K || k < ke) a = vfma(cval[q], g[q], a); }
     for (int k = ks + l + 4 * LPR; k < ke; k += LPR) a = vfma((double)val[k], x[col[k]], a);
   }
   a = lsum<LPR>(a);
@@ -1386,31 +1391,39 @@
                                                            const int *__restrict__ rpC, const int *__restrict__ clC,
                                                            const double *__restrict__ vlC, const T *__restrict__ xc,
                                                            T *__restrict__ x, double ea, double eb, const double *__restrict__ ezH,
-                                                           const double *__restrict__ er, const unsigned char *__restrict__ epbc) {
+                                                           const double *__restrict__ er, const unsigned char *__restrict__ epbc,
+                                                           int KB, const int *__restrict__ pcB, const double *__restrict__ pvB,
+                                                           int KC, const int *__restrict__ pcC, const double *__restrict__ pvC) {
   const int gid = blockIdx.x * TPB + threadIdx.x;
   const int row = gid >> 3, l = gid & 7;
   T a = vzero((const T *)nullptr);
   if (row < n) {
+    int cb[2], cc[2];
+    double vb[2], vc[2];
+    const size_t pB = (size_t)row * KB * 8 + l, pC = (size_t)row * KC * 8 + l;
+#pragma unroll
+    for (int q = 0; q < 2; q++) {
+      if (q < KB) { cb[q] = pcB[pB + 8 * q]; vb[q] = pvB[pB + 8 * q]; }
+      if (q < KC) { cc[q] = pcC[pC + 8 * q]; vc[q] = pvC[pC + 8 * q]; }
+    }
     const int kb = rpB[row] + l, keB = rpB[row + 1];
     int kc = 0, keC = 0;
     if (rpC) { kc = rpC[row] + l; keC = rpC[row + 1]; }
-    int cb[2], cc[2];
-    double vb[2], vc[2];
 #pragma unroll
     for (int q = 0; q < 2; q++) {
-      if (kb + 8 * q < keB) { cb[q] = clB[kb + 8 * q]; vb[q] = vlB[kb + 8 * q]; }
-      if (kc + 8 * q < keC) { cc[q] = clC[kc + 8 * q]; vc[q] = vlC[kc + 8 * q]; }
+      if (q >= KB && kb + 8 * q < keB) { cb[q] = clB[kb + 8 * q]; vb[q] = vlB[kb + 8 * q]; }
+      if (q >= KC && kc + 8 * q < keC) { cc[q] = clC[kc + 8 * q]; vc[q] = vlC[kc + 8 * q]; }
     }
     T gb[2], gc[2];
 #pragma unroll
     for (int q = 0; q < 2; q++) {
-      if (kb + 8 * q < keB) gb[q] = b[cb[q]];
-      if (kc + 8 * q < keC) gc[q] = xc[cc[q]];
+      if (q < KB || kb + 8 * q < keB) gb[q] = b[cb[q]];
+      if (q < KC || kc + 8 * q < keC) gc[q] = xc[cc[q]];
     }
 #pragma unroll
     for (int q = 0; q < 2; q++) {
-      if (kb + 8 * q < keB) a = vfma(vb[q], gb[q], a);
-      if (kc + 8 * q < keC) a = vfma(vc[q], gc[q], a);
+      if (q < KB || kb + 8 * q < keB) a = vfma(vb[q], gb[q], a);
+      if (q < KC || kc + 8 * q < keC) a = vfma(vc[q], gc[q], a);
     }
     for (int k = kb + 16; k < keB; k += 8) a = vfma(vlB[k], b[clB[k]], a);
     for (int k = kc + 16; k < keC; k += 8) a = vfma(vlC[k], xc[clC[k]], a);
@@ -1464,18 +1477,26 @@
 __global__ __launch_bounds__(TPB) void fused_up_dense_kernel(int n, const int *__restrict__ rpB, const int *__restrict__ clB,
                                                              const double *__restrict__ vlB, const T *__restrict__ b,
                                                              const float *__restrict__ D, int nc, const T *__restrict__ bc,
-                                                             T *__restrict__ x) {
+                                                             T *__restrict__ x, int KB, const int *__restrict__ pcB,
+                                                             const double *__restrict__ pvB) {
   const int gid = blockIdx.x * TPB + threadIdx.x;
   const int row = gid >> 6, l = gid & 63;
   T a = vzero((const T *)nullptr);
   if (row < n) {
-    for (int k = rpB[row] + l, ke = rpB[row + 1]; k < ke; k += 64) a = vfma(vlB[k], b[clB[k]], a);
+    int cb[2];
+    double vb[2];
+    const size_t pB = (size_t)row * KB * 64 + l;
+#pragma unroll
+    for (int q = 0; q < 2; q++) if (q < KB) { cb[q] = pcB[pB + 64 * q]; vb[q] = pvB[pB + 64 * q]; }
     const float *Dr = D + (size_t)row * nc;
     float dv[12];
     T bv[12];
 #pragma unroll
     for (int q = 0; q < 12; q++) { const int j = l + 64 * q; if (j < nc) { dv[q] = Dr[j]; bv[q] = bc[j]; } }
 #pragma unroll
+    for (int q = 0; q < 2; q++) if (q < KB) a = vfma(vb[q], b[cb[q]], a);
+    for (int k = rpB[row] + l + 64 * KB, ke = rpB[row + 1]; k < ke; k += 64) a = vfma(vlB[k], b[clB[k]], a);
+#pragma unroll
     for (int q = 0; q < 12; q++) { const int j = l + 64 * q; if (j < nc) a = vfma((double)dv[q], bv[q], a); }
     for (int j = l + 768; j < nc; j += 64) a = vfma((double)Dr[j], bc[j], a);
   }
@@ -1485,14 +1506,17 @@
 
 template <typename VT, typename T>
 static void launch_down(cfdh_ctx *c, const CsrDev &G, const VT *val, const T *x, T *y) {
-  const long long avg = G.n > 0 ? (G.nnz + G.n - 1) / G.n : 1;
-  const int lpr = avg > 96 ? 64 : (avg > 48 ? 32 : (avg > 20 ? 16 : 8));
+  const int lpr = cfdh_pad::down_lpr(G.n, G.nnz);
+  const int K = (sizeof(VT) == sizeof(double) && G.pad_lpr == lpr) ? G.pad_k : 0;
+  const int *pc = G.pcol.p;
+  const double *pv = G.pval.p;
   dim3 block(TPB), grid((unsigned)(((long long)G.n * lpr + TPB - 1) / TPB));
-  if (lpr == 64) hipLaunchKernelGGL((fused_down_kernel<64, VT, T>), grid, block, 0, c->stream, G.n, G.rowptr.p, G.col.p, val, x, y);
-  else if (lpr == 32) hipLaunchKernelGGL((fused_down_kernel<32, VT, T>), grid, block, 0, c->stream, G.n, G.rowptr.p, G.col.p, val, x, y);
-  else if (lpr == 16) hipLaunchKernelGGL((fused_down_kernel<16, VT, T>), grid, block, 0, c->stream, G.n, G.rowptr.p, G.col.p, val, x, y);
-  else hipLaunchKernelGGL((fused_down_kernel<8, VT, T>), grid, block, 0, c->stream, G.n, G.rowptr.p, G.col.p, val, x, y);
-}
+  if (lpr == 64) hipLaunchKernelGGL((fused_down_kernel<64, VT, T>), grid, block, 0, c->stream, G.n, G.rowptr.p, G.col.p, val, x, y, K, pc, pv);
+  else if (lpr == 32) hipLaunchKernelGGL((fused_down_kernel<32, VT, T>), grid, block, 0, c->stream, G.n, G.rowptr.p, G.col.p, val, x, y, K, pc, pv);
+  else if (lpr == 16) hipLaunchKernelGGL((fused_down_kernel<16, VT, T>), grid, block, 0, c->stream, G.n, G.rowptr.p, G.col.p, val, x, y, K, pc, pv);
+  else hipLaunchKernelGGL((fused_down_kernel<8, VT, T>), grid, block, 0, c->stream, G.n, G.rowptr.p, G.col.p, val, x, y, K, pc, pv);
+}
+static inline int pad_k_for(const CsrDev &M, int lpr) { return M.pad_lpr == lpr ? M.pad_k : 0; }
 
 template <typename T>
 static int amg_cycle_fused(cfdh_ctx *c, AmgHier &H, const T *b, T *x, int prof, int l0 = 0) {
@@ -1516,7 +1540,7 @@
       T *xu = nl - 2 == l0 ? x : (T *)U->x.p;
       const int un = (nl - 2 == 0 && c->up0_rows > 0 && c->up0_rows < U->n) ? c->up0_rows : U->n;
       hipLaunchKernelGGL((fused_up_dense_kernel<T>), dim3((unsigned)((64ll * un + TPB - 1) / TPB)), dim3(TPB), 0, c->stream, un,
-                         U->Sb.rowptr.p, U->Sb.col.p, U->Sb.val.p, bu, U->D.p, U->Dn, bl, xu);
+                         U->Sb.rowptr.p, U->Sb.col.p, U->Sb.val.p, bu, U->D.p, U->Dn, bl, xu, pad_k_for(U->Sb, 64), U->Sb.pcol.p, U->Sb.pval.p);
       l = nl - 3;
     } else {
       if (H.coarse_n > 0)
@@ -1530,7 +1554,8 @@
         hipLaunchKernelGGL((fused_up_csr_kernel<T>), dim3((unsigned)((8ll * L->n + TPB - 1) / TPB)), dim3(TPB), 0, c->stream, L->n,
                            L->Sb.rowptr.p, L->Sb.col.p, L->Sb.val.p, bl, (const int *)nullptr, (const int *)nullptr,
                            (const double *)nullptr, (const T *)nullptr, xl, 0.0, 0.0, (const double *)nullptr, (const double *)nullptr,
-                           (const unsigned char *)nullptr);
+                           (const unsigned char *)nullptr, pad_k_for(L->Sb, 8), L->Sb.pcol.p, L->Sb.pval.p, 0, (const int *)nullptr,
+                           (const double *)nullptr);
       l = nl - 2;
     }
   }
@@ -1556,7 +1581,8 @@
     else
       hipLaunchKernelGGL((fused_up_csr_kernel<T>), dim3((unsigned)((8ll * nrow + TPB - 1) / TPB)), dim3(TPB), 0, c->stream, nrow,
                          L->Sb.rowptr.p, L->Sb.col.p, L->Sb.val.p, bl, L->Sc.rowptr.p, L->Sc.col.p, L->Sc.val.p, (const T *)N->x.p, xl,
-                         ea, eb, ezH, er, epbc);
+                         ea, eb, ezH, er, epbc, pad_k_for(L->Sb, 8), L->Sb.pcol.p, L->Sb.pval.p, pad_k_for(L->Sc, 8), L->Sc.pcol.p,
+                         L->Sc.pval.p);
     if (prof && l == 0) prof_end(c, prof);
   }
   HIPCHK(c, hipGetLastError());
@@ -2263,12 +2289,31 @@
   HIPCHK(c, hipStreamSynchronize(c->stream));
   return 0;
 }
+__global__ __launch_bounds__(64) void gram_solve_lds_kernel(int k, const double *__restrict__ hd, double *__restrict__ y, double *__restrict__ info) {
+  __shared__ cfdh_krylov::GramWork ws;
+  __shared__ double s_hd[8 * 9], s_y[8];
+  __shared__ int s_rank, s_used;
+  for (int i = threadIdx.x; i < 8 * (k + 1); i += 64) s_hd[i] = hd[i];
+  __syncthreads();
+  if (threadIdx.x == 0) {
+    int r = 0;
+    s_used = cfdh_krylov::gram_solve_ws<true>(k, s_hd, s_y, &r, ws) ? 1 : 0;
+    s_rank = r;
+  }
+  __syncthreads();
+  if ((int)threadIdx.x < k) { y[threadIdx.x] = s_y[threadIdx.x]; info[3 + threadIdx.x] = s_y[threadIdx.x]; }
+  if (threadIdx.x == 0) { info[1] = s_used ? 1.0 : 0.0; info[2] = (double)s_rank; }
+}
+static void launch_gram_solve(cfdh_ctx *c, int k, const double *hd, double *y, double *info) {
+  if (c->trim) hipLaunchKernelGGL(gram_solve_lds_kernel, dim3(1), dim3(64), 0, c->stream, k, hd, y, info);
+  else hipLaunchKernelGGL(gram_solve_kernel, dim3(1), dim3(64), 0, c->stream, k, hd, y, info);
+}
 #define CFDH_LEAN_S2 12
 int v_guess_combine(cfdh_ctx *c, int n, const double *U, const double *W, int ld, int k, const double *hd, const double *b, double *x, double *r) {
   if (k < 1 || k > 8) return cfdh_fail(c, CFDH_E_STATE, "projected guess: %d kept vectors", k);
   const int nb = vgrid(n) > c->red_blocks ? c->red_blocks : vgrid(n);
   double *mir = lean_mirror(c);
-  hipLaunchKernelGGL(gram_solve_kernel, dim3(1), dim3(64), 0, c->stream, k, hd, c->ky.p, mir);
+  launch_gram_solve(c, k, hd, c->ky.p, mir);
   hipLaunchKernelGGL(guess_combine_kernel, dim3(nb), dim3(TPB), 0, c->stream, n, U, W, (size_t)ld, k, (const double *)c->ky.p, b, x, r, c->red_partial.p);
   hipLaunchKernelGGL(reduce_final_kernel<0>, dim3(1), dim3(TPB), 0, c->stream, nb, nb, c->red_partial.p, c->red_out.p + CFDH_LEAN_S2, mir);
   HIPCHK(c, hipGetLastError());
@@ -2278,6 +2323,19 @@
   CHK(lean_sync(c));
   const double *m = c->h_pinned + CFDH_MIRROR_OFF;
   *beta = sqrt(m[0]);
+  *used = m[1] != 0.0;
+  *rank = (int)m[2];
+  for (int i = 0; i < k; i++) y[i] = m[3 + i];
+  return 0;
+}
+int v_gram_solve_debug(cfdh_ctx *c, int k, const double *hd_host, double *y, int *rank, int *used) {
+  if (k < 1 || k > 8) return cfdh_fail(c, CFDH_E_ARG, "Gram solve: k = %d outside 1 .. 8", k);
+  HIPCHK(c, hipStreamSynchronize(c->stream));
+  HIPCHK(c, hipMemcpyAsync(c->kh.p, hd_host, sizeof(double) * 8 * (size_t)(k + 1), hipMemcpyHostToDevice, c->stream));
+  launch_gram_solve(c, k, c->kh.p, c->ky.p, lean_mirror(c));
+  HIPCHK(c, hipGetLastError());
+  CHK(lean_sync(c));
+  const double *m = c->h_pinned + CFDH_MIRROR_OFF;
   *used = m[1] != 0.0;
   *rank = (int)m[2];
   for (int i = 0; i < k; i++) y[i] = m[3 + i];
diff --git a/cfd_hemodynamic_amd/csrc/cfdh_krylov_host.hpp b/cfd_hemodynamic_amd/csrc/cfdh_krylov_host.hpp
--- a/cfd_hemodynamic_amd/csrc/cfdh_krylov_host.hpp
+++ b/cfd_hemodynamic_amd/csrc/cfdh_krylov_host.hpp
@@ -11,10 +11,27 @@
 
 namespace cfdh_krylov {
 
-CFDH_HD inline bool gram_solve(int k, const double *hd, double *y, int *rank) {
+struct GramWork {
   double G[64], Lc[64], dg[8], g[8], yy[8], t[8];
   int piv[8];
   bool taken[8];
+};
+template <bool STRICT>
+CFDH_HD inline double gram_prod(double a, double b) {
+  if constexpr (STRICT) {
+#ifdef __clang__
+#pragma clang fp contract(off)
+#endif
+    return a * b;
+  } else {
+    return a * b;
+  }
+}
+template <bool STRICT>
+CFDH_HD inline bool gram_solve_ws(int k, const double *hd, double *y, int *rank, GramWork &ws) {
+  double *G = ws.G, *Lc = ws.Lc, *dg = ws.dg, *g = ws.g, *yy = ws.yy, *t = ws.t;
+  int *piv = ws.piv;
+  bool *taken = ws.taken;
   for (int i = 0; i < k; i++) {
     for (int q = 0; q < k; q++) { G[q * k + i] = hd[i * 8 + q]; Lc[q * k + i] = 0.0; }
     g[i] = hd[k * 8 + i]; yy[i] = 0.0; taken[i] = false;
@@ -32,7 +49,7 @@
     for (int it = 0; it < k; it++) {
       int p = -1;
       for (int i = 0; i < k; i++) if (!taken[i] && (p < 0 || dg[i] > dg[p])) p = i;
-      if (p < 0 || !(dg[p] > 1e-10 * G[p * k + p]) || !(dg[p] > 1e-14 * dmax0)) break;
+      if (p < 0 || !(dg[p] > gram_prod<STRICT>(1e-10, G[p * k + p])) || !(dg[p] > gram_prod<STRICT>(1e-14, dmax0))) break;
       taken[p] = true;
       const int rr = r;
       piv[r++] = p;
@@ -41,19 +58,19 @@
       for (int i = 0; i < k; i++) {
         if (taken[i]) continue;
         double sacc = G[i * k + p];
-        for (int q = 0; q < rr; q++) sacc -= Lc[i * k + q] * Lc[p * k + q];
+        for (int q = 0; q < rr; q++) sacc -= gram_prod<STRICT>(Lc[i * k + q], Lc[p * k + q]);
         Lc[i * k + rr] = sacc / lpp;
-        dg[i] -= Lc[i * k + rr] * Lc[i * k + rr];
+        dg[i] -= gram_prod<STRICT>(Lc[i * k + rr], Lc[i * k + rr]);
       }
     }
     for (int a = 0; a < r; a++) {
       double sacc = g[piv[a]];
-      for (int q = 0; q < a; q++) sacc -= Lc[piv[a] * k + q] * t[q];
+      for (int q = 0; q < a; q++) sacc -= gram_prod<STRICT>(Lc[piv[a] * k + q], t[q]);
       t[a] = sacc / Lc[piv[a] * k + a];
     }
     for (int a = r - 1; a >= 0; a--) {
       double sacc = t[a];
-      for (int q = a + 1; q < r; q++) sacc -= Lc[piv[q] * k + a] * yy[piv[q]];
+      for (int q = a + 1; q < r; q++) sacc -= gram_prod<STRICT>(Lc[piv[q] * k + a], yy[piv[q]]);
       yy[piv[a]] = sacc / Lc[piv[a] * k + a];
     }
   }
@@ -62,6 +79,10 @@
   for (int i = 0; i < k; i++) y[i] = used ? yy[i] : 0.0;
   *rank = r;
   return used;
+}
+CFDH_HD inline bool gram_solve(int k, const double *hd, double *y, int *rank) {
+  GramWork ws;
+  return gram_solve_ws<false>(k, hd, y, rank, ws);
 }
 
 CFDH_HD inline double gs_scale(double ww, double hh2) {
diff --git a/cfd_hemodynamic_amd/csrc/cfdh_pad_layout.hpp b/cfd_hemodynamic_amd/csrc/cfdh_pad_layout.hpp
--- /dev/null
+++ b/cfd_hemodynamic_amd/csrc/cfdh_pad_layout.hpp
@@ -0,0 +1,46 @@
+#pragma once
+#include <cstddef>
+
+#ifdef __HIPCC__
+#define CFDH_PAD_HD __host__ __device__
+#else
+#define CFDH_PAD_HD
+#endif
+
+namespace cfdh_pad {
+
+CFDH_PAD_HD inline int down_lpr(long long n, long long nnz) {
+  const long long avg = n > 0 ? (nnz + n - 1) / n : 1;
+  return avg > 96 ? 64 : (avg > 48 ? 32 : (avg > 20 ? 16 : 8));
+}
+CFDH_PAD_HD inline int choose_k(long long n, long long nnz, int lpr, int kcap) {
+  int K = 0;
+  for (int k = 1; k <= kcap; k++)
+    if (2 * n * k * lpr <= 3 * nnz) K = k;
+  return n > 0 ? K : 0;
+}
+CFDH_PAD_HD inline size_t slot_count(long long n, int K, int lpr) { return (size_t)n * (size_t)K * (size_t)lpr; }
+CFDH_PAD_HD inline size_t slot_index(long long r, int K, int q, int lpr, int l) { return ((size_t)r * K + q) * lpr + l; }
+CFDH_PAD_HD inline int slot_entry(int ks, int ke, int q, int lpr, int l) {
+  const long long k = (long long)ks + l + (long long)q * lpr;
+  return k < ke ? (int)k : -1;
+}
+CFDH_PAD_HD inline long long tail_begin(int ks, int K, int lpr) { return (long long)ks + (long long)K * lpr; }
+CFDH_PAD_HD inline bool has_tail(int ks, int ke, int K, int lpr) { return tail_begin(ks, K, lpr) < ke; }
+CFDH_PAD_HD inline void fill_slot(const int *rowptr, const int *col, const double *val, long long r, int K, int q, int lpr, int l,
+                                  int *pcol, double *pval) {
+  const int ks = rowptr[r], ke = rowptr[r + 1];
+  const int k = slot_entry(ks, ke, q, lpr, l);
+  const size_t s = slot_index(r, K, q, lpr, l);
+  if (k >= 0) { pcol[s] = col[k]; pval[s] = val[k]; }
+  else { pcol[s] = ks < ke ? col[ks] : 0; pval[s] = 0.0; }
+}
+inline double lane_sum(const int *rowptr, const int *col, const double *val, const int *pcol, const double *pval, long long r, int K, int lpr,
+                       int l, const double *x) {
+  double a = 0.0;
+  for (int q = 0; q < K; q++) { const size_t s = slot_index(r, K, q, lpr, l); a += pval[s] * x[pcol[s]]; }
+  for (long long k = tail_begin(rowptr[r], K, lpr) + l; k < rowptr[r + 1]; k += lpr) a += val[k] * x[col[k]];
+  return a;
+}
+
+}
diff --git a/cfd_hemodynamic_amd/csrc/cfdh_setup.cpp b/cfd_hemodynamic_amd/csrc/cfdh_setup.cpp
--- a/cfd_hemodynamic_amd/csrc/cfdh_setup.cpp
+++ b/cfd_hemodynamic_amd/csrc/cfdh_setup.cpp
@@ -759,6 +759,7 @@
     }
   }
   H.fine_nnz = A0.nnz();
+  CHK(cfdh_amg_pad_levels(c, H));
   H.valid = true;
   HIPCHK(c, hipStreamSynchronize(c->stream));
   if (c->opt.verbose) {
diff --git a/cfd_hemodynamic_amd/csrc/cfdh_solver.cpp b/cfd_hemodynamic_amd/csrc/cfdh_solver.cpp
--- a/cfd_hemodynamic_amd/csrc/cfdh_solver.cpp
+++ b/cfd_hemodynamic_amd/csrc/cfdh_solver.cpp
@@ -748,6 +748,10 @@
   CHK(ensure_krylov(c));
   return pc_then_product(c, r, z, c->kw.p);
 }
+int cfdh_gram_solve_dev(cfdh_ctx *c, int k, const double *hd, double *y, int *rank, int *used) {
+  CHK(ensure_krylov(c));
+  return v_gram_solve_debug(c, k, hd, y, rank, used);
+}
 
 static int ensure_krylov(cfdh_ctx *c) {
   const int m = c->opt.ksp_restart;
diff --git a/include/cfdh.h b/include/cfdh.h
--- a/include/cfdh.h
+++ b/include/cfdh.h
@@ -113,6 +113,7 @@
 int cfdh_get_pcd_operator(cfdh_ctx *ctx, int64_t *nnz, int32_t *rowptr, int32_t *col, double *vals, double *mass_diag);
 int cfdh_apply_preconditioner(cfdh_ctx *ctx, const double *r, double *z);
 int cfdh_apply_operator(cfdh_ctx *ctx, const double *r, double *z, double *w);
+int cfdh_gram_solve(cfdh_ctx *ctx, int k, const double *hd, double *y, int32_t *rank, int32_t *used);
 
 #define CFDH_AMG_HIER_A 0
 #define CFDH_AMG_HIER_P 1
```

Result: slower. 424.4 (-2.2%).
